# crowsonkb/style_transfer

Measured on AMD Instinct MI355X. Metric: tile-iterations/sec, VGG-19 2048px/1024-tile (fwd+bwd, Gram/content losses, regularizers, Adam step), higher is better.
Workload: dtype f32 (fp16x2-split MFMA, fp32 accumulate)

## Files before the change

### include/stx.h

```cpp
#ifndef STX_H_
#define STX_H_

#include <stddef.h>
#include <stdint.h>

#ifdef __cplusplus
extern "C" {
#endif

typedef struct stx_engine stx_engine;

typedef enum stx_status {
    STX_OK = 0,
    STX_ERR_ARG = -1,
    STX_ERR_HIP = -2,
    STX_ERR_STATE = -3,
    STX_ERR_UNSUPPORTED = -4,
    STX_ERR_NOMEM = -5
} stx_status;

typedef enum stx_mem { STX_HOST = 0, STX_DEVICE = 1 } stx_mem;

typedef enum stx_layer_type {
    STX_LAYER_INPUT = 0, STX_LAYER_CONV = 1, STX_LAYER_RELU = 2, STX_LAYER_POOL = 3
// ... 225 lines not shown
int stx_map_place(stx_engine *e, float *dst, int channels, int dst_h, int dst_w, int y0, int x0,
                  const float *src, int h, int w);
int stx_map_roll_add(stx_engine *e, float *acc, const float *src, int channels, int h, int w,
                     const int roll_xy[2], double alpha, double init_divisor);

int stx_image_resample(stx_engine *e, const float *src, int channels, int H, int W, float *dst,
                       int out_h, int out_w, const int *bounds_x, const double *weights_x,
                       int ksize_x, const int *bounds_y, const double *weights_y, int ksize_y,
                       int clamp_min_zero);

int stx_image_regularizers(stx_engine *e, const float *img, float *grad, int H, int W,
                           const float mean_bgr[3], double tv_scale, double tv_power,
                           double p_scale, double p_power, const float *aux, double aux_scale,
                           const int aux_roll_xy[2], double *loss_out);

int stx_image_swt_haar(stx_engine *e, const float *img, float *grad, int H, int W,
                       const int roll_xy[2], double scale, double power, double *loss_out);

int stx_image_swt_haar_levels(stx_engine *e, const float *img, float *grad, int H, int W, int levels,
                              const int roll_xy[2], double scale, double power, double *loss_out);

int stx_image_swt_daub_levels(stx_engine *e, const float *img, float *grad, int H, int W,
                              int order, int levels, const int *roll_xy,
                              double scale, double power, double *loss_out);

int stx_adam_step(stx_engine *e, float *params, const float *grad, float *g1, float *g2, float *p1,
                  float *avg_out, size_t n, double lr, double b1, double b2, double bp1,
                  double corr1, double corr2, double corrp);

int stx_vec_dot(stx_engine *e, const float *x, const float *y, size_t n, double *out_host_sync);
int stx_vec_axpy(stx_engine *e, double a, const float *x, float *y, size_t n);
int stx_vec_scale(stx_engine *e, double a, float *x, size_t n);
int stx_vec_mean_abs(stx_engine *e, const float *x, size_t n, double *out_host_sync);
int stx_vec_dot_async(stx_engine *e, const float *x, const float *y, size_t n, double *out_dev);
int stx_vec_abs_sum_async(stx_engine *e, const float *x, size_t n, double *out_dev);
int stx_vec_axpy_dev(stx_engine *e, double c1, const double *a_dev, double da, double c2,
                     const double *b_dev, double db, const float *x, float *y, size_t n);
int stx_vec_scale_dev(stx_engine *e, double c, const double *den_dev, double den_div, float *x,
                      size_t n);
int stx_vec_axpy_dot_dev(stx_engine *e, double c1, const double *a_dev, double da, double c2,
                         const double *b_dev, double db, double scale_c, const double *scale_den_dev,
                         double scale_div, const float *x, const float *src, float *y, const float *z,
                         size_t n, double *out_dev);
int stx_vec_lbfgs_pair(stx_engine *e, const float *g_new, float *g_old, const float *s, float *y, size_t n,
                       double *out_dev2, double *sy_host_sync);
int stx_vec_scale2_axpy(stx_engine *e, double c1, double c2, float *s, float *params, size_t n);

int stx_image_step_stats(stx_engine *e, const float *avg, float *old, int H, int W,
                         double stats[2]);
int stx_image_step_stats_async(stx_engine *e, const float *avg, float *old, int H, int W,
                               double raw_sums[2]);

int stx_image_to_u8(stx_engine *e, const float *img, int H, int W, const float mean_bgr[3],
                    uint8_t *out_rgb_u8);

int stx_image_to_u8_luma(stx_engine *e, const float *img, const float *content, int H, int W,
                         const float mean_bgr[3], uint8_t *out_rgb_u8);
int stx_image_color_stats(stx_engine *e, const float *img, int H, int W, double out_host_sync[9]);
int stx_image_color_affine(stx_engine *e, const float *src, float *dst, int H, int W, const double A[9],
                           const double b[3], const float mean_bgr[3]);

size_t stx_image_lap_floats(int H, int W, int n_pools, const int *pools);
int stx_image_lap_target(stx_engine *e, const float *content, int H, int W, int n_pools,
                         const int *pools, float *target_out);
int stx_image_lap(stx_engine *e, const float *img, float *grad, int H, int W, int n_pools,
                  const int *pools, const double *weights, const float *target, double scale,
                  double *loss_out);

int stx_image_photo(stx_engine *e, const float *img, const float *content, float *grad, int H, int W,
                    double eps, double scale, double *loss_out);

int stx_op_conv_forward(stx_engine *e, const float *x, int Cin, int H, int W, const float *w,
                        const float *b, int Cout, int ksize, int relu, float *y);
int stx_op_conv_backward_data(stx_engine *e, const float *dy, int Cout, int H, int W,
                              const float *w, int Cin, int ksize, const float *relu_mask_data,
                              float *dx);
int stx_op_pool_forward(stx_engine *e, const float *x, int C, int H, int W, int mode, float *y);
int stx_op_pool_backward(stx_engine *e, const float *dy, const float *x, int C, int H, int W,
                         int mode, const float *relu_mask_data, float *dx);

int stx_op_style_terms(stx_engine *e, const float *feat, int channels, int h, int w,
                       const float *gram_target, float *s_out, float *normalized_out,
                       double *half_sumsq, double *abs_sum);
int stx_op_masked_style_terms(stx_engine *e, const float *feat, int channels, int h, int w,
                              const float *mask_map, int mh, int mw, int oy, int ox, const int roll_xy[2],
                              const float *gram_target, float *sgrad_out, double out[3]);
int stx_op_masked_content_terms(stx_engine *e, const float *feat, int channels, int h, int w,
                                const float *content, int ch, int cw, const float *mask_map, int oy, int ox,
                                const int roll_xy[2], float *sgrad_out, double out[3]);
int stx_op_stat_terms(stx_engine *e, const float *feat, int channels, int h, int w, const float *MU,
                      const float *SD, float *s_out, double out[2]);
int stx_op_nnfm_terms(stx_engine *e, const float *feat, int channels, int h, int w, const float *bank, int rows,
                      float *s_out, int *index_out, double out[2]);
int stx_op_nnfm_patch_terms(stx_engine *e, const float *feat, int channels, int h, int w, int patch,
                            const float *bank, int rows, float *s_out, int *index_out, double out[2]);
int stx_op_nnfm_knn_terms(stx_engine *e, const float *feat, int channels, int h, int w, int patch, int k,
                          const float *bank, int rows, float *s_out, int *index_out, double out[2]);
int stx_op_nnfm_cover_terms(stx_engine *e, const float *feat, int channels, int h, int w, int patch, int k, float cover,
                            const float *bank, int rows, float *s_out, int *index_out, int *winner_out, double out[3]);
int stx_op_nnfm_guided_terms(stx_engine *e, const float *feat, int channels, int h, int w, int k, const float *bank,
                             const int *seg_rows, int segments, const float *mask_maps, int mh, int mw, int oy, int ox,
                             const int roll_xy[2], float *s_out, int *index_out, double out[3]);
int stx_op_swd_terms(stx_engine *e, const float *feat, int channels, int h, int w, const float *V, int dirs,
                     const float *Tq, int quantiles, float *s_out, int *rank_out, double out[2]);
int stx_op_selfsim_terms(stx_engine *e, const float *feat, const float *content, int channels, int h, int w,
                         int points, float *sgrad, double sc[2], signed char *signs_out);
int stx_op_shift_terms(stx_engine *e, const float *feat, int channels, int h, int w, const int *offsets,
                       int n_offsets, const float *grams, float *s_out, double out[2]);
int stx_op_content_terms(stx_engine *e, const float *feat, int channels, int h, int w,
                         const float *content, int content_h, int content_w, int oy, int ox,
                         const int roll_xy[2], float *normalized_out, double sums[2]);

int stx_profile_enable(stx_engine *e, int on);
int stx_profile_read(stx_engine *e, char *buf, size_t buf_len, size_t *needed);

int stx_amax_audit(stx_engine *e, int on);
int stx_amax_audit_read(stx_engine *e, char *buf, size_t buf_len, size_t *needed);

int stx_last_tile_ms(stx_engine *e, float *ms);

int stx_last_tile_flops(stx_engine *e, double *algorithmic, double *issued);

int stx_clock_marks(stx_engine *e, int on);
int stx_clock_marks_read(stx_engine *e, double *mhz, int max_values, int *n_values);

#ifdef __cplusplus
}
#endif
#endif
```

### style_transfer_amd/csrc/common.h

```cpp
#pragma once

#include <hip/hip_runtime.h>

#include <vector>

#include <cstdarg>
#include <cstdio>
#include <functional>
#include <string>

#include "stx.h"

namespace stx {

constexpr float kEps = 1.1920928955078125e-07f;

void set_error(const char *fmt, ...);

const char *sw_env(const char *name);
void sw_reread();

#define STX_HIP(call)                                                                       \
    do {                                                                                    \
        hipError_t err__ = (call);                                                          \
// ... 25 lines not shown
constexpr int kBlocks = 1024;
inline int blocks_for(size_t n) {
    const size_t b = (n + 255) / 256;
    return b < (size_t)kBlocks ? (int)b : kBlocks;
}
#ifdef __HIPCC__
__device__ __forceinline__ float wave_sum_f(float v) {
#pragma unroll
    for (int off = 32; off > 0; off >>= 1) v += __shfl_down(v, off, 64);
    return v;
}

template <int NV>
__device__ __forceinline__ void block_partials(float (&v)[NV], float *partials) {
    __shared__ float red[NV][4];
#pragma unroll
    for (int k = 0; k < NV; ++k) {
        const float s = wave_sum_f(v[k]);
        if ((threadIdx.x & 63) == 0) red[k][threadIdx.x >> 6] = s;
    }
    __syncthreads();
    if (threadIdx.x == 0) {
#pragma unroll
        for (int k = 0; k < NV; ++k)
            partials[k * gridDim.x + blockIdx.x] = red[k][0] + red[k][1] + red[k][2] + red[k][3];
    }
}

__device__ __forceinline__ unsigned pool_max_code(float v00, float v01, float v10, float v11, bool hx,
                                                  bool hy) {
    unsigned arg = 0;
    float best = v00;
    if (hx && v01 > best) best = v01, arg = 1;
    if (hy && v10 > best) best = v10, arg = 2;
    if (hx && hy && v11 > best) best = v11, arg = 3;
    return arg | (best > 0.f ? 4u : 0u);
}
__device__ __forceinline__ unsigned pool_ave_code(float v00, float v01, float v10, float v11, bool hx,
                                                  bool hy) {
    return (v00 > 0.f ? 1u : 0u) | (hx && v01 > 0.f ? 2u : 0u) | (hy && v10 > 0.f ? 4u : 0u) |
           (hx && hy && v11 > 0.f ? 8u : 0u);
}
#endif


enum ConvEpilogue {
    kEpiForward = 0,
    kEpiDgrad = 1,
    kEpiSymm = 2,
    kEpiDgradInject = 3,
    kEpiPartial = 4
};

struct ContentWindow {
    int C, fh, fw;
    int ch, cw;
    int oy, ox;
    int sy, sx;
};

struct ConvInject {
    const float *sgrad = nullptr, *s_abs_sum = nullptr;
    float s_coef = 0.f;
    const float *content = nullptr, *c_sums = nullptr, *feat = nullptr;
    float c_coef = 0.f;
    ContentWindow win{};
};

struct ConvProblem {
    const float *x;
    const float *w;
    float *y;
    const float *bias;
    const float *mask;
    float *partials;
    int K, M, H, W;
    int ksize;
    int relu;
    int epilogue;
    ConvInject inject;
    unsigned char *pool_codes = nullptr;
    unsigned char *in_codes = nullptr;
    const unsigned char *mask_codes = nullptr;
    unsigned char *out_codes = nullptr;
    bool wants_codes = false;
    bool skip_y = false;
    float *pool_out = nullptr;
    int pool_mode = 0;
    float *splitk_ws = nullptr;
    size_t splitk_ws_floats = 0;
    long long *clock_out = nullptr;
    const unsigned *x_amax = nullptr;
    unsigned *y_amax = nullptr;
    const unsigned char *pin_codes = nullptr;
    int pin_mode = 0;
    bool pin_mask = false;
    int *variant_out = nullptr;
#ifdef STX_EXPERIMENT_BF3
    const void *x_split = nullptr;
#endif
};

enum class ConvFamily { Direct, Wino2, H2 };

struct ConvConfig {
    ConvFamily family;
    int id;
    int bm;
    int kc;
    int pr, pc;
    int threads;
    size_t lds_bytes;
};

ConvConfig conv_pick_config(int ksize, int K, int M, int H, int W);
ConvConfig conv_config_by_id(int id);
bool direct_takes_inject(const ConvConfig &cfg);
int conv_num_workgroups(const ConvConfig &cfg, int M, int H, int W);
size_t conv_packed_floats(const ConvConfig &cfg, int K, int M, int ksize);
int conv_pack_weights(hipStream_t s, const float *w_caffe, int Mo, int Ko, int ksize,
                      int transpose_flip, const ConvConfig &cfg, float *packed);
int conv_launch(hipStream_t s, const ConvConfig &cfg, const ConvProblem &p, bool packed_weights);
int direct_splitk_factor(const ConvConfig &cfg, const ConvProblem &p, bool packed_weights);

int splitk_reduce_launch(hipStream_t s, const ConvProblem &p, int ksplit);
int splitk_reduce_items_launch(hipStream_t s, const ConvProblem &p, const ConvConfig &cfg, int slices,
                               int item_base, int items);
__host__ __device__ inline void wino2_item_tiles(int lt, int m_tiles, int n_patches, int &pt, int &mt) {
    pt = lt / m_tiles;
    mt = lt - pt * m_tiles;
    if (m_tiles == 8 && (n_patches & 7) == 0) {
        const int g = lt >> 5, r = lt & 31;
        mt = (g & 1) * 4 + (r & 3);
        pt = (g >> 1) * 8 + (r >> 2);
    }
}

struct WinoArgs {
    const float *x;
    const float *w;
    float *y;
    const float *bias;
    const float *mask;
    int K, M, H, W;
    int n_chunks, tiles_x, tiles_y, m_tiles, ksplit;
    int w_tile_stride;
    int x_bytes, w_bytes;
    int relu;
    ConvInject inj;
    float *pool_out;
    int pool_mode;
    unsigned char *pool_codes;
    int skip_y = 0;
    unsigned char *out_codes = nullptr;
    unsigned char *in_codes = nullptr;
    const unsigned char *mask_codes = nullptr;
    long long *clock_out = nullptr;
    int item_base = 0;
    const unsigned *x_amax = nullptr;
    unsigned *y_amax = nullptr;
    const unsigned char *pin_codes = nullptr;
    int pin_mode = 0, pin_mask = 0;
#ifdef STX_EXPERIMENT_BF3
    int vp_rows = 0, vp_tp = 0;
#endif
};

bool conv_first_usable(int K, int M, int ksize);
int conv_first_workgroups(int H, int W);
int conv_first_launch(hipStream_t s, const float *x, const float *w_caffe, const float *bias, float *y,
                      int K, int H, int W, int relu, float *gram_partials, unsigned *y_amax = nullptr);

ConvConfig wino2_config(int geometry = 0);
int wino2_pick_geometry(int H, int W);
size_t wino2_packed_floats(int K, int M);
int wino2_pack_weights(hipStream_t s, const float *w_caffe, int Mo, int Ko, int transpose_flip,
                       float *packed);
int wino2_launch(hipStream_t s, const ConvConfig &cfg, const ConvProblem &p, int ksplit);
bool wino2_fuses_pool(const ConvProblem &p);
bool wino2_uses_relu_codes(const ConvProblem &p, int ksplit);
bool wino2_writes_out_codes(const ConvConfig &cfg, const ConvProblem &p);
int wino2_splitk_factor(const ConvConfig &cfg, const ConvProblem &p);
struct Wino2Tail { int items, slices; };
Wino2Tail wino2_tail_split(const ConvConfig &cfg, const ConvProblem &p);
int wino2_max_slices(const ConvConfig &cfg, const ConvProblem &p);

constexpr int kAmaxSlots = 64;
ConvConfig h2_config(int mb, int pb = 1);
ConvConfig h2_pick_config(const ConvProblem &p);
bool h2_usable(const ConvProblem &p);
size_t h2_packed_floats(int K, int M);
int h2_pack_weights(hipStream_t s, const float *w_caffe, int Mo, int Ko, int transpose_flip, float *packed);
int h2_launch(hipStream_t s, const ConvConfig &cfg, const ConvProblem &p, int ksplit);
enum { kH2Style = 1, kH2Content = 2, kH2MaskNibbles = 4, kH2MaskBlob = 8 };
int h2_variant(const ConvProblem &p, int pin, bool split);
int h2_launch_variant(hipStream_t s, const WinoArgs &a, int n_wg, int cfg_id, int pin, int var);
int h2_splitk_factor(const ConvConfig &cfg, const ConvProblem &p);
bool h2_fuses_pool(const ConvProblem &p);
bool h2_takes_pooled_input(const ConvConfig &cfg, const ConvProblem &p);
int absmax_launch(hipStream_t s, const float *x, size_t n, unsigned *slots);

size_t conv_small_packed_floats(int K);
int conv_small_pack(hipStream_t s, const float *w_caffe, int Mo, int Ko, int transpose_flip,
                    float *packed);
int conv_small_launch(hipStream_t s, const float *x, const float *packed, float *y,
                      const float *mask, int K, int M, int H, int W);

bool conv_h2_enabled();
struct ConvTuner { int device; hipStream_t stream; hipEvent_t ev0, ev1; std::function<int(const ConvConfig &, const float **)> bank; };
int conv_choose(const ConvProblem &p, bool winograd, const ConvTuner *tuner, ConvConfig *out);
struct ConvBank { int key; size_t floats; std::function<int(hipStream_t, const float *w_caffe, float *packed)> pack; };
ConvBank conv_bank(const ConvConfig &cfg, int dir, int Mo, int Ko, int ksize);
ConvBank conv_small_bank(int Mo, int Ko);
int conv_dispatch(hipStream_t s, const ConvConfig &cfg, const ConvProblem &p, double *flop_algorithmic,
                  double *flop_issued);
int conv_splitk_factor(const ConvConfig &cfg, const ConvProblem &p);
size_t conv_splitk_floats(const ConvConfig &cfg, const ConvProblem &p);
bool conv_takes_clock(const ConvConfig &cfg);
bool conv_fuses_pool(const ConvConfig &cfg, const ConvProblem &p);
bool conv_writes_pool_codes(const ConvConfig &cfg);
bool conv_reads_x_amax(const ConvConfig &cfg);
bool conv_leaves_y_amax(const ConvConfig &cfg);
bool conv_takes_inject(const ConvConfig &cfg);
bool conv_takes_pooled_input(const ConvConfig &cfg, const ConvProblem &p);
bool conv_uses_relu_codes(const ConvConfig &cfg, const ConvProblem &p, int ksplit);
bool conv_writes_out_codes(const ConvConfig &cfg, const ConvProblem &p, int ksplit);

int pool_forward_launch(hipStream_t s, const float *x, int C, int H, int W, int mode, float *y,
                        unsigned char *codes = nullptr);
int pool_backward_codes_launch(hipStream_t s, const float *dy, const unsigned char *codes, int C,
                               int H, int W, int mode, bool relu_mask, float *dx);
int pool_backward_launch(hipStream_t s, const float *dy, const float *x, int C, int H, int W,
                         int mode, bool relu_mask, float *dx);

struct GramPlan {
    int C, HW, splits, tiles;
    int parts;
    size_t partial_floats;
};
GramPlan gram_plan(int C, int HW);
bool gram_h2_usable(const float *feat, int C, int HW);
int gram_partials_launch(hipStream_t s, const float *feat, const GramPlan &plan, float *partials,
                         const unsigned *f_amax = nullptr);
int gram_finish_blocks(const GramPlan &plan);
int gram_finish_launch(hipStream_t s, const float *partials, const GramPlan &plan, float *gram_out,
                       const float *target, float *dsym, float *sumsq, unsigned short *pieces = nullptr,
                       const unsigned *f_amax = nullptr, float *block_out = nullptr);

size_t symm_pieces_elems(int C);
int symm_num_workgroups(int C, int HW);
bool symm_bf3_usable(const float *feat, const float *out, int C, int HW);
bool symm_h2_usable(const float *feat, const float *out, int C, int HW);
int symm_h2_launch(hipStream_t s, const float *feat, const float *dsym, const unsigned *d_amax, int n_damax,
                   const unsigned *f_amax, float *out, float *partials, int C, int HW);
int symm_bf3_launch(hipStream_t s, const float *feat, const float *dsym, unsigned short *pieces,
                    bool pieces_ready, float *out, float *partials, int C, int HW);

#ifdef __HIPCC__
__device__ __forceinline__ int content_origin_y(const ContentWindow &w) { return w.oy - w.sy; }
__device__ __forceinline__ int content_origin_x(const ContentWindow &w) { return w.ox - w.sx; }
__device__ __forceinline__ size_t content_index(const ContentWindow &w, int c, int y, int x) {
    int yy = (content_origin_y(w) + y) % w.ch;
    int xx = (content_origin_x(w) + x) % w.cw;
    if (yy < 0) yy += w.ch;
    if (xx < 0) xx += w.cw;
    return ((size_t)c * w.ch + yy) * w.cw + xx;
}
#endif

struct SumJob {
    const float *src;
    int n;
    float *dst;
};
int sum_jobs_launch(hipStream_t s, const SumJob *jobs, int n_jobs);
int content_sums_launch(hipStream_t s, const float *feat, const float *content,
                        const ContentWindow &win, float *sums , std::vector<SumJob> *defer = nullptr);
int inject_style_launch(hipStream_t s, float *diff, const float *sgrad, size_t n,
                        const float *abs_sum, float coef, bool accumulate, unsigned *y_amax = nullptr);
int inject_content_launch(hipStream_t s, float *diff, const float *feat, const float *content,
                          const ContentWindow &win, const float *sums, float coef, bool accumulate,
                          unsigned *y_amax = nullptr);
int relu_inplace_launch(hipStream_t s, float *x, size_t n);
int sum_partials_launch(hipStream_t s, const float *partials, int n, float *out);
int sum_partials2_launch(hipStream_t s, const float *a, int na, float *out_a, const float *b, int nb,
                         float *out_b);

constexpr int kMaskParts = 1024;
constexpr int kMaskSgradParts = 2048;
int mask_map_launch(hipStream_t s, const float *mask, int H, int W, int scale, float *out);
int mask_apply_launch(hipStream_t s, const float *feat, const float *map, const ContentWindow &win, float *fm,
                      float *m2_partials, int *n_parts);
int mask_target_launch(hipStream_t s, const float *gs, int C, const float *m2_partials, int n_parts, int HW,
                       float *out, float *a_out);
int mask_sgrad_launch(hipStream_t s, float *sgrad, const float *map, const ContentWindow &win, const float *a,
                      float *partials, int *n_parts);

constexpr int kContentMaskParts = 1024;
int content_mask_mean_launch(hipStream_t s, const float *map, const ContentWindow &win, float *a_out);
int content_mask_term_launch(hipStream_t s, const float *feat, const float *content, const float *map,
                             const ContentWindow &win, const float *a, float *sgrad, float *partials,
                             int *n_parts);

constexpr int kStatSlice = 16384;
constexpr float kStatEps = 1e-5f;
int stat_slices(int HW);
size_t stat_scratch_floats(int C, int HW);
int stat_partials_launch(hipStream_t s, const float *feat, int C, int HW, float *partials);
int stat_finish_launch(hipStream_t s, const float *partials, int C, int HW, const float *MU, const float *SD,
                       float *table, float *e_out, float *mean_out, float *sd_out);
int stat_grad_launch(hipStream_t s, const float *feat, int C, int HW, const float *table, float *sgrad,
                     float *abs_partials, int *n_parts);

constexpr int kSwdBlock = 8192;
constexpr int kSwdMaxDirs = 4096, kSwdMaxQuantiles = 65536, kSwdMaxPixels = 1 << 22;
int swd_padded(int n);
int swd_check(const char *who, int C, long long n, int D, int Q);
int swd_e_parts(int n, int D);
size_t swd_scratch_floats(int C, int n, int D);
size_t swd_work_floats(int n, int D);
int swd_project_launch(hipStream_t s, const float *feat, int C, int n, const float *V, int D, void *records);
int swd_sort_launch(hipStream_t s, void *records, int n, int D);
int swd_finish_launch(hipStream_t s, void *records, int n, int D, const float *Tq, int Q, float *G, int *rank_out,
                      float *e_parts);
int swd_sort_passes(int n);
int swd_grad_launch(hipStream_t s, const float *V, const float *G, int C, int n, int D, float *sgrad, float *abs_parts,
                    int *n_parts);
int swd_quantiles_launch(hipStream_t s, const void *records, int n, int D, int Q, float *out);

constexpr int kSelfsimMaxPoints = 4096;
constexpr float kSelfsimEps = 1e-6f;
struct SelfsimGrid {
    int g, gh, gw, N;
};
SelfsimGrid selfsim_grid(int h, int w, int points);
int selfsim_check(const char *who, int C, int points);
struct SelfsimSource {
// ... 208 lines not shown
```

### style_transfer_amd/csrc/conv_h2.hip

```cpp

#include <algorithm>
#include <cstdlib>
#include <type_traits>

#include "common.h"
#include "f16x2.h"

#ifndef STX_H2_SKIP
#define STX_H2_SKIP 0
#endif

namespace stx {

namespace {

typedef _Float16 f16x8 __attribute__((ext_vector_type(8)));
typedef float f32x16 __attribute__((ext_vector_type(16)));
typedef float f32x4 __attribute__((ext_vector_type(4)));
typedef float f32x2 __attribute__((ext_vector_type(2)));
typedef unsigned int u32x4 __attribute__((ext_vector_type(4)));
typedef unsigned int u32x3 __attribute__((ext_vector_type(3)));
typedef unsigned int u32x2v __attribute__((__vector_size__(2 * sizeof(unsigned int))));

constexpr int KC = 16;
constexpr int NT = 512;
constexpr int PC = 32, TX = PC / 2;
constexpr int EX_BYTES = 4 * 2 * 4 * 4 * 64 * 16;
template <int PB>
struct Geo {
    static constexpr int PR = 8 * PB;
    static constexpr int XR = PR + 2;
    static constexpr int RT = XR * TX;
    static constexpr int V_PIECE = RT * 32;
    static constexpr int V_BYTES = 4 * 2 * V_PIECE;
    static constexpr int FULL = RT * 4 / 512;
    static constexpr int NU = FULL + 1;
    static constexpr size_t kLds = (EX_BYTES > 2 * V_BYTES ? EX_BYTES : 2 * V_BYTES) + 64;
};
constexpr int FRAG = 1024;
constexpr int U_KY = 4 * 2 * FRAG;
constexpr int U_BLK = 3 * U_KY;
constexpr int kHeaderFloats = 64;

__device__ __forceinline__ int sgpr(int v) { return __builtin_amdgcn_readfirstlane(v); }

template <int I, int N, typename F>
__device__ __forceinline__ void static_for(F &&f) {
    if constexpr (I < N) {
        f(std::integral_constant<int, I>{});
        static_for<I + 1, N>(f);
    }
}

__device__ __forceinline__ void lds_barrier() {
    asm volatile("s_waitcnt lgkmcnt(0)\n\ts_barrier" ::: "memory");
}


}

#ifdef STX_H2_TIMING
__device__ long long g_h2_timing[8][8];
__device__ long long g_h2_epi[8][8];
#define STX_H2_STAMP(i) if (pass == 0) t_epi[i] = clock64()
#else
#define STX_H2_STAMP(i)
#endif

template <int EPI, int MB, int PB, int PIN, int VAR = 0>
__global__ __launch_bounds__(NT) void conv_h2_kernel(WinoArgs a) {
    static_assert(VAR == 0 || EPI == kEpiDgradInject, "variants are of the injecting epilogue");
    static_assert(VAR == 0 || (((VAR & 3) == 1 || (VAR & 3) == 2) && ((VAR >> 2) == 1 || (VAR >> 2) == 2)), "h2_variant's codes");
    const bool inj_style = VAR ? (VAR & 1) != 0 : a.inj.sgrad != nullptr;
    const bool inj_content = VAR ? (VAR & 2) != 0 : a.inj.content != nullptr;
    const bool mask_nibbles = VAR ? (VAR >> 2) == 1 : a.mask_codes != nullptr;
    const bool mask_blob = VAR ? (VAR >> 2) == 2 : !a.mask_codes && a.mask;
    using G = Geo<PB>;
    [[maybe_unused]] constexpr int PR = G::PR, RT = G::RT, V_PIECE = G::V_PIECE, V_BYTES = G::V_BYTES, NU = G::NU, FULL = G::FULL;
    constexpr size_t kLdsBytes = G::kLds;
    constexpr int NJ = 4 * PB;
    extern __shared__ __attribute__((aligned(16))) char ldsb[];
#ifdef STX_H2_TIMING
    const long long t_start = clock64(), w_start = wall_clock64();
#endif
    constexpr int BM = 64 * MB;

    const int tid = threadIdx.x, lane = tid & 63;
    const int wave = sgpr(tid >> 6);
    const int xi = wave & 3, wh = wave >> 2;
    const int l31 = lane & 31, half = lane >> 5;

    const int m_tiles = a.m_tiles, a_tiles_x = a.tiles_x, a_tiles_y = a.tiles_y, a_H = a.H, a_W = a.W;
    const int a_n_chunks = a.n_chunks, a_ksplit = a.ksplit, a_item_base = a.item_base, a_x_bytes = a.x_bytes,
              a_w_bytes = a.w_bytes;
    const float *const a_x = a.x, *const a_w = a.w;
    asm volatile("" ::"s"(m_tiles), "s"(a_tiles_x), "s"(a_tiles_y), "s"(a_H), "s"(a_W), "s"(a_n_chunks), "s"(a_ksplit),
                 "s"(a_item_base), "s"(a_x_bytes), "s"(a_w_bytes), "s"(a_x), "s"(a_w));
    const int nb = gridDim.x, xcd = blockIdx.x & 7, slot_x = blockIdx.x >> 3;
    const int q8 = nb >> 3, r8 = nb & 7;
    const int L = (xcd < r8 ? xcd * (q8 + 1) : r8 * (q8 + 1) + (xcd - r8) * q8) + slot_x;
    const int kslice = sgpr(EPI == kEpiPartial ? L % a_ksplit : 0);
    const int Lt = sgpr(EPI == kEpiPartial ? a_item_base + L / a_ksplit : L);
    int ptile, mtile;
    wino2_item_tiles(Lt, m_tiles, a_tiles_x * a_tiles_y, ptile, mtile);
    ptile = sgpr(ptile);
    mtile = sgpr(mtile);
    const int c_begin = sgpr(EPI == kEpiPartial ? 2 * (kslice * (a_n_chunks >> 1) / a_ksplit) : 0);
    const int c_end = sgpr(EPI == kEpiPartial ? 2 * ((kslice + 1) * (a_n_chunks >> 1) / a_ksplit) : a_n_chunks);
    const int y0 = sgpr((ptile / a_tiles_x) * PR);
    const int x0 = sgpr((ptile % a_tiles_x) * PC);
    const int m0 = mtile * BM;
    const int HW = a_H * a_W;
    const unsigned HW4 = (unsigned)HW * 4u;
    const int pih = (a_H + 1) >> 1, piw = (a_W + 1) >> 1;
    const unsigned XP4 = PIN ? (unsigned)(pih * piw) * 4u : HW4;

    constexpr unsigned kOob = 0x80000000u;
    const __amdgpu_buffer_rsrc_t rx = __builtin_amdgcn_make_buffer_rsrc(
        const_cast<float *>(a_x), 0, a_x_bytes, 0x00020000);
    const __amdgpu_buffer_rsrc_t rw = __builtin_amdgcn_make_buffer_rsrc(
        const_cast<float *>(a_w), 0, a_w_bytes, 0x00020000);
    const __amdgpu_buffer_rsrc_t rcx = __builtin_amdgcn_make_buffer_rsrc(
        const_cast<unsigned char *>(a.pin_codes), 0, PIN ? (a_x_bytes >> 2) + 3 : 0, 0x00020000);

    float sv = 0.f, out_scale = 0.f, out_scale2 = 0.f;
    auto read_scales = [&]() __attribute__((always_inline)) {
        typedef const __attribute__((address_space(4))) unsigned *kconst_u32;
        const kconst_u32 slots = (kconst_u32)(uintptr_t)a.x_amax, header = (kconst_u32)(uintptr_t)a_w;
        unsigned amax_bits = 0;
#pragma unroll
        for (int i = 0; i < kAmaxSlots; ++i) amax_bits = max(amax_bits, slots[i]);
        const int es = sgpr(h2_scale_exp(amax_bits));
        const int ew = sgpr((int)header[(a_w_bytes >> 2) + 1]);
        sv = pow2f(es);
        const int eo = -es - ew, eo1 = eo < -126 ? -126 : eo > 127 ? 127 : eo;
        out_scale = pow2f(eo1), out_scale2 = pow2f(eo - eo1);
    };

    const bool edge = x0 == 0 || x0 + PC + 2 > a.W;
    unsigned xvoff[NU], v_dst[NU];
    bool left[NU], ok2[NU], ok3[NU];
#pragma unroll
    for (int n = 0; n < NU; ++n) {
        const int u = tid + n * NT;
        const int rt = n < FULL ? u >> 2 : 128 * FULL + (tid >> 4);
        const int ch0 = n < FULL ? (u & 3) * 4 : tid & 15;
        const int st_r = rt / TX, st_t = rt % TX;
        const int st_y = y0 - 1 + st_r, st_x = x0 + 2 * st_t - 1;
        left[n] = st_x < 0;
        ok2[n] = st_x + 2 < a.W, ok3[n] = st_x + 3 < a.W;
        xvoff[n] = kOob;
        if (PIN) {
            const int w0 = (x0 >> 1) + st_t - 1;
            if ((unsigned)st_y < (unsigned)a.H && st_x + 1 < a.W)
                xvoff[n] = (unsigned)(ch0 * pih * piw + (st_y >> 1) * piw + (left[n] ? 0 : w0)) * 4u +
                           (unsigned)(st_y & 1) + ((st_y | 1) < a.H ? 2u : 0u);
        } else if ((unsigned)st_y < (unsigned)a.H && st_x + 1 < a.W)
            xvoff[n] = (unsigned)(ch0 * HW + st_y * a.W + (left[n] ? 0 : st_x)) * 4u;
        v_dst[n] = (unsigned)(rt * 32 + ((ch0 * 2) ^ ((st_t & 8) << 1)));
// ... 160 lines not shown
        }
    };

    const unsigned a_voff = (unsigned)(xi * 2 * FRAG + lane * 16);
    const unsigned w_blk0 = (unsigned)(mtile * 2 * MB + wh * MB);
    constexpr bool LEAN = MB * PB == 2;
    f16x8 af[LEAN ? 2 : 3][MB][2];
    auto a_load = [&](int aslot, int ky, int chunk) __attribute__((always_inline)) {
#pragma unroll
        for (int b = 0; b < MB; ++b) {
            const unsigned ws = (unsigned)sgpr(
                (int)(((w_blk0 + b) * (unsigned)a.n_chunks + (unsigned)chunk) * U_BLK + (unsigned)ky * U_KY));
#pragma unroll
            for (int q = 0; q < 2; ++q)
                af[aslot][b][q] = __builtin_bit_cast(
                    f16x8, __builtin_amdgcn_raw_buffer_load_b128(rw, a_voff + q * FRAG, ws, 0));
        }
    };

    f32x16 acc[MB][NJ];
#pragma unroll
    for (int b = 0; b < MB; ++b)
#pragma unroll
        for (int j = 0; j < NJ; ++j)
#pragma unroll
            for (int r = 0; r < 16; ++r) acc[b][j][r] = 0.f;

    const unsigned b_base = (unsigned)(xi * 2 * V_PIECE + ((l31 >> 4) * 2 * TX + (l31 & 15)) * 32 +
                                       ((half * 16) ^ ((l31 & 8) << 1)));
    f16x8 bq[2][2];
    auto b_read = [&](int slot, int buf, int blk) __attribute__((always_inline)) {
        const int j = blk % NJ, ky = blk / NJ;
        const char *vb = ldsb + buf * V_BYTES + b_base + (4 * (j >> 1) + (j & 1) + ky) * TX * 32;
#pragma unroll
        for (int q = 0; q < 2; ++q) bq[slot][q] = *reinterpret_cast<const f16x8 *>(vb + q * V_PIECE);
    };

#ifdef STX_H2_TIMING
    const long long t_p0 = clock64();
#endif
    static_for<0, NU>([&](auto n_c) __attribute__((always_inline)) { x_load(decltype(n_c)::value, c_begin); });
    if (LEAN) {
        a_load(0, 0, c_begin);
    } else {
#pragma unroll
        for (int ky = 0; ky < 3; ++ky) a_load(ky, ky, c_begin);
    }
    __builtin_amdgcn_sched_barrier(0);
    read_scales();
#pragma unroll
    for (int b = 0; b < MB; ++b)
#pragma unroll
        for (int j = 0; j < NJ; ++j) asm volatile("" : "+v"(acc[b][j]));
    float s_scale = 0.f, c_scale = 0.f;
    if (EPI == kEpiDgradInject) {
        const float n = (float)((size_t)a.M * HW);
        if (inj_style) s_scale = a.inj.s_coef * (1.0f / (a.inj.s_abs_sum[0] / n + kEps));
        if (inj_content) c_scale = a.inj.c_coef * (1.0f / (a.inj.c_sums[1] / n + kEps));
    }
    const int hh = wave & 1, mrow = (wave >> 1) & 1, rqp = wave >> 2;
    const bool weven = (a.W & 1) == 0;
    const int xx0 = x0 + 2 * (l31 & 15);
    const unsigned plane_bytes = (unsigned)a.M * HW4;
    const __amdgpu_buffer_rsrc_t ry = __builtin_amdgcn_make_buffer_rsrc(
        a.y + (EPI == kEpiPartial ? (size_t)kslice * a.M * HW : 0), 0, (int)plane_bytes, 0x00020000);
    const __amdgpu_buffer_rsrc_t rmask = __builtin_amdgcn_make_buffer_rsrc(
        const_cast<float *>(a.mask), 0, a.mask ? (int)plane_bytes : 0, 0x00020000);
    const __amdgpu_buffer_rsrc_t rsg = __builtin_amdgcn_make_buffer_rsrc(
        const_cast<float *>(a.inj.sgrad), 0, a.inj.sgrad ? (int)plane_bytes : 0, 0x00020000);
    const __amdgpu_buffer_rsrc_t rft = __builtin_amdgcn_make_buffer_rsrc(
        const_cast<float *>(a.inj.feat), 0, a.inj.feat ? (int)plane_bytes : 0, 0x00020000);
    const __amdgpu_buffer_rsrc_t rbias = __builtin_amdgcn_make_buffer_rsrc(
        const_cast<float *>(a.bias), 0, a.bias ? a.M * 4 : 0, 0x00020000);
    const int ph = (a.H + 1) >> 1, pw = (a.W + 1) >> 1;
    const __amdgpu_buffer_rsrc_t rpool = __builtin_amdgcn_make_buffer_rsrc(
        a.pool_out, 0, a.pool_out ? a.M * ph * pw * 4 : 0, 0x00020000);
    const __amdgpu_buffer_rsrc_t rcodes = __builtin_amdgcn_make_buffer_rsrc(
        a.pool_codes, 0, a.pool_codes ? a.M * ph * pw : 0, 0x00020000);
    const int cph = (a.H + 1) >> 1, cpw = (a.W + 1) >> 1;
    const __amdgpu_buffer_rsrc_t rmc = __builtin_amdgcn_make_buffer_rsrc(
        const_cast<unsigned char *>(a.mask_codes), 0, a.mask_codes ? a.M * cph * cpw : 0, 0x00020000);
    const __amdgpu_buffer_rsrc_t roc = __builtin_amdgcn_make_buffer_rsrc(
        a.out_codes, 0, a.out_codes ? a.M * cph * cpw : 0, 0x00020000);
    const int M_ = a.M;
    struct LaneRows {
        int yy;
        unsigned vo[2][2], vpool, vmc;
    };
    const float *const content = a.inj.content;
    const int cw_ch = a.inj.win.ch, cw_cw = a.inj.win.cw, cw_oy = a.inj.win.oy - a.inj.win.sy,
              cw_ox = a.inj.win.ox - a.inj.win.sx;
    auto lane_rows = [&](int pbi) __attribute__((always_inline)) {
        LaneRows r;
        r.yy = y0 + 8 * pbi + 4 * mrow + 2 * (l31 >> 4);
        const unsigned lane_base = (unsigned)((4 * half) * HW + r.yy * a.W + xx0) * 4u;
#pragma unroll
        for (int y = 0; y < 2; ++y)
#pragma unroll
            for (int e = 0; e < 2; ++e)
                r.vo[y][e] = (r.yy + y < a.H && xx0 + e < a.W) ? lane_base + (unsigned)(y * a.W + e) * 4u : kOob;
        const bool in = r.yy < a.H && xx0 < a.W;
        r.vpool = in ? (unsigned)((4 * half) * ph * pw + (r.yy >> 1) * pw + (xx0 >> 1)) * 4u : kOob;
        r.vmc = in ? (unsigned)((4 * half) * cph * cpw + (r.yy >> 1) * cpw + (xx0 >> 1)) : kOob;
        return r;
    };
    constexpr bool HOIST = !(PIN && PB == 2);
    LaneRows rows0{};
    if (HOIST) rows0 = lane_rows(0);
    auto ld2 = [&](const __amdgpu_buffer_rsrc_t &rs, const LaneRows &lr, int y, unsigned so, auto even_c)
                   __attribute__((always_inline)) {
        if (decltype(even_c)::value)
            return __builtin_bit_cast(f32x2, __builtin_amdgcn_raw_buffer_load_b64(rs, lr.vo[y][0], so, 0));
        f32x2 v;
        v.x = __builtin_bit_cast(float, __builtin_amdgcn_raw_buffer_load_b32(rs, lr.vo[y][0], so, 0));
        v.y = __builtin_bit_cast(float, __builtin_amdgcn_raw_buffer_load_b32(rs, lr.vo[y][1], so, 0));
        return v;
    };
    auto st2 = [&](const __amdgpu_buffer_rsrc_t &rs, const LaneRows &lr, int y, unsigned so, f32x2 v, auto even_c)
                   __attribute__((always_inline)) {
        if (STX_H2_SKIP & 8) {
            if (v.x == 1.2345e-30f) __builtin_amdgcn_raw_buffer_store_b32(0u, rs, lr.vo[y][0], so, 0);
            return;
        }
        if (decltype(even_c)::value) {
            __builtin_amdgcn_raw_buffer_store_b64(__builtin_bit_cast(u32x2v, v), rs, lr.vo[y][0], so, 0);
        } else {
            const float v0 = v.x, v1 = v.y;
            __builtin_amdgcn_raw_buffer_store_b32(__builtin_bit_cast(unsigned, v0), rs, lr.vo[y][0], so, 0);
            __builtin_amdgcn_raw_buffer_store_b32(__builtin_bit_cast(unsigned, v1), rs, lr.vo[y][1], so, 0);
        }
    };
    int ccol[2] = {0, 0};
    auto content_columns = [&](const LaneRows &lr) __attribute__((always_inline)) {
        if (EPI == kEpiDgradInject && inj_content) {
#pragma unroll
            for (int e = 0; e < 2; ++e) {
                const bool ok = lr.yy < a.H && xx0 < a.W;
                const int x = ok ? (xx0 + e < a.W ? xx0 + e : xx0) : (e && 1 < a.W ? 1 : 0);
                int r = (cw_ox + x) % cw_cw;
                ccol[e] = r < 0 ? r + cw_cw : r;
            }
        }
    };
    if (HOIST) content_columns(rows0);
#ifdef STX_H2_TIMING
    __builtin_amdgcn_sched_barrier(0);
    const long long t_p1 = clock64();
    asm volatile("s_waitcnt vmcnt(0)" ::: "memory");
    const long long t_p2 = clock64();
#endif
    static_for<0, NU>([&](auto n_c) __attribute__((always_inline)) {
        constexpr int n = decltype(n_c)::value;
        stage_all(n, 0);
        if (c_begin + 1 < c_end) x_load(n, c_begin + 1);
    });
#ifdef STX_H2_TIMING
    __builtin_amdgcn_sched_barrier(0);
    const long long t_p3 = clock64();
#endif
    lds_barrier();
    b_read(0, 0, 0);

    constexpr int NBLK = 3 * NJ;
    constexpr int PER_BLK = 3 * MB, SLOTS = (NBLK - 1) * PER_BLK;
    constexpr int NQ = PIN ? 5 : 4, NQ1 = PIN ? 3 : 2;
    constexpr int NP = NQ * NU;
    constexpr int STEP = (SLOTS - 2) / NP;
#ifdef STX_H2_NO_BRANCH
    const bool edge_fix = false;
#else
    const bool edge_fix = edge;
#endif
    auto run_chunk = [&](auto buf_c, int chunk, auto more_c) __attribute__((always_inline)) {
        constexpr bool MORE = decltype(more_c)::value;
        constexpr int BUF = decltype(buf_c)::value, buf = BUF;
        char *vnext = ldsb + (buf ^ 1) * V_BYTES;
        static_for<0, NBLK>([&](auto blk_c) __attribute__((always_inline)) {
            constexpr int blk = decltype(blk_c)::value;
            constexpr int ky = blk / NJ, j = blk % NJ, slot = blk & 1;
            if (blk == NBLK - 1) {
                __builtin_amdgcn_sched_barrier(0);
                lds_barrier();
            }
            __builtin_amdgcn_sched_barrier(0);
            if (blk < NBLK - 1) b_read(slot ^ 1, buf, blk + 1);
            else if (MORE) b_read(0, buf ^ 1, 0);
            static_for<0, PER_BLK>([&](auto m_c) __attribute__((always_inline)) {
                constexpr int m = decltype(m_c)::value;
                constexpr int b = m % MB, t = m / MB;
// ... 7 lines not shown
                    if (ky < 2) a_load(as ^ 1, ky + 1, chunk);
                    else if (MORE) a_load(as ^ 1, 0, chunk + 1);
                }
                if (MORE && !(STX_H2_SKIP & 1) && s >= 1 && (s - 1) % STEP == 0) {
                    constexpr int k = (s - 1) / STEP;
                    constexpr int n = k % NU, q = k / NU;
                    if (k < NP && PIN && q == 0) unpool(n, edge_fix);
                    else if (k < NP && n < FULL) piece(n, q - (PIN ? 1 : 0), vnext, edge_fix);
                    else if (k < NP && q < NQ1) piece_one(2 * (q - (PIN ? 1 : 0)), vnext, edge_fix);
                }
                if (MORE && !(STX_H2_SKIP & 4)) {
                    static_for<0, NU>([&](auto u_c) __attribute__((always_inline)) {
                        constexpr int u = decltype(u_c)::value;
                        if (s == 1 + (((u < FULL ? NQ : NQ1) - 1) * NU + u) * STEP + 1 && chunk + 2 < c_end)
                            x_load(u, chunk + 2);
                    });
                }
            });
            if (!LEAN && j == NJ - 1 && MORE && !(STX_H2_SKIP & 2)) a_load(ky, ky, chunk + 1);
        });
        __builtin_amdgcn_sched_barrier(0);
    };
    using yes = std::integral_constant<bool, true>;
    using no = std::integral_constant<bool, false>;
    using b0 = std::integral_constant<int, 0>;
    using b1 = std::integral_constant<int, 1>;
#ifdef STX_H2_TIMING
    const long long t_loop = clock64(), w_loop = wall_clock64();
#endif
    const bool mark = a.clock_out != nullptr && (int)blockIdx.x == (int)(gridDim.x >> 1);
    long long mark_c = 0, mark_w = 0;
    if (mark) {
        mark_c = clock64();
        mark_w = wall_clock64();
    }
    {
        int chunk = c_begin;
        for (; chunk + 2 < c_end; chunk += 2) {
            run_chunk(b0{}, chunk, yes{});
            run_chunk(b1{}, chunk + 1, yes{});
        }
        run_chunk(b0{}, chunk, yes{});
        run_chunk(b1{}, chunk + 1, no{});
    }
    if (mark) {
        const long long dc = clock64() - mark_c, dw = wall_clock64() - mark_w;
        if (tid == 0) {
            a.clock_out[0] = dw >= 100 ? dc : 0;
            a.clock_out[1] = dw >= 100 ? dw : 0;
        }
    }
#ifdef STX_H2_TIMING
    const long long t_end = clock64(), w_end = wall_clock64();
#endif

    float amax = 0.f;
    f32x4 *ex = reinterpret_cast<f32x4 *>(ldsb);

#ifdef STX_H2_TIMING
    long long t_epi[4] = {0, 0, 0, 0};
#endif
    auto epilogue_pass = [&](auto pass_c, auto even_c) __attribute__((always_inline)) {
        constexpr int pass = decltype(pass_c)::value;
        constexpr int mbi = pass % MB, pbi = pass / MB;
        const LaneRows lr = pbi == 0 && HOIST ? rows0 : lane_rows(pbi);
        if (!HOIST && pass == 0) content_columns(lr);
        int crow[2] = {0, 0};
        if (EPI == kEpiDgradInject && inj_content) {
#pragma unroll
            for (int y = 0; y < 2; ++y) {
                const bool ok = lr.yy + y < a.H && xx0 < a.W;
                int q = (cw_oy + (ok ? lr.yy + y : 0)) % cw_ch;
                crow[y] = (q < 0 ? q + cw_ch : q) * cw_cw;
            }
        }
        const int cblk = m0 + (hh * MB + mbi) * 32;
        auto chan = [&](int n) __attribute__((always_inline)) {
            const int c0 = cblk + (n & 3) + 8 * (2 * rqp + (n >> 2));
            return sgpr(c0 < M_ ? c0 : M_);
        };
        float bs[8];
        f32x2 mk[16], sg[16];
        unsigned mkb[8];
#pragma unroll
        for (int n = 0; n < 8; ++n) {
            const int c = chan(n);
            const unsigned so = (unsigned)c * HW4;
            if (EPI == kEpiForward) {
                bs[n] = a.bias ? __builtin_bit_cast(float, __builtin_amdgcn_raw_buffer_load_b32(
                                                               rbias, (unsigned)half * 16u, (unsigned)c * 4u, 0))
                               : 0.f;
            } else if (EPI != kEpiPartial) {
                if (mask_nibbles) mkb[n] = __builtin_amdgcn_raw_buffer_load_b8(rmc, lr.vmc, (unsigned)(c * cph * cpw), 0);
#pragma unroll
                for (int y = 0; y < 2; ++y) {
                    if (mask_blob && !(STX_H2_SKIP & 16)) mk[2 * n + y] = ld2(rmask, lr, y, so, even_c);
                    if (EPI == kEpiDgradInject && inj_style) sg[2 * n + y] = ld2(rsg, lr, y, so, even_c);
                }
            }
        }
        STX_H2_STAMP(0);
        __syncthreads();
        STX_H2_STAMP(1);
#pragma unroll
        for (int j = 0; j < 4; ++j)
#pragma unroll
            for (int rq = 0; rq < 4; ++rq)
                ex[(((xi * 2 + wh) * 4 + j) * 4 + rq) * 64 + lane] =
                    f32x4{acc[mbi][4 * pbi + j][4 * rq], acc[mbi][4 * pbi + j][4 * rq + 1],
                          acc[mbi][4 * pbi + j][4 * rq + 2], acc[mbi][4 * pbi + j][4 * rq + 3]};
        __syncthreads();
        STX_H2_STAMP(2);
#pragma unroll
        for (int rqi = 0; rqi < 2; ++rqi) {
            const int rq = 2 * rqp + rqi;
            f32x4 o[2][2];
#pragma unroll
            for (int s = 0; s < 2; ++s) {
                f32x4 p[4];
#pragma unroll
                for (int c = 0; c < 4; ++c) p[c] = ex[(((c * 2 + hh) * 4 + 2 * mrow + s) * 4 + rq) * 64 + lane];
                o[s][0] = (p[0] + p[1] + p[2]) * out_scale * out_scale2;
                o[s][1] = (p[1] - p[2] - p[3]) * out_scale * out_scale2;
            }
#pragma unroll
            for (int e = 0; e < 4; ++e) {
                const int n = 4 * rqi + e;
                const int c = chan(n);
                const unsigned so = (unsigned)c * HW4;
                f32x2 v[2];
#pragma unroll
                for (int y = 0; y < 2; ++y) v[y] = f32x2{o[y][0][e], o[y][1][e]};
                if (EPI == kEpiForward) {
                    if (a.bias) {
#pragma unroll
                        for (int y = 0; y < 2; ++y) v[y].x += bs[n], v[y].y += bs[n];
                    }
                    if (a.relu) {
#pragma unroll
                        for (int y = 0; y < 2; ++y) v[y].x = fmaxf(v[y].x, 0.f), v[y].y = fmaxf(v[y].y, 0.f);
                    }
                } else if (EPI != kEpiPartial) {
#pragma unroll
                    for (int y = 0; y < 2; ++y) {
                        if (mask_nibbles) {
                            const unsigned nib = mkb[n] >> (2 * y);
                            v[y].x = (nib & 1u) ? v[y].x : 0.f;
                            v[y].y = (nib & 2u) ? v[y].y : 0.f;
                        } else if (mask_blob && !(STX_H2_SKIP & 16)) {
                            v[y].x = mk[2 * n + y].x > 0.f ? v[y].x : 0.f;
                            v[y].y = mk[2 * n + y].y > 0.f ? v[y].y : 0.f;
                        }
                        if (EPI == kEpiDgradInject) {
                            if (inj_content) {
                                const f32x2 ft = ld2(rft, lr, y, so, even_c);
                                const int mm = c + 4 * half;
                                const int cm = mm < a.M ? mm : 0;
                                const float *cp = content + (size_t)cm * cw_ch * cw_cw + crow[y];
                                v[y].x += c_scale * (ft.x - cp[ccol[0]]);
                                v[y].y += c_scale * (ft.y - cp[ccol[1]]);
                            }
                            if (inj_style) {
                                v[y].x += s_scale * sg[2 * n + y].x;
                                v[y].y += s_scale * sg[2 * n + y].y;
                            }
                        }
                    }
                }
#pragma unroll
                for (int y = 0; y < 2; ++y) {
                    if (EPI != kEpiForward || !a.skip_y) st2(ry, lr, y, so, v[y], even_c);
                    if (EPI != kEpiPartial)
                        amax = fmaxf(amax, fmaxf(lr.vo[y][0] != kOob ? fabsf(v[y].x) : 0.f,
                                                 lr.vo[y][1] != kOob ? fabsf(v[y].y) : 0.f));
                }
                if (EPI == kEpiForward && a.out_codes) {
                    const unsigned nib = (lr.vo[0][0] != kOob && v[0].x > 0.f ? 1u : 0u) |
                                         (lr.vo[0][1] != kOob && v[0].y > 0.f ? 2u : 0u) |
                                         (lr.vo[1][0] != kOob && v[1].x > 0.f ? 4u : 0u) |
                                         (lr.vo[1][1] != kOob && v[1].y > 0.f ? 8u : 0u);
                    __builtin_amdgcn_raw_buffer_store_b8((unsigned char)nib, roc, lr.vmc, (unsigned)(c * cph * cpw), 0);
                }
                if (EPI == kEpiForward && a.pool_out) {
                    const bool hy = lr.yy + 1 < a.H, hx = decltype(even_c)::value || xx0 + 1 < a.W;
                    float pr;
                    if (a.pool_mode == STX_POOL_MAX) {
                        pr = hx ? fmaxf(v[0].x, v[0].y) : v[0].x;
                        if (hy) pr = hx ? fmaxf(fmaxf(pr, v[1].x), v[1].y) : fmaxf(pr, v[1].x);
                    } else {
                        pr = (v[0].x + (hx ? v[0].y : 0.f) + (hy ? v[1].x : 0.f) + (hx && hy ? v[1].y : 0.f)) *
                             (hy ? (hx ? 0.25f : 0.5f) : (hx ? 0.5f : 1.0f));
                    }
                    __builtin_amdgcn_raw_buffer_store_b32(__builtin_bit_cast(unsigned, pr), rpool, lr.vpool,
                                                          (unsigned)c * (unsigned)(ph * pw * 4), 0);
                    if (a.pool_codes) {
                        const unsigned code = a.pool_mode == STX_POOL_MAX
                                                  ? pool_max_code(v[0].x, v[0].y, v[1].x, v[1].y, hx, hy)
                                                  : pool_ave_code(v[0].x, v[0].y, v[1].x, v[1].y, hx, hy);
                        __builtin_amdgcn_raw_buffer_store_b8((unsigned char)code, rcodes, lr.vpool >> 2,
                                                             (unsigned)c * (unsigned)(ph * pw), 0);
                    }
                }
            }
        }
    };
    static_for<0, MB * PB>([&](auto pass_c) __attribute__((always_inline)) {
        [[maybe_unused]] constexpr int pass = decltype(pass_c)::value;
        if (weven) epilogue_pass(pass_c, yes{});
        else epilogue_pass(pass_c, no{});
        STX_H2_STAMP(3);
    });
    if (EPI != kEpiPartial && a.y_amax) {
#pragma unroll
        for (int d = 32; d >= 1; d >>= 1) amax = fmaxf(amax, __shfl_xor(amax, d));
        float *wmax = reinterpret_cast<float *>(ldsb + kLdsBytes - 64);
        if (lane == 0) wmax[wave] = amax;
        __syncthreads();
        if (tid == 0) {
#pragma unroll
            for (int w = 1; w < 8; ++w) amax = fmaxf(amax, wmax[w]);
            atomicMax(a.y_amax + (blockIdx.x & (kAmaxSlots - 1)), __builtin_bit_cast(unsigned, amax));
        }
    }
#ifdef STX_H2_TIMING
    if (blockIdx.x == gridDim.x - 3 && lane == 0) {
        g_h2_timing[wave][0] = t_loop - t_start, g_h2_timing[wave][1] = t_end - t_loop;
        g_h2_timing[wave][2] = clock64() - t_end;
        g_h2_timing[wave][3] = w_loop - w_start, g_h2_timing[wave][4] = w_end - w_loop;
        g_h2_timing[wave][5] = wall_clock64() - w_end;
        for (int i = 0; i < 4; ++i) g_h2_epi[wave][i] = t_epi[i] - t_end;
        g_h2_epi[wave][4] = t_p0 - t_start, g_h2_epi[wave][5] = t_p1 - t_p0, g_h2_epi[wave][6] = t_p2 - t_p1, g_h2_epi[wave][7] = t_p3 - t_p2;
    }
#endif
}

template <int EPI, int MB, int PB, int PIN = 0, int VAR = 0>
static int h2_launch_epi(hipStream_t s, const WinoArgs &args, int n_wg) {
    auto kern = conv_h2_kernel<EPI, MB, PB, PIN, VAR>;
    constexpr size_t kLdsBytes = Geo<PB>::kLds;
    hipError_t e = hipFuncSetAttribute(reinterpret_cast<const void *>(kern),
                                       hipFuncAttributeMaxDynamicSharedMemorySize, (int)kLdsBytes);
    if (e != hipSuccess) {
        set_error("hipFuncSetAttribute(lds=%zu): %s", kLdsBytes, hipGetErrorString(e));
        return STX_ERR_HIP;
    }
    kern<<<n_wg, NT, kLdsBytes, s>>>(args);
    STX_CHECK_LAUNCH();
    return STX_OK;
}

#if defined(STX_H2_VARIANTS_ONLY) || !(defined(STX_H2_SPLIT_UNITS) || defined(STX_H2_DEV_SUBSET))
int h2_launch_variant(hipStream_t s, const WinoArgs &a, int n_wg, int cfg_id, int pin, int var) {
#define STX_H2_VAR(V, P)                                                                                      \
    if (var == (V) && pin == (P))                                                                             \
        return cfg_id == 1   ? h2_launch_epi<kEpiDgradInject, 2, 1, P, V>(s, a, n_wg)                         \
               : cfg_id == 2 ? h2_launch_epi<kEpiDgradInject, 1, 2, P, V>(s, a, n_wg)                         \
                             : h2_launch_epi<kEpiDgradInject, 1, 1, P, V>(s, a, n_wg);
    STX_H2_VAR(kH2Style | kH2MaskNibbles, 0)
    STX_H2_VAR(kH2Style | kH2MaskBlob, 0)
    STX_H2_VAR(kH2Content | kH2MaskNibbles, 0)
    STX_H2_VAR(kH2Content | kH2MaskBlob, 0)
    STX_H2_VAR(kH2Style | kH2MaskNibbles, 1 + STX_POOL_MAX)
    STX_H2_VAR(kH2Style | kH2MaskBlob, 1 + STX_POOL_MAX)
    STX_H2_VAR(kH2Style | kH2MaskNibbles, 1 + STX_POOL_AVE)
    STX_H2_VAR(kH2Style | kH2MaskBlob, 1 + STX_POOL_AVE)
#undef STX_H2_VAR
    set_error("h2_launch_variant: no specialised body %d for a pooled input of kind %d", var, pin);
    return STX_ERR_UNSUPPORTED;
}
#endif
#ifndef STX_H2_VARIANTS_ONLY

__global__ __launch_bounds__(256) void absmax_kernel(const float *__restrict__ x, size_t n, unsigned *slots) {
    float m = 0.f;
    const size_t head = ((16 - (reinterpret_cast<size_t>(x) & 15)) & 15) >> 2;
    const size_t h = head < n ? head : n;
    const size_t n4 = (n - h) >> 2;
    const f32x4 *x4 = reinterpret_cast<const f32x4 *>(x + h);
    for (size_t i = blockIdx.x * (size_t)256 + threadIdx.x; i < n4; i += (size_t)gridDim.x * 256) {
        const f32x4 v = x4[i];
        m = fmaxf(fmaxf(m, fmaxf(fabsf(v.x), fabsf(v.y))), fmaxf(fabsf(v.z), fabsf(v.w)));
    }
    if (blockIdx.x == 0) {
        if (threadIdx.x < h) m = fmaxf(m, fabsf(x[threadIdx.x]));
        const size_t tail = h + (n4 << 2);
        if (tail + threadIdx.x < n && threadIdx.x < 4) m = fmaxf(m, fabsf(x[tail + threadIdx.x]));
    }
#pragma unroll
    for (int d = 32; d >= 1; d >>= 1) m = fmaxf(m, __shfl_xor(m, d));
    __shared__ float wmax[4];
    if ((threadIdx.x & 63) == 0) wmax[threadIdx.x >> 6] = m;
    __syncthreads();
    if (threadIdx.x == 0)
        atomicMax(slots + (blockIdx.x & (kAmaxSlots - 1)),
                  __builtin_bit_cast(unsigned, fmaxf(fmaxf(wmax[0], wmax[1]), fmaxf(wmax[2], wmax[3]))));
}

int absmax_launch(hipStream_t s, const float *x, size_t n, unsigned *slots) {
    STX_HIP(hipMemsetAsync(slots, 0, kAmaxSlots * sizeof(unsigned), s));
    if ((reinterpret_cast<size_t>(x) & 3) != 0) {
        set_error("absmax_launch: the array is not float-aligned");
        return STX_ERR_ARG;
    }
    const int blocks = (int)std::min<size_t>((n / 4 + 2047) / 2048 + 1, 1024);
    absmax_kernel<<<blocks, 256, 0, s>>>(x, n, slots);
    STX_CHECK_LAUNCH();
    return STX_OK;
}

size_t h2_packed_floats(int K, int M) {
    return (size_t)ceil_div(M, 32) * ceil_div(K, KC) * (U_BLK / 4) + kHeaderFloats;
}

__device__ __forceinline__ float h2_u(const float *__restrict__ w, int Ko, int transpose_flip, int m, int k,
                                      int ky, int x) {
    float g[3];
#pragma unroll
    for (int b = 0; b < 3; ++b) {
        const int t = ky * 3 + b;
        g[b] = transpose_flip ? w[((size_t)k * Ko + m) * 9 + (8 - t)] : w[((size_t)m * Ko + k) * 9 + t];
    }
    return x == 0 ? g[0] : x == 1 ? (g[0] + g[1] + g[2]) * 0.5f : x == 2 ? (g[0] - g[1] + g[2]) * 0.5f : g[2];
}

__global__ void h2_bank_max_kernel(const float *__restrict__ w, int Ko, int transpose_flip, int M, int K,
                                   unsigned *header) {
    const size_t total = (size_t)M * K * 12;
    float mx = 0.f;
    for (size_t idx = blockIdx.x * (size_t)blockDim.x + threadIdx.x; idx < total;
         idx += (size_t)gridDim.x * blockDim.x) {
        const int x = idx % 4, ky = (idx / 4) % 3;
        const size_t mk = idx / 12;
        mx = fmaxf(mx, fabsf(h2_u(w, Ko, transpose_flip, (int)(mk / K), (int)(mk % K), ky, x)));
    }
#pragma unroll
    for (int d = 32; d >= 1; d >>= 1) mx = fmaxf(mx, __shfl_xor(mx, d));
    __shared__ float wmax[4];
    if ((threadIdx.x & 63) == 0) wmax[threadIdx.x >> 6] = mx;
    __syncthreads();
    if (threadIdx.x == 0)
        atomicMax(header, __builtin_bit_cast(unsigned, fmaxf(fmaxf(wmax[0], wmax[1]), fmaxf(wmax[2], wmax[3]))));
}

__global__ void h2_pack_kernel(const float *__restrict__ w, int Ko, int transpose_flip, int M, int K,
                               int n_chunks, unsigned short *__restrict__ packed, size_t total,
                               unsigned *header) {
    const int ew = h2_scale_exp(header[0]);
    const float sw = pow2f(ew);
// ... 30 lines not shown
        w_caffe, Ko, transpose_flip, M, K, header);
    STX_CHECK_LAUNCH();
    const size_t total = bank_floats * 2;
    h2_pack_kernel<<<(int)std::min<size_t>((total + 255) / 256, 8192), 256, 0, s>>>(
        w_caffe, Ko, transpose_flip, M, K, ceil_div(K, KC), reinterpret_cast<unsigned short *>(packed), total,
        header);
    STX_CHECK_LAUNCH();
    return STX_OK;
}

ConvConfig h2_config(int mb, int pb) {
    const bool two = mb != 2 && pb == 2;
    return {ConvFamily::H2, mb == 2 ? 1 : two ? 2 : 0, mb == 2 ? 128 : 64, KC, two ? 16 : 8, PC, NT,
            two ? Geo<2>::kLds : Geo<1>::kLds};
}

bool h2_usable(const ConvProblem &p) {
    if (p.ksize != 3 || p.K % (2 * KC) != 0 || p.K < 2 * KC) return false;
    if (p.epilogue != kEpiForward && p.epilogue != kEpiDgrad) return false;
    if (p.epilogue == kEpiForward && (p.wants_codes || p.in_codes)) return false;
    const double xb = 4.0 * p.K * (double)p.H * p.W, yb = 4.0 * p.M * (double)p.H * p.W;
    const double wb = 4.0 * (double)h2_packed_floats(p.K, p.M);
    return xb < 2147483648.0 && yb < 2147483648.0 && wb < 2147483648.0;
}

static double h2_plan(const ConvConfig &cfg, const ConvProblem &p, int *factor) {
    const int n_pairs = p.K / (2 * KC);
    const long n = (long)ceil_div(p.M, cfg.bm) * ceil_div(p.H, cfg.pr) * ceil_div(p.W, PC);
    const double out_mb = 4e-6 * p.M * (double)p.H * p.W;
    const double t_chunk = cfg.id == 1 ? 2.75 : cfg.id == 2 ? 3.5 : 2.0, t_fixed = cfg.id != 0 ? 17.0 : 8.5;
    const bool may_split = p.epilogue == kEpiForward || p.epilogue == kEpiDgrad;
    double best_cost = 0;
    int best = 1;
    for (int f = 1; f <= 8 && (f == 1 || (may_split && n_pairs / f >= 2)); ++f) {
        const double rounds = (double)ceil_div((int)std::min<long>(n * f, 1 << 30), 256);
        double c = rounds * (2.0 * ceil_div(n_pairs, f) * t_chunk + t_fixed);
        if (f > 1) c += (f + 1) * out_mb / 3.0 + 5.0;
        if (f == 1 || c < best_cost) {
            best_cost = c;
            best = f;
        }
    }
    *factor = best;
    return best_cost;
}

int h2_splitk_factor(const ConvConfig &cfg, const ConvProblem &p) {
    int f;
    h2_plan(cfg, p, &f);
    return f;
}

ConvConfig h2_pick_config(const ConvProblem &p) {
    int f;
    ConvConfig best = h2_config(1, 1);
    double best_cost = h2_plan(best, p, &f);
    const ConvConfig cand[2] = {h2_config(2, 1), h2_config(1, 2)};
    for (int i = 0; i < 2; ++i) {
        if (i == 0 && p.M % 128 != 0) continue;
        const double c = h2_plan(cand[i], p, &f);
        if (c < best_cost) best_cost = c, best = cand[i];
    }
    return best;
}

bool h2_takes_pooled_input(const ConvConfig &cfg, const ConvProblem &p) {
    return p.epilogue == kEpiDgrad && h2_usable(p) && h2_splitk_factor(cfg, p) == 1;
}

bool h2_fuses_pool(const ConvProblem &p) {
    return p.pool_out && p.epilogue == kEpiForward && (((size_t)p.y | (size_t)p.pool_out) & 7) == 0;
}

#ifdef STX_H2_DEV_SUBSET
template __global__ void conv_h2_kernel<0, 2, 1, 0>(WinoArgs);
template __global__ void conv_h2_kernel<0, 1, 2, 0>(WinoArgs);
template __global__ void conv_h2_kernel<1, 2, 1, 0>(WinoArgs);
template __global__ void conv_h2_kernel<3, 2, 1, 0>(WinoArgs);
template __global__ void conv_h2_kernel<3, 1, 2, 1>(WinoArgs);
template __global__ void conv_h2_kernel<3, 2, 1, 0, kH2Style | kH2MaskNibbles>(WinoArgs);
template __global__ void conv_h2_kernel<3, 2, 1, 0, kH2Content | kH2MaskNibbles>(WinoArgs);
template __global__ void conv_h2_kernel<3, 1, 2, 1, kH2Style | kH2MaskBlob>(WinoArgs);
template __global__ void conv_h2_kernel<3, 2, 1, 1, kH2Style | kH2MaskNibbles>(WinoArgs);
#else
int h2_variant(const ConvProblem &p, int pin, bool split) {
    if (split || p.epilogue != kEpiDgrad) return 0;
    const bool style = p.inject.sgrad != nullptr, content = p.inject.content != nullptr;
    if (style == content) return 0;
    if (!p.mask_codes && !p.mask) return 0;
    if (content && pin) return 0;
    const char *env = sw_env("STX_H2_INJECT_GENERIC");
    if (env && atoi(env) != 0) return 0;
    return (style ? kH2Style : kH2Content) | (p.mask_codes ? kH2MaskNibbles : kH2MaskBlob);
}

int h2_launch(hipStream_t s, const ConvConfig &cfg, const ConvProblem &p, int ksplit) {
    if (!h2_usable(p) || !p.x_amax) {
        set_error("h2_launch: unsupported problem (K %d, epilogue %d, input maximum %s)", p.K, p.epilogue,
                  p.x_amax ? "given" : "missing");
        return STX_ERR_UNSUPPORTED;
    }
    WinoArgs a;
    a.x = p.x;
    a.w = p.w;
    a.y = p.y;
    a.bias = p.bias;
    a.mask = p.mask;
    a.K = p.K;
    a.M = p.M;
    a.H = p.H;
    a.W = p.W;
    a.n_chunks = p.K / KC;
    a.tiles_x = ceil_div(p.W, PC);
    a.tiles_y = ceil_div(p.H, cfg.pr);
    a.m_tiles = ceil_div(p.M, cfg.bm);
    a.ksplit = 1;
    a.w_tile_stride = 0;
    a.relu = p.relu;
    a.inj = p.inject;
    a.pool_out = nullptr;
    a.pool_codes = nullptr;
    a.pool_mode = p.pool_mode;
    a.x_bytes = (int)(4.0 * p.K * (double)p.H * p.W);
    const bool pin = p.pin_codes != nullptr;
    if (pin) {
        if (!h2_takes_pooled_input(cfg, p) || ksplit > 1) {
            set_error("h2_launch: a pooled input goes with unsplit backward launches only");
            return STX_ERR_UNSUPPORTED;
        }
        a.x_bytes = (int)(4.0 * p.K * (double)((p.H + 1) / 2) * ((p.W + 1) / 2));
        a.pin_codes = p.pin_codes;
        a.pin_mode = p.pin_mode;
        a.pin_mask = p.pin_mask ? 1 : 0;
    }
    a.w_bytes = (int)(4 * (h2_packed_floats(p.K, p.M) - kHeaderFloats));
    a.clock_out = p.clock_out;
    a.x_amax = p.x_amax;
    a.y_amax = p.y_amax;
    a.mask_codes = p.epilogue == kEpiDgrad ? p.mask_codes : nullptr;
    a.out_codes = p.epilogue == kEpiForward && p.relu ? p.out_codes : nullptr;
    const bool inject = p.epilogue == kEpiDgrad && (p.inject.sgrad || p.inject.content);
    int n_wg = a.m_tiles * a.tiles_x * a.tiles_y;
    const bool split = ksplit > 1 && p.splitk_ws && p.splitk_ws_floats >= (size_t)ksplit * p.M * p.H * p.W;
    if (split) {
        a.ksplit = ksplit;
        a.y = p.splitk_ws;
        a.y_amax = nullptr;
        a.mask_codes = nullptr;
        a.out_codes = nullptr;
        n_wg *= ksplit;
    } else if (h2_fuses_pool(p)) {
        a.pool_out = p.pool_out;
        a.pool_codes = p.pool_codes;
        a.skip_y = p.skip_y && p.pool_codes != nullptr;
    }
    const int epi = split ? kEpiPartial : inject ? kEpiDgradInject : p.epilogue;
    const int pin_kind = pin ? 1 + p.pin_mode : 0;
    const int var = h2_variant(p, pin_kind, split);
    if (p.variant_out) *p.variant_out = var;
    if (var) return h2_launch_variant(s, a, n_wg, cfg.id, pin_kind, var);
#define STX_H2_CASE(E)                                                                   \
    case E:                                                                              \
        STX_TRY(cfg.id == 1   ? (h2_launch_epi<E, 2, 1>(s, a, n_wg))                   \
                : cfg.id == 2 ? (h2_launch_epi<E, 1, 2>(s, a, n_wg))                   \
                                : (h2_launch_epi<E, 1, 1>(s, a, n_wg)));                 \
        break;
#define STX_H2_PIN_CASE(E, P)                                                            \
    case E:                                                                              \
        STX_TRY(cfg.id == 1   ? (h2_launch_epi<E, 2, 1, P>(s, a, n_wg))                \
                : cfg.id == 2 ? (h2_launch_epi<E, 1, 2, P>(s, a, n_wg))                \
                                : (h2_launch_epi<E, 1, 1, P>(s, a, n_wg)));              \
        break;
    if (pin && p.pin_mode == STX_POOL_MAX) {
        switch (epi) {
            STX_H2_PIN_CASE(kEpiDgrad, 1 + STX_POOL_MAX)
            STX_H2_PIN_CASE(kEpiDgradInject, 1 + STX_POOL_MAX)
        }
        return STX_OK;
    }
    if (pin) {
        switch (epi) {
            STX_H2_PIN_CASE(kEpiDgrad, 1 + STX_POOL_AVE)
            STX_H2_PIN_CASE(kEpiDgradInject, 1 + STX_POOL_AVE)
        }
        return STX_OK;
    }
#undef STX_H2_PIN_CASE
    switch (epi) {
        STX_H2_CASE(kEpiForward)
        STX_H2_CASE(kEpiDgrad)
        STX_H2_CASE(kEpiDgradInject)
        STX_H2_CASE(kEpiPartial)
        default:
            set_error("h2_launch: no kernel for epilogue %d", p.epilogue);
            return STX_ERR_UNSUPPORTED;
    }
#undef STX_H2_CASE
    return split ? splitk_reduce_launch(s, p, ksplit) : STX_OK;
}
#endif
#endif

}
```

### style_transfer_amd/csrc/engine.cpp

```cpp

#include <algorithm>
#include <atomic>
#include <cstdlib>
#include <cstring>

#include "engine.h"

namespace stx {

static thread_local std::string g_error;

void set_error(const char *fmt, ...) {
    char buf[1024];
    va_list ap;
    va_start(ap, fmt);
    vsnprintf(buf, sizeof buf, fmt, ap);
    va_end(ap);
    g_error = buf;
}

int alloc_scalars(stx_engine *e, size_t n, size_t *index) {
    stx_engine::ScalarArena &a = e->A();
    if (a.used + n > e->scalars_cap) {
        set_error("scalar arena exhausted (%zu + %zu > %zu)", a.used, n, e->scalars_cap);
// ... 264 lines not shown
    }
    {
        std::vector<int> h224(e->blobs.size(), 224);
        for (size_t li = 1; li < e->layers.size(); ++li) {
            const Layer &L = e->layers[li];
            if (L.type == STX_LAYER_CONV) h224[L.top_blob] = h224[L.bottom_blob];
            if (L.type == STX_LAYER_POOL) h224[L.top_blob] = pooled_len(h224[L.bottom_blob]);
        }
        for (size_t bi = 0; bi < e->blobs.size(); ++bi) e->blobs[bi].scale = 224 / h224[bi];
    }
    enable_peer_access(device);
    STX_HIP(hipStreamCreateWithFlags(&e->stream, hipStreamNonBlocking));
    for (int i = 0; i < stx_engine::kTimed; ++i) {
        STX_HIP(hipEventCreate(&e->ev_start[i]));
        STX_HIP(hipEventCreate(&e->ev_stop[i]));
    }
    STX_HIP(hipEventCreate(&e->ev_tune0));
    STX_HIP(hipEventCreate(&e->ev_tune1));
    if (const char *env = sw_env("STX_AUTOTUNE")) e->autotune = atoi(env) != 0;
    if (const char *env = sw_env("STX_POOL_CODES")) e->pool_codes = atoi(env) != 0;
    if (const char *env = sw_env("STX_WINOGRAD")) e->winograd = atoi(env) != 0;
    e->scalars_cap = kScalarFloats;
    for (stx_engine::ScalarArena &a : e->arena) {
        STX_TRY(a.scalars.ensure(e->scalars_cap * sizeof(float)));
        STX_HIP(hipHostMalloc(reinterpret_cast<void **>(&a.host), e->scalars_cap * sizeof(float),
                              hipHostMallocDefault));
        STX_TRY(a.dscalars.ensure(e->dscalars_cap * sizeof(double)));
        STX_HIP(hipHostMalloc(reinterpret_cast<void **>(&a.dhost), e->dscalars_cap * sizeof(double),
                              hipHostMallocDefault));
        STX_HIP(hipEventCreateWithFlags(&a.fence, hipEventDisableTiming));
    }
    STX_TRY(e->red_scratch.ensure(9 * kBlocks * sizeof(float)));
    {
        std::lock_guard<std::mutex> lock(e->sh->mutex);
        e->sh->members.push_back(e.get());
    }
    *out = e.release();
    return STX_OK;
}

extern "C" {

int stx_engine_create(int device, const stx_layer_desc *layers, int n_layers, stx_engine **out) {
    return build_engine(device, layers, n_layers, nullptr, out);
}

int stx_engine_create_shared(stx_engine *primary, stx_engine **out) {
    if (!primary || !out) {
        set_error("stx_engine_create_shared: bad arguments");
        return STX_ERR_ARG;
    }
    std::vector<stx_layer_desc> descs(primary->layers.size());
    for (size_t i = 0; i < descs.size(); ++i) {
        const Layer &L = primary->layers[i];
        stx_layer_desc &d = descs[i];
        d.name = L.name.c_str();
        d.type = L.type;
        d.bottom = L.bottom.empty() ? nullptr : L.bottom.c_str();
        d.top = L.top.c_str();
        d.num_output = i == 0 ? primary->blobs[L.top_blob].channels : L.num_output;
        d.kernel_size = L.ksize;
        d.pad = L.pad;
        d.stride = L.stride;
        d.pool_mode = L.pool_mode;
    }
    STX_TRY(primary->set_device());
    for (stx_engine *m : primary->sh->members) STX_HIP(hipStreamSynchronize(m->stream));
    return build_engine(primary->device, descs.data(), (int)descs.size(), primary->sh, out);
}

void stx_engine_destroy(stx_engine *e) {
    if (!e) return;
    (void)hipSetDevice(e->device);
    if (e->stream) (void)hipStreamSynchronize(e->stream);
    for (auto &b : e->sgrad) b->release();
    e->marks_buf.release();
    e->amax.release();
    e->audit_buf.release();
    for (Blob &b : e->blobs) {
        b.data.release();
        b.diff.release();
        b.codes.release();
        b.relu_codes.release();
    }
    for (hipEvent_t ev : e->fence_events) (void)hipEventDestroy(ev);
    bool last;
    {
        std::lock_guard<std::mutex> lock(e->sh->mutex);
        auto &m = e->sh->members;
        m.erase(std::remove(m.begin(), m.end(), e), m.end());
        last = m.empty();
    }
    if (last) {
        for (auto &kv : e->sh->conv) {
            kv.second.w.release();
            kv.second.b.release();
            for (auto &p : kv.second.packed) p.second->release();
        }
        clear_all_targets(*e->sh);
    }
    DevBuf *bufs[] = {&e->shift_io, &e->selfsim_io, &e->swd_work, &e->swd_io, &e->nnfm_scratch, &e->stat_scratch, &e->masked_feat, &e->masked_target, &e->splitk, &e->gram_partials, &e->gram, &e->dsym, &e->dsym_pieces, &e->symm_partials,
                      &e->upload, &e->red_scratch, &e->swt_scratch, &e->lap_scratch, &e->first_gram, &e->color_sums};
    for (DevBuf *b : bufs) b->release();
    for (stx_engine::SwtTable &t : e->swt_tables) t.taps.release();
    for (stx_engine::ScalarArena &a : e->arena) {
        a.scalars.release();
        a.dscalars.release();
        if (a.host) (void)hipHostFree(a.host);
        if (a.dhost) (void)hipHostFree(a.dhost);
        if (a.fence) (void)hipEventDestroy(a.fence);
    }
    for (auto &pe : e->prof) {
        (void)hipEventDestroy(pe.start);
        (void)hipEventDestroy(pe.stop);
    }
    for (hipEvent_t ev : e->event_pool) (void)hipEventDestroy(ev);
    for (int i = 0; i < stx_engine::kTimed; ++i) {
        if (e->ev_start[i]) (void)hipEventDestroy(e->ev_start[i]);
        if (e->ev_stop[i]) (void)hipEventDestroy(e->ev_stop[i]);
    }
    if (e->ev_tune0) (void)hipEventDestroy(e->ev_tune0);
    if (e->ev_tune1) (void)hipEventDestroy(e->ev_tune1);
    if (e->stream) (void)hipStreamDestroy(e->stream);
    delete e;
}

int stx_set_conv_weights(stx_engine *e, const char *conv_layer, const float *weights,
                         const float *bias, int mem) {
    if (!e || !conv_layer || !weights) return STX_ERR_ARG;
    STX_TRY(e->set_device());
    auto it = e->layer_index.find(conv_layer);
    if (it == e->layer_index.end() || e->layers[it->second].type != STX_LAYER_CONV) {
        set_error("stx_set_conv_weights: '%s' is not a convolution layer", conv_layer);
        return STX_ERR_ARG;
    }
    std::lock_guard<std::mutex> lock(e->sh->mutex);
    const bool shared = e->sh->members.size() > 1;
    if (shared) STX_TRY(quiesce_members(e));
    ConvParams &cp = e->sh->conv[it->second];
    const size_t nw = (size_t)cp.cout * cp.cin * cp.ks * cp.ks;
    STX_TRY(cp.w.ensure(nw * sizeof(float)));
    STX_TRY(cp.b.ensure((size_t)cp.cout * sizeof(float)));
    STX_TRY(copy_in(e, cp.w.ptr, weights, mem, nw * sizeof(float)));
    if (bias)
        STX_TRY(copy_in(e, cp.b.ptr, bias, mem, (size_t)cp.cout * sizeof(float)));
    else
        STX_HIP(hipMemsetAsync(cp.b.ptr, 0, (size_t)cp.cout * sizeof(float), e->stream));
    if (mem == STX_HOST || shared) STX_HIP(hipStreamSynchronize(e->stream));
    for (auto &p : cp.packed) p.second->release();
    cp.packed.clear();
    cp.set = true;
    return STX_OK;
}

int stx_sync(stx_engine *e) {
    if (!e) return STX_ERR_ARG;
    STX_TRY(e->set_device());
    return do_sync(e);
}

int stx_fence(stx_engine *e, unsigned long long *ticket) {
    if (!e || !ticket) return STX_ERR_ARG;
    STX_TRY(e->set_device());
    stx_engine::ScalarArena &a = e->A();
    STX_HIP(hipEventRecord(a.fence, e->stream));
    a.ticket = e->next_ticket++;
// ... 262 lines not shown
```

### style_transfer_amd/csrc/engine.h

```cpp
#pragma once

#include <deque>
#include <map>
#include <memory>
#include <mutex>
#include <string>
#include <vector>

#include "common.h"

namespace stx {

struct DevBuf {
    void *ptr = nullptr;
    size_t bytes = 0;
    int ensure(size_t need) {
        if (need <= bytes) return STX_OK;
        if (ptr) STX_HIP(hipFree(ptr));
        ptr = nullptr;
        bytes = 0;
        const size_t want = (need + 255) & ~(size_t)255;
        hipError_t err = hipMalloc(&ptr, want);
        if (err != hipSuccess) {
            set_error("hipMalloc(%zu bytes) failed: %s", want, hipGetErrorString(err));
            ptr = nullptr;
            return STX_ERR_NOMEM;
        }
        bytes = want;
        return STX_OK;
    }
    void release() {
        if (ptr) (void)hipFree(ptr);
        ptr = nullptr;
        bytes = 0;
    }
    float *f() const { return static_cast<float *>(ptr); }
};

struct Layer {
    std::string name, bottom, top;
    int type = 0, num_output = 0, ksize = 0, pad = 0, stride = 1, pool_mode = 0;
    int bottom_blob = -1, top_blob = -1;
};

struct Blob {
    std::string name;
    int channels = 0;
    int producer = -1;
    bool relu = false;
    int scale = 1;
    int h = 0, w = 0;
    DevBuf data, diff;
    DevBuf codes;
    bool codes_valid = false;
    DevBuf relu_codes;
    bool relu_codes_valid = false;
    bool relu_codes_wanted = false;
    int amax_data = -1, amax_diff = -1;
    size_t count() const { return (size_t)channels * h * w; }
};

struct ConvParams {
    int cin = 0, cout = 0, ks = 0;
    DevBuf w, b;
    bool set = false;
    std::map<int, std::unique_ptr<DevBuf>> packed;
};

struct ContentTarget {
    int index, blob, C, h, w;
    std::unique_ptr<DevBuf> feat;
    void release() { feat->release(); }
};

struct StyleTarget {
    int index, blob, C;
    std::unique_ptr<DevBuf> gram;
    void release() { gram->release(); }
};

struct StyleMask {
    int index, blob, h, w;
    std::unique_ptr<DevBuf> map;
    void release() { map->release(); }
};

struct ContentMask {
    int blob, h, w;
    std::unique_ptr<DevBuf> map;
    void release() { map->release(); }
};

struct StatTarget {
    int blob, C;
    double weight;
    std::unique_ptr<DevBuf> ms;
    void release() { ms->release(); }
};

struct NnfmTarget {
    int blob, C, rows;
    double weight;
    std::unique_ptr<DevBuf> bank, pieces;
    int patch = 1, k = 1;
    float cover = 0.f;
    NnfmSegments segs{};
    int mh = 0, mw = 0;
    std::unique_ptr<DevBuf> maps;
    const unsigned short *pieces_hi_lo() const { return static_cast<const unsigned short *>(pieces->ptr); }
    void release() {
        bank->release();
        pieces->release();
        if (maps) maps->release();
    }
};

struct SwdTarget {
    int blob, C, D, Q;
    double weight;
    std::unique_ptr<DevBuf> vt;
    const float *V() const { return vt->f(); }
    const float *Tq() const { return vt->f() + (size_t)D * C; }
    void release() { vt->release(); }
};

struct SelfsimTarget {
    int blob, points;
    double weight;
    void release() {}
};

struct ShiftTarget {
    int blob, C;
    ShiftOffsets off;
    double weight;
    std::unique_ptr<DevBuf> grams;
    void release() { grams->release(); }
};

struct LossTerm {
// ... 197 lines not shown
    clear_dependent_targets(sh);
}
ConvProblem conv_fwd_problem(const float *x, float *y, const float *bias, int Cin, int Cout, int H, int W,
                             int ks, int relu);
ConvProblem conv_bwd_problem(const float *dy, float *dx, const float *mask, int Cout, int Cin, int H, int W,
                             int ks);
int attach_splitk(stx_engine *e, const ConvConfig &cfg, ConvProblem &p);
int launch_conv(stx_engine *e, const ConvConfig &cfg, const ConvProblem &problem);
int amax_scratch(stx_engine *e, unsigned **out);
constexpr size_t kMaxAmaxAudit = 2048;
int amax_audit_note(stx_engine *e, hipStream_t stream, const std::string &consumer, const std::string &blob,
                    bool diff, const unsigned *slots, const float *x, size_t n);
struct Tap {
    int blob;
    const stx_tap *t;
};

struct TileCall {
    const float *img;
    int img_mem, th, tw, rx, ry, start[2];
    const stx_tap *taps;
    int n_taps;
    float *grad_out;
    int grad_mem;
};

enum class TermKind { Content, MaskedContent, Style, MaskedStyle, Stat, Nnfm, NnfmGuided, Swd, Selfsim, Shift, Dream };
constexpr size_t kNoSlot = ~(size_t)0;
constexpr size_t kResidualScalars = 2 + 2 * 1024;

struct PlannedTerm {
    TermKind kind;
    int tap;
    const float *target, *mask;
    ContentWindow win;
    double coef;
    size_t scalars;
    size_t scratch_off, scratch_len;
    size_t sgrad_off;
    const NnfmTarget *nnfm = nullptr;
    const SwdTarget *swd = nullptr;
    int points = 0;
    const ShiftTarget *shift = nullptr;
};

struct TilePlan {
    std::vector<Tap> order;
    std::vector<char> needed;
    std::vector<int> tap_of;
    std::deque<stx_tap> extra;
    bool sums_late;
    bool interleave;
    std::vector<PlannedTerm> terms;
    std::vector<size_t> first_term;
    std::vector<size_t> sgrad_floats;
    size_t scratch_floats = 0, scalars = 0;
};

struct Term {
    enum Kind { Gradient, Residual } kind;
    const float *src;
    const float *sums;
    float coef;
    ContentWindow win;
};

struct TileRun {
    stx_engine *e;
    const TilePlan &plan;
    PendingLoss &pl;
    std::vector<std::vector<Term>> terms;
    std::vector<SumJob> sum_jobs;
    std::vector<SumJob> *defer() { return plan.sums_late ? &sum_jobs : nullptr; }
};

int plan_terms(stx_engine *e, const TileCall &c, TilePlan &plan);
int queue_tap_terms(TileRun &run, size_t k);
int inject_terms(TileRun &run, size_t k, bool &diff_written);
bool tap_fusable(const TileRun &run, size_t k);
ConvInject make_inject(const TileRun &run, size_t k, const Blob &bot);
int launch_style_terms(stx_engine *e, hipStream_t stream, const float *feat, int C, int h, int w,
                       const float *target, float *sgrad, float *sc, const std::string &name,
                       const unsigned *f_amax = nullptr, float *term_scratch = nullptr,
                       std::vector<SumJob> *defer = nullptr);
constexpr size_t kMaskScratchFloats = kMaskParts + kMaskSgradParts;
int launch_masked_style_terms(stx_engine *e, hipStream_t stream, const float *feat, int C, int h, int w,
                              const float *mask_map, const ContentWindow &win, const float *target,
                              float *sgrad, float *sc, const std::string &name, const unsigned *f_amax,
                              float *term_scratch, float *mask_scratch, std::vector<SumJob> *defer);
int launch_stat_terms(stx_engine *e, hipStream_t stream, const float *feat, int C, int h, int w, const float *MU,
                      const float *SD, float *sgrad, float *sc, const std::string &name, float *stat_scratch,
                      std::vector<SumJob> *defer);
int launch_nnfm_terms(stx_engine *e, hipStream_t stream, const float *feat, int C, int h, int w, int patch,
                      const float *bank, const unsigned short *pieces, int rows, float *sgrad, int *idx_out, float *sc,
                      const std::string &name, float *scratch, std::vector<SumJob> *defer, int k = 1, float cover = 0.f,
                      int *winner_out = nullptr, float *e_cov_out = nullptr);
int launch_nnfm_guided_terms(stx_engine *e, hipStream_t stream, const float *feat, int C, int h, int w,
                             const float *bank, const unsigned short *pieces, const NnfmSegments &segs,
                             const float *maps, const ContentWindow &win, float *sgrad, int *idx_out, float *sc,
                             const std::string &name, float *scratch, std::vector<SumJob> *defer, int k,
                             bool scale_by_a);
int launch_swd_terms(stx_engine *e, hipStream_t stream, const float *feat, int C, int h, int w, const float *V, int D,
                     const float *Tq, int Q, float *sgrad, int *rank_out, float *sc, const std::string &name,
                     float *scratch, std::vector<SumJob> *defer);
int launch_selfsim_terms(stx_engine *e, hipStream_t stream, const float *feat, const SelfsimSource &content, int C,
                         int h, int w, int points, float *sgrad, signed char *signs_out, float *sc,
                         const std::string &name, float *scratch, std::vector<SumJob> *defer);
int launch_shift_terms(stx_engine *e, hipStream_t stream, const float *feat, int C, int h, int w,
                       const ShiftOffsets &off, const float *targets, float *sgrad, float *sc, const std::string &name,
                       float *scratch, std::vector<SumJob> *defer);
constexpr size_t kContentMaskScratchFloats = 2 * kContentMaskParts;
int launch_masked_content_terms(stx_engine *e, hipStream_t stream, const float *feat, const float *content,
                                const float *mask_map, const ContentWindow &win, float *sgrad, float *sc,
                                const std::string &name, float *partials, std::vector<SumJob> *defer);
#pragma GCC visibility pop

}
```

### style_transfer_amd/csrc/op_hooks.cpp

```cpp

#include <cmath>

#include "engine.h"

extern "C" {

static int scratch_pack(stx_engine *e, const ConvBank &bank, const float *w, const float **packed) {
    STX_TRY(e->upload.ensure(bank.floats * sizeof(float)));
    STX_TRY(bank.pack(e->stream, w, e->upload.f()));
    *packed = e->upload.f();
    return STX_OK;
}

static int hook_conv(stx_engine *e, ConvProblem &p, const float *w, int Mo, int Ko, int dir) {
    ConvConfig cfg;
    STX_TRY(conv_choose(p, e->winograd, nullptr, &cfg));
    if (conv_reads_x_amax(cfg)) {
        unsigned *scratch;
        STX_TRY(amax_scratch(e, &scratch));
        STX_TRY(absmax_launch(e->stream, p.x, (size_t)p.K * p.H * p.W, scratch));
        STX_HIP(hipMemsetAsync(scratch + kAmaxSlots, 0, kAmaxSlots * sizeof(unsigned), e->stream));
        p.x_amax = scratch;
        p.y_amax = scratch + kAmaxSlots;
    }
// ... 310 lines not shown

int stx_op_nnfm_guided_terms(stx_engine *e, const float *feat, int C, int h, int w, int k, const float *bank,
                             const int *seg_rows, int segments, const float *mask_maps, int mh, int mw, int oy, int ox,
                             const int roll_xy[2], float *s_out, int *index_out, double out[3]) {
    const char *const who = "stx_op_nnfm_guided_terms";
    if (!e || !feat || !bank || !seg_rows || !mask_maps || !s_out || !index_out || !out || C <= 0 || h <= 0 || w <= 0) {
        set_error("%s: bad arguments", who);
        return STX_ERR_ARG;
    }
    if (segments < 1 || segments > kNnfmMaxSegments) {
        set_error("%s: %d segments (1 to %d are expected)", who, segments, kNnfmMaxSegments);
        return STX_ERR_ARG;
    }
    if (k < 1 || k > kNnfmMaxK) {
        set_error("%s: k %d (1 to %d is expected)", who, k, kNnfmMaxK);
        return STX_ERR_ARG;
    }
    long long rows = 0;
    for (int s = 0; s < segments; ++s) {
        if (seg_rows[s] < k) {
            set_error("%s: segment %d has %d rows, fewer than k = %d", who, s, seg_rows[s], k);
            return STX_ERR_ARG;
        }
        rows += seg_rows[s];
    }
    if (oy < 0 || ox < 0 || oy + h > mh || ox + w > mw) {
        set_error("%s: window exceeds the mask maps", who);
        return STX_ERR_ARG;
    }
    if (C % 64 != 0) {
        set_error("%s: the channel count %d is not a multiple of 64", who, C);
        return STX_ERR_UNSUPPORTED;
    }
    const long long n = (long long)h * w;
    if (n >= (1ll << 31) / C || rows >= (1ll << 31) / C) {
        set_error("%s: %lld columns against %lld rows of %d channels exceed 32-bit offsets", who, n, rows, C);
        return STX_ERR_UNSUPPORTED;
    }
    const NnfmSegments segs = nnfm_segments(seg_rows, segments);
    STX_TRY(e->set_device());
    HookScalars scalars(e);
    float *sc;
    const float *host;
    STX_TRY(scalars.take(3, &sc));
    const size_t pieces = nnfm_pieces_floats((int)rows, C);
    STX_TRY(e->nnfm_scratch.ensure((pieces + nnfm_guided_scratch_floats(C, h * w, segs, k)) * sizeof(float)));
    unsigned short *bhi = static_cast<unsigned short *>(e->nnfm_scratch.ptr);
    STX_TRY(nnfm_split_rows_launch(e->stream, bank, (int)rows, C, bhi, bhi + (size_t)rows * C));
    STX_TRY(launch_nnfm_guided_terms(e, e->stream, feat, C, h, w, bank, bhi, segs, mask_maps,
                                     hook_window(C, h, w, mh, mw, oy, ox, roll_xy), s_out, index_out, sc, "op",
                                     e->nnfm_scratch.f() + pieces, nullptr, k, false));
    STX_TRY(scalars.fetch(&host));
    out[0] = (double)host[0];
    out[1] = (double)host[1];
    out[2] = (double)host[2];
    return STX_OK;
}

int stx_op_content_terms(stx_engine *e, const float *feat, int C, int h, int w,
                         const float *content, int content_h, int content_w, int oy, int ox,
                         const int roll_xy[2], float *normalized_out, double sums[2]) {
    if (!e || !feat || !content || C <= 0 || h <= 0 || w <= 0) return STX_ERR_ARG;
    if (oy < 0 || ox < 0 || oy + h > content_h || ox + w > content_w) {
        set_error("stx_op_content_terms: window exceeds the content map");
        return STX_ERR_ARG;
    }
    STX_TRY(e->set_device());
    const ContentWindow win = hook_window(C, h, w, content_h, content_w, oy, ox, roll_xy);
    HookScalars scalars(e);
    float *s;
    const float *host;
    STX_TRY(scalars.take(kResidualScalars, &s));
    STX_TRY(content_sums_launch(e->stream, feat, content, win, s));
    if (normalized_out)
        STX_TRY(inject_content_launch(e->stream, normalized_out, feat, content, win, s, 1.0f, false));
    STX_TRY(scalars.fetch(&host));
    if (sums) {
        sums[0] = (double)host[0];
        sums[1] = (double)host[1];
    }
    return STX_OK;
}

}
```

### style_transfer_amd/csrc/symm.hip

```cpp

#include <algorithm>
#include <cstdlib>
#include <cstring>

#include "bf16x3.h"
#include "common.h"
#include "f16x2.h"

#ifndef STX_SYMM_SKIP
#define STX_SYMM_SKIP 0
#endif

namespace stx {

namespace {

constexpr int kSM = 64;
constexpr int kSN = 256;
#ifndef STX_SYMM_KSK
#define STX_SYMM_KSK 32
#endif
constexpr int kSK = STX_SYMM_KSK;
constexpr int kSPC = kSK / 16;
constexpr int kSegs = kSK / 8;
constexpr int kDLoads = 3 * kSM * kSegs / 256;
constexpr int kRowBytes = 2 * kSK + 16;
#ifndef STX_SYMM_RING
#define STX_SYMM_RING 3
#endif
constexpr int kRing = STX_SYMM_RING;
constexpr int kPieceBytes = kSM * kRowBytes;
constexpr int kChunkBytes = 3 * kPieceBytes;

typedef unsigned u32x4y __attribute__((ext_vector_type(4)));

}

size_t symm_pieces_elems(int C) {
    const size_t cp = (size_t)ceil_div(C, kSM) * kSM;
    return 3 * cp * cp;
}

template <bool BIG>
__global__ __launch_bounds__(256, 2) void symm_bf3_kernel(const float *__restrict__ F,
                                                          const unsigned short *__restrict__ Dp,
                                                          float *__restrict__ S,
                                                          float *__restrict__ partials, int C, int Cp,
                                                          int HW, unsigned f_bytes, int m_tiles) {
    __shared__ __attribute__((aligned(16))) unsigned char lds[2 * kChunkBytes];
    __shared__ float wave_sum[4];
    const int tid = threadIdx.x, lane = tid & 63;
    const int wave = __builtin_amdgcn_readfirstlane(tid >> 6);
    const int l31 = lane & 31, g = lane >> 5;
    const int nb = gridDim.x, xcd = blockIdx.x & 7, slot = blockIdx.x >> 3;
    const int q8 = nb >> 3, r8 = nb & 7;
    const int L = (xcd < r8 ? xcd * (q8 + 1) : r8 * (q8 + 1) + (xcd - r8) * q8) + slot;
    const int mt = __builtin_amdgcn_readfirstlane(L % m_tiles), pt = __builtin_amdgcn_readfirstlane(L / m_tiles);
    const int m0 = mt * kSM;
    const int px0 = pt * kSN + wave * 64;

    constexpr unsigned kOob = 0x80000000u;
    const __amdgpu_buffer_rsrc_t rf =
        __builtin_amdgcn_make_buffer_rsrc(const_cast<float *>(F), 0, BIG ? 0 : f_bytes, 0x00020000);
    const __amdgpu_buffer_rsrc_t rs = __builtin_amdgcn_make_buffer_rsrc(S, 0, BIG ? 0 : f_bytes, 0x00020000);
    unsigned voff[2];
#pragma unroll
    for (int j = 0; j < 2; ++j) {
        const int px = px0 + j * 32 + l31;
        voff[j] = px < HW ? (unsigned)((g * 8) * HW + px) * 4u : kOob;
    }
    const unsigned HW4 = (unsigned)HW * 4u;
    const int n_steps = Cp / 16, n_chunks = Cp / kSK;

    const unsigned short *dsrc[kDLoads];
    unsigned ddst[kDLoads];
#pragma unroll
    for (int n = 0; n < kDLoads; ++n) {
        const int e = tid + 256 * n;
        const int pc = e / (kSM * kSegs), rem = e - pc * (kSM * kSegs);
        const int row = rem / kSegs, seg = rem - row * kSegs;
        dsrc[n] = Dp + ((size_t)pc * Cp + (m0 + row)) * Cp + seg * 8;
        ddst[n] = (unsigned)(pc * kPieceBytes + row * kRowBytes + seg * 16);
    }
    u32x4y dreg[kDLoads];
    auto d_load = [&](int chunk) {
#pragma unroll
        for (int n = 0; n < kDLoads; ++n) dreg[n] = *reinterpret_cast<const u32x4y *>(dsrc[n] + chunk * kSK);
    };
    auto d_store = [&](int buf) {
#pragma unroll
        for (int n = 0; n < kDLoads; ++n) *reinterpret_cast<u32x4y *>(lds + buf * kChunkBytes + ddst[n]) = dreg[n];
    };

    float raw[kRing][2][8];
    auto f_load = [&](int step, int slot_) {
        const int k0 = __builtin_amdgcn_readfirstlane(step * 16);
        const int left = C - k0 < 16 ? C - k0 : 16;
        const __amdgpu_buffer_rsrc_t rk =
            BIG ? __builtin_amdgcn_make_buffer_rsrc(const_cast<float *>(F) + (size_t)k0 * (size_t)HW, 0,
                                                    (left > 0 ? left : 0) * HW * 4, 0x00020000)
                : rf;
#pragma unroll
        for (int j = 0; j < 2; ++j)
#pragma unroll
            for (int e = 0; e < 8; ++e)
                raw[slot_][j][e] = __builtin_bit_cast(
                    float, __builtin_amdgcn_raw_buffer_load_b32(
                               rk, voff[j], BIG ? (unsigned)e * HW4 : (unsigned)min(k0 + e, C) * HW4, 0));
    };

    f32x16b acc[2][2];
#pragma unroll
    for (int i = 0; i < 2; ++i)
#pragma unroll
        for (int j = 0; j < 2; ++j)
#pragma unroll
            for (int r = 0; r < 16; ++r) acc[i][j][r] = 0.f;
// ... 12 lines not shown
#pragma unroll
        for (int j = 0; j < 2; ++j) {
            if (STX_SYMM_SKIP & 2) {
                typedef float f32x4s __attribute__((ext_vector_type(4)));
                const float *x = raw[slot_][j];
                pb[j][0] = __builtin_bit_cast(bf16x8, (f32x4s){x[0], x[1], x[2], x[3]});
                pb[j][1] = __builtin_bit_cast(bf16x8, (f32x4s){x[4], x[5], x[6], x[7]});
                pb[j][2] = pb[j][0];
            } else {
                split3_bf16(raw[slot_][j], pb[j][0], pb[j][1], pb[j][2]);
            }
        }
        const unsigned char *base = lds + buf * kChunkBytes + a_off + s_in_chunk * 32;
#pragma unroll
        for (int i = 0; i < 2; ++i)
#pragma unroll
            for (int n = 0; n < 3; ++n)
                pa[i][n] = *reinterpret_cast<const bf16x8 *>(base + n * kPieceBytes + i * 32 * kRowBytes);
#pragma unroll
        for (int i = 0; i < 2; ++i)
#pragma unroll
            for (int j = 0; j < 2; ++j) {
                if (STX_SYMM_SKIP & 1) {
#pragma unroll
                    for (int q = 0; q < 3; ++q) acc[i][j][q] += (float)(pa[i][q][0] + pb[j][q][1]);
                    continue;
                }
                acc[i][j] = mfma_split6(pa[i], pb[j], acc[i][j]);
            }
    };

    int step = 0;
    auto advance = [&](int slot_) {
        const int chunk = step / kSPC, s_in = step % kSPC, buf = chunk & 1;
        if (step + kRing - 1 < n_steps && !(STX_SYMM_SKIP & 4)) f_load(step + kRing - 1, (slot_ + kRing - 1) % kRing);
        do_step(step, slot_, buf, s_in);
        if (s_in == kSPC - 1) {
            if (chunk + 1 < n_chunks) d_store(buf ^ 1);
            if (chunk + 2 < n_chunks) d_load(chunk + 2);
            __syncthreads();
        }
        ++step;
    };
    while (step < n_steps) {
#pragma unroll
        for (int r = 0; r < kRing; ++r)
            if (step < n_steps) advance(r);
    }

    float asum = 0.f;
#pragma unroll
    for (int i = 0; i < 2; ++i)
#pragma unroll
        for (int r = 0; r < 16; ++r) {
            const int row = m0 + i * 32 + (r & 3) + 8 * (r >> 2) + 4 * g;
            const int row0 = min(__builtin_amdgcn_readfirstlane(m0 + i * 32 + (r & 3) + 8 * (r >> 2)), C);
            const unsigned so = BIG ? 0u : (unsigned)row0 * HW4;
            const int rows_left = C - row0 < 5 ? C - row0 : 5;
            const __amdgpu_buffer_rsrc_t rrow =
                BIG ? __builtin_amdgcn_make_buffer_rsrc(S + (size_t)row0 * (size_t)HW, 0,
                                                        (rows_left > 0 ? rows_left : 0) * HW * 4, 0x00020000)
                    : rs;
#pragma unroll
            for (int j = 0; j < 2; ++j) {
                const int px = px0 + j * 32 + l31;
                const bool ok = row < C && px < HW;
                const float v = acc[i][j][r];
                asum += ok ? fabsf(v) : 0.f;
                const unsigned vo = ok ? (unsigned)((4 * g) * HW + px) * 4u : kOob;
                if (!(STX_SYMM_SKIP & 8))
                    __builtin_amdgcn_raw_buffer_store_b32(__builtin_bit_cast(unsigned, v), rrow, vo, so, 0);
            }
        }
#pragma unroll
    for (int off = 32; off > 0; off >>= 1) asum += __shfl_down(asum, off, 64);
    if (lane == 0) wave_sum[wave] = asum;
    __syncthreads();
    if (tid == 0) partials[blockIdx.x] = ((wave_sum[0] + wave_sum[1]) + wave_sum[2]) + wave_sum[3];
}

constexpr int kHChunkBytes = 2 * kPieceBytes;
constexpr int kHDLoads = kSM * kSK / 4 / 256;

template <bool BIG>
__global__ __launch_bounds__(256, 2) void symm_h2_kernel(const float *__restrict__ F,
                                                         const float *__restrict__ D,
                                                         const unsigned *__restrict__ d_amax, int n_damax,
                                                         const unsigned *__restrict__ f_amax,
                                                         float *__restrict__ S,
                                                         float *__restrict__ partials, int C, int Cp,
                                                         int HW, unsigned f_bytes, int m_tiles) {
    __shared__ __attribute__((aligned(16))) unsigned char lds[2 * kHChunkBytes];
    __shared__ float wave_sum[4];
    __shared__ unsigned wave_max[4];
    const int tid = threadIdx.x, lane = tid & 63;
    const int wave = __builtin_amdgcn_readfirstlane(tid >> 6);
    const int l31 = lane & 31, g = lane >> 5;
    const int nb = gridDim.x, xcd = blockIdx.x & 7, slot = blockIdx.x >> 3;
    const int q8 = nb >> 3, r8 = nb & 7;
    const int L = (xcd < r8 ? xcd * (q8 + 1) : r8 * (q8 + 1) + (xcd - r8) * q8) + slot;
    const int mt = __builtin_amdgcn_readfirstlane(L % m_tiles), pt = __builtin_amdgcn_readfirstlane(L / m_tiles);
    const int m0 = mt * kSM;
    const int px0 = pt * kSN + wave * 64;

    constexpr unsigned kOob = 0x80000000u;
    const __amdgpu_buffer_rsrc_t rf =
        __builtin_amdgcn_make_buffer_rsrc(const_cast<float *>(F), 0, BIG ? 0 : f_bytes, 0x00020000);
    const __amdgpu_buffer_rsrc_t rs = __builtin_amdgcn_make_buffer_rsrc(S, 0, BIG ? 0 : f_bytes, 0x00020000);
    const __amdgpu_buffer_rsrc_t rd =
        __builtin_amdgcn_make_buffer_rsrc(const_cast<float *>(D), 0, (unsigned)(C * C) * 4u, 0x00020000);
    unsigned voff[2];
#pragma unroll
    for (int j = 0; j < 2; ++j) {
        const int px = px0 + j * 32 + l31;
        voff[j] = px < HW ? (unsigned)((g * 8) * HW + px) * 4u : kOob;
    }
    const unsigned HW4 = (unsigned)HW * 4u;
    const int n_steps = Cp / 16, n_chunks = Cp / kSK;

    unsigned dvoff[kHDLoads], ddst[kHDLoads];
    int dcol[kHDLoads];
#pragma unroll
    for (int n = 0; n < kHDLoads; ++n) {
        const int e = tid + 256 * n;
        const int row = e / (kSK / 4), seg = e - row * (kSK / 4);
        dcol[n] = seg * 4;
        dvoff[n] = m0 + row < C ? (unsigned)((m0 + row) * C + seg * 4) * 4u : kOob;
        ddst[n] = (unsigned)(row * kRowBytes + seg * 8);
    }
    u32x4y dreg[kHDLoads];
    auto d_load = [&](int chunk) {
        const unsigned so = (unsigned)__builtin_amdgcn_readfirstlane(chunk * kSK * 4);
#pragma unroll
        for (int n = 0; n < kHDLoads; ++n)
            dreg[n] = __builtin_amdgcn_raw_buffer_load_b128(rd, dcol[n] + chunk * kSK < C ? dvoff[n] : kOob, so, 0);
    };

    float raw[kRing][2][8];
    auto f_load = [&](int step, int slot_) {
        const int k0 = __builtin_amdgcn_readfirstlane(step * 16);
        const int left = C - k0 < 16 ? C - k0 : 16;
        const __amdgpu_buffer_rsrc_t rk =
            BIG ? __builtin_amdgcn_make_buffer_rsrc(const_cast<float *>(F) + (size_t)k0 * (size_t)HW, 0,
                                                    (left > 0 ? left : 0) * HW * 4, 0x00020000)
                : rf;
#pragma unroll
        for (int j = 0; j < 2; ++j)
#pragma unroll
            for (int e = 0; e < 8; ++e)
                raw[slot_][j][e] = __builtin_bit_cast(
                    float, __builtin_amdgcn_raw_buffer_load_b32(
                               rk, voff[j], BIG ? (unsigned)e * HW4 : (unsigned)min(k0 + e, C) * HW4, 0));
    };

    f32x16h acc[2][2];
#pragma unroll
    for (int i = 0; i < 2; ++i)
#pragma unroll
        for (int j = 0; j < 2; ++j)
#pragma unroll
            for (int r = 0; r < 16; ++r) acc[i][j][r] = 0.f;

    d_load(0);
#pragma unroll
    for (int r = 0; r < kRing - 1; ++r)
        if (r < n_steps) f_load(r, r);

    const int ef = h2_scale_exp(amax_of_slots(f_amax, kAmaxSlots));
    unsigned dm = 0;
    for (int i = tid; i < n_damax; i += 256) dm = max(dm, d_amax[i]);
#pragma unroll
    for (int off = 32; off > 0; off >>= 1) dm = max(dm, (unsigned)__shfl_xor((int)dm, off, 64));
    if (lane == 0) wave_max[wave] = dm;
    __syncthreads();
    dm = max(max(wave_max[0], wave_max[1]), max(wave_max[2], wave_max[3]));
    const int ed = __builtin_amdgcn_readfirstlane(h2_scale_exp(dm));
    const float sf = pow2f(ef), sd = pow2f(ed);

    auto d_store = [&](int buf) {
#pragma unroll
        for (int n = 0; n < kHDLoads; ++n) {
            unsigned h[2], l[2];
            const unsigned d0 = dreg[n].x, d1 = dreg[n].y, d2 = dreg[n].z, d3 = dreg[n].w;
            split2_f16_quad(__builtin_bit_cast(float, d0), __builtin_bit_cast(float, d1),
                            __builtin_bit_cast(float, d2), __builtin_bit_cast(float, d3), sd, h, l);
            typedef unsigned u32x2s __attribute__((ext_vector_type(2)));
            unsigned char *q = lds + buf * kHChunkBytes + ddst[n];
            *reinterpret_cast<u32x2s *>(q) = (u32x2s){h[0], h[1]};
            *reinterpret_cast<u32x2s *>(q + kPieceBytes) = (u32x2s){l[0], l[1]};
        }
    };
    d_store(0);
    if (n_chunks > 1) d_load(1);
    __syncthreads();

    const unsigned a_off = (unsigned)(l31 * kRowBytes + g * 16);
    auto do_step = [&](int slot_, int buf, int s_in_chunk) {
        f16x8h bh[2], bl[2], ah[2], al[2];
#pragma unroll
        for (int j = 0; j < 2; ++j) split2_f16(raw[slot_][j], sf, bh[j], bl[j]);
        const unsigned char *base = lds + buf * kHChunkBytes + a_off + s_in_chunk * 32;
#pragma unroll
        for (int i = 0; i < 2; ++i) {
            ah[i] = *reinterpret_cast<const f16x8h *>(base + i * 32 * kRowBytes);
            al[i] = *reinterpret_cast<const f16x8h *>(base + kPieceBytes + i * 32 * kRowBytes);
        }
#pragma unroll
        for (int i = 0; i < 2; ++i)
#pragma unroll
            for (int j = 0; j < 2; ++j) acc[i][j] = mfma_split3(ah[i], al[i], bh[j], bl[j], acc[i][j]);
    };

    int step = 0;
    auto advance = [&](int slot_) {
        const int chunk = step / kSPC, s_in = step % kSPC, buf = chunk & 1;
        if (step + kRing - 1 < n_steps) f_load(step + kRing - 1, (slot_ + kRing - 1) % kRing);
        do_step(slot_, buf, s_in);
        if (s_in == kSPC - 1) {
            if (chunk + 1 < n_chunks) d_store(buf ^ 1);
            if (chunk + 2 < n_chunks) d_load(chunk + 2);
            __syncthreads();
        }
        ++step;
    };
    while (step < n_steps) {
#pragma unroll
        for (int r = 0; r < kRing; ++r)
            if (step < n_steps) advance(r);
    }

    const float ud = pow2f(-ed), uf = pow2f(-ef);
    float asum = 0.f;
#pragma unroll
    for (int i = 0; i < 2; ++i)
#pragma unroll
        for (int r = 0; r < 16; ++r) {
            const int row = m0 + i * 32 + (r & 3) + 8 * (r >> 2) + 4 * g;
            const int row0 = min(__builtin_amdgcn_readfirstlane(m0 + i * 32 + (r & 3) + 8 * (r >> 2)), C);
            const unsigned so = BIG ? 0u : (unsigned)row0 * HW4;
            const int rows_left = C - row0 < 5 ? C - row0 : 5;
            const __amdgpu_buffer_rsrc_t rrow =
                BIG ? __builtin_amdgcn_make_buffer_rsrc(S + (size_t)row0 * (size_t)HW, 0,
                                                        (rows_left > 0 ? rows_left : 0) * HW * 4, 0x00020000)
                    : rs;
#pragma unroll
            for (int j = 0; j < 2; ++j) {
                const int px = px0 + j * 32 + l31;
                const bool ok = row < C && px < HW;
                const float v = (acc[i][j][r] * ud) * uf;
                asum += ok ? fabsf(v) : 0.f;
                const unsigned vo = ok ? (unsigned)((4 * g) * HW + px) * 4u : kOob;
                __builtin_amdgcn_raw_buffer_store_b32(__builtin_bit_cast(unsigned, v), rrow, vo, so, 0);
            }
        }
#pragma unroll
    for (int off = 32; off > 0; off >>= 1) asum += __shfl_down(asum, off, 64);
    if (lane == 0) wave_sum[wave] = asum;
    __syncthreads();
    if (tid == 0) partials[blockIdx.x] = ((wave_sum[0] + wave_sum[1]) + wave_sum[2]) + wave_sum[3];
}

__global__ void symm_split_kernel(const float *__restrict__ dsym, int C, int Cp,
                                  unsigned short *__restrict__ pieces) {
    const int idx = blockIdx.x * blockDim.x + threadIdx.x;
    if (idx >= Cp * Cp) return;
    const int i = idx / Cp, j = idx - i * Cp;
    unsigned short s1 = 0, s2 = 0, s3 = 0;
    if (i < C && j < C) split3_bf16_scalar(dsym[i * C + j], s1, s2, s3);
    pieces[idx] = s1;
    pieces[(size_t)Cp * Cp + idx] = s2;
    pieces[2 * (size_t)Cp * Cp + idx] = s3;
}

int symm_num_workgroups(int C, int HW) { return ceil_div(C, kSM) * ceil_div(HW, kSN); }

bool symm_bf3_usable(const float *feat, const float *out, int C, int HW) {
    const char *env = sw_env("STX_SYMM");
    if (env && !strcmp(env, "fp32")) return false;
    return 64.0 * (double)HW < 2147483648.0 &&
           ((reinterpret_cast<uintptr_t>(feat) | reinterpret_cast<uintptr_t>(out)) & 3) == 0;
}

int symm_bf3_launch(hipStream_t s, const float *feat, const float *dsym, unsigned short *pieces,
                    bool pieces_ready, float *out, float *partials, int C, int HW) {
    const int Cp = ceil_div(C, kSM) * kSM;
    if (!pieces_ready || Cp != C) {
        symm_split_kernel<<<ceil_div(Cp * Cp, 256), 256, 0, s>>>(dsym, C, Cp, pieces);
        STX_CHECK_LAUNCH();
    }
    const int m_tiles = Cp / kSM;
    const double bytes = 4.0 * C * (double)HW;
    const char *force_big = sw_env("STX_WINO_BIG");
    if (bytes >= 2147483648.0 || (force_big && atoi(force_big) == 1))
        symm_bf3_kernel<true><<<symm_num_workgroups(C, HW), 256, 0, s>>>(feat, pieces, out, partials, C, Cp,
                                                                       HW, 0u, m_tiles);
    else
        symm_bf3_kernel<false><<<symm_num_workgroups(C, HW), 256, 0, s>>>(feat, pieces, out, partials, C, Cp,
                                                                        HW, (unsigned)bytes, m_tiles);
    STX_CHECK_LAUNCH();
    return STX_OK;
}

bool symm_h2_usable(const float *feat, const float *out, int C, int HW) {
    const char *env = sw_env("STX_SYMM");
    if (env && (!strcmp(env, "fp32") || !strcmp(env, "bf3"))) return false;
    return C % 4 == 0 && symm_bf3_usable(feat, out, C, HW);
}

int symm_h2_launch(hipStream_t s, const float *feat, const float *dsym, const unsigned *d_amax, int n_damax,
                   const unsigned *f_amax, float *out, float *partials, int C, int HW) {
    const int Cp = ceil_div(C, kSM) * kSM;
    const int m_tiles = Cp / kSM;
    const double bytes = 4.0 * C * (double)HW;
    const char *force_big = sw_env("STX_WINO_BIG");
    if (bytes >= 2147483648.0 || (force_big && atoi(force_big) == 1))
        symm_h2_kernel<true><<<symm_num_workgroups(C, HW), 256, 0, s>>>(feat, dsym, d_amax, n_damax, f_amax, out,
                                                                      partials, C, Cp, HW, 0u, m_tiles);
    else
        symm_h2_kernel<false><<<symm_num_workgroups(C, HW), 256, 0, s>>>(feat, dsym, d_amax, n_damax, f_amax, out,
                                                                       partials, C, Cp, HW, (unsigned)bytes, m_tiles);
    STX_CHECK_LAUNCH();
    return STX_OK;
}

}
```

### style_transfer_amd/csrc/tile_path.cpp

```cpp

#include <algorithm>
#include <cmath>
#include <cstdlib>

#include "engine.h"

namespace stx {

ConvProblem conv_fwd_problem(const float *x, float *y, const float *bias, int Cin, int Cout, int H, int W,
                             int ks, int relu) {
    ConvProblem p{};
    p.x = x;
    p.y = y;
    p.bias = bias;
    p.K = Cin;
    p.M = Cout;
    p.H = H;
    p.W = W;
    p.ksize = ks;
    p.relu = relu;
    p.epilogue = kEpiForward;
    return p;
}

// ... 95 lines not shown
    ConvProblem p = problem;
    e->last_mark = -1;
    if (e->clock_marks && conv_takes_clock(cfg) && e->marks_used < kMaxClockMarks) {
        e->last_mark = e->marks_used++;
        p.clock_out = static_cast<long long *>(e->marks_buf.ptr) + 2 * (size_t)e->last_mark;
    }
    int var = 0;
    p.variant_out = &var;
    const int rc = conv_dispatch(e->stream, cfg, p, &e->flop_algorithmic, &e->flop_issued);
    if (var) {
        ++e->n_inject_specialised;
        e->inject_variants |= 1u << var;
    }
    return rc;
}

static int amax_for(stx_engine *e, int blob, bool diff, const std::string &consumer, const unsigned **out) {
    Blob &b = e->blobs[blob];
    int &src = diff ? b.amax_diff : b.amax_data;
    if (src < 0) {
        ProfScope scope(e, std::string("absmax ") + b.name, 0.0);
        STX_TRY(absmax_launch(e->stream, diff ? b.diff.f() : b.data.f(), b.count(), e->amax_slots(blob, diff)));
        src = blob;
    } else if (e->amax_audit) {
        STX_TRY(amax_audit_note(e, e->stream, consumer, b.name, diff, e->amax_slots(src, diff),
                                diff ? b.diff.f() : b.data.f(), b.count()));
    }
    *out = e->amax_slots(src, diff);
    return STX_OK;
}

int amax_audit_note(stx_engine *e, hipStream_t stream, const std::string &consumer, const std::string &blob,
                    bool diff, const unsigned *slots, const float *x, size_t n) {
    if (!e->amax_audit) return STX_OK;
    if (e->audit.size() >= kMaxAmaxAudit) {
        set_error("stx_amax_audit: more than %zu hand-offs since the last stx_amax_audit_read", kMaxAmaxAudit);
        return STX_ERR_STATE;
    }
    const size_t group = (size_t)(slots - static_cast<const unsigned *>(e->amax.ptr)) / kAmaxSlots;
    const size_t nb = e->blobs.size();
    const std::string source = group < 2 * nb ? e->blobs[group % nb].name : "(scratch)";
    unsigned *const rec = static_cast<unsigned *>(e->audit_buf.ptr) + 2 * e->audit.size() * kAmaxSlots;
    STX_HIP(hipMemcpyAsync(rec, slots, kAmaxSlots * sizeof(unsigned), hipMemcpyDeviceToDevice, stream));
    STX_TRY(absmax_launch(stream, x, n, rec + kAmaxSlots));
    e->audit.push_back(stx_engine::AuditEntry{consumer, blob, source, diff});
    return STX_OK;
}

int amax_scratch(stx_engine *e, unsigned **out) {
    STX_TRY(e->amax_ensure());
    *out = e->amax_slots((int)e->blobs.size(), true);
    return STX_OK;
}

struct FwdConvPlan {
    bool force_relu;
    const Layer *pool;
    int pool_li;
    bool top_unobserved;
    bool conv_reader;
    bool relu_codes;
};

static FwdConvPlan plan_fwd_conv(const stx_engine *e, size_t li, const std::vector<char> &needed, int relu_blob,
                                 bool relu_codes, const std::vector<char> &observed) {
    const Layer &L = e->layers[li];
    FwdConvPlan plan{L.top_blob == relu_blob, nullptr, -1, false, false, relu_codes};
    int readers = 0;
    for (size_t lj = li + 1; lj < e->layers.size(); ++lj) {
        const Layer &P = e->layers[lj];
        if (P.type == STX_LAYER_RELU || P.bottom_blob != L.top_blob) continue;
        ++readers;
        plan.conv_reader |= P.type == STX_LAYER_CONV && needed[P.top_blob];
        if (!plan.pool && P.type == STX_LAYER_POOL && needed[P.top_blob] && P.ksize == 2 && P.stride == 2 &&
            P.pad == 0 && !e->blobs[P.top_blob].relu && P.top_blob != relu_blob) {
            plan.pool = &P;
            plan.pool_li = (int)lj;
        }
    }
    plan.top_unobserved = plan.pool && !observed[L.top_blob] && L.top_blob != relu_blob && readers == 1;
    return plan;
}

static int run_conv_forward(stx_engine *e, int li, const FwdConvPlan &plan, bool *pooled) {
    const Layer &L = e->layers[li];
    const Layer *const pool = plan.pool;
    Blob &b = e->blobs[L.bottom_blob];
    Blob &t = e->blobs[L.top_blob];
    const ConvParams &cp = e->sh->conv[li];
    ConvProblem p = conv_fwd_problem(b.data.f(), t.data.f(), cp.b.f(), cp.cin, cp.cout, b.h, b.w, cp.ks,
                                     (t.relu || plan.force_relu) ? 1 : 0);
    const double direct = conv_flops(cp.cin, cp.cout, b.h, b.w, cp.ks);
    *pooled = false;
    if (conv_first_usable(cp.cin, cp.cout, cp.ks) && !pool) {
        b.relu_codes_valid = false;
        b.relu_codes_wanted = false;
        t.relu_codes_valid = false;
        unsigned *y_amax = nullptr;
        t.amax_data = -1;
        if (conv_h2_enabled()) {
            y_amax = e->amax_slots(L.top_blob, false);
            t.amax_data = L.top_blob;
        }
        float *gram = nullptr;
        if (L.top_blob == e->first_gram_blob) {
            const int parts = conv_first_workgroups(b.h, b.w);
            STX_TRY(e->first_gram.ensure(((size_t)parts * 64 * 64 + 64 * 64 / 64 + 64) * sizeof(float)));
            gram = e->first_gram.f();
            e->first_gram_parts = parts;
            e->first_gram_valid = true;
        }
        ProfScope scope(e, "fwd " + L.name, direct);
        e->flop_algorithmic += direct;
        e->flop_issued += direct;
        return conv_first_launch(e->stream, p.x, cp.w.f(), cp.b.f(), p.y, cp.cin, b.h, b.w, p.relu, gram, y_amax);
    }
    ConvConfig cfg;
    STX_TRY(choose_conv(e, li, 0, p, &cfg));
    b.relu_codes_wanted = !conv_reads_x_amax(cfg) && !b.relu_codes_valid && plan.relu_codes && b.relu && b.channels <= 128;
    p.wants_codes = b.relu_codes_wanted;
    t.amax_data = -1;
    if (conv_reads_x_amax(cfg)) STX_TRY(amax_for(e, L.bottom_blob, false, "fwd " + L.name, &p.x_amax));
    if (conv_leaves_y_amax(cfg)) {
        p.y_amax = e->amax_slots(L.top_blob, false);
        t.amax_data = L.top_blob;
    }
    STX_TRY(get_packed(e, li, 0, cfg, &p.w));
    STX_TRY(attach_splitk(e, cfg, p));
    if (b.relu_codes_wanted) {
        const size_t bytes = (size_t)b.channels * ((b.h + 1) / 2) * ((b.w + 1) / 2);
        STX_TRY(b.relu_codes.ensure(bytes));
        p.in_codes = static_cast<unsigned char *>(b.relu_codes.ptr);
        b.relu_codes_valid = conv_uses_relu_codes(cfg, p, conv_splitk_factor(cfg, p));
        if (!b.relu_codes_valid) p.in_codes = nullptr;
    }
    if (pool) {
        Blob &pt = e->blobs[pool->top_blob];
        p.pool_out = pt.data.f();
        p.pool_mode = pool->pool_mode;
        pt.codes_valid = false;
        pt.amax_data = -1;
        if (conv_fuses_pool(cfg, p)) {
            *pooled = true;
            pt.amax_data = t.amax_data;
            if (conv_writes_pool_codes(cfg) && e->pool_codes) {
                STX_TRY(pt.codes.ensure(pt.count() + 4));
                p.pool_codes = static_cast<unsigned char *>(pt.codes.ptr);
                pt.codes_valid = true;
                p.skip_y = plan.top_unobserved;
            }
        } else {
            p.pool_out = nullptr;
        }
    }
    t.relu_codes_valid = false;
    if (plan.relu_codes && t.relu && plan.conv_reader && conv_h2_enabled()) {
        const size_t bytes = (size_t)t.channels * ((t.h + 1) / 2) * ((t.w + 1) / 2);
        STX_TRY(t.relu_codes.ensure(bytes));
        p.out_codes = static_cast<unsigned char *>(t.relu_codes.ptr);
        t.relu_codes_valid = conv_writes_out_codes(cfg, p, conv_splitk_factor(cfg, p));
        if (!t.relu_codes_valid) p.out_codes = nullptr;
    }
    ProfScope scope(e, "fwd " + L.name, direct);
    return launch_conv(e, cfg, p);
}

static ConvProblem conv_backward_shape(stx_engine *e, int li) {
    const Layer &L = e->layers[li];
    const Blob &b = e->blobs[L.bottom_blob];
    const ConvParams &cp = e->sh->conv[li];
    return conv_bwd_problem(nullptr, nullptr, nullptr, cp.cout, cp.cin, b.h, b.w, cp.ks);
}

static bool conv_backward_takes_pooled(stx_engine *e, int li) {
    const char *env = sw_env("STX_POOL_BWD_FUSE");
    if (env && atoi(env) == 0) return false;
    const ConvProblem p = conv_backward_shape(e, li);
    ConvConfig cfg;
    return p.ksize == 3 && p.M > 4 && conv_choose(p, e->winograd, nullptr, &cfg) == STX_OK &&
           conv_takes_pooled_input(cfg, p);
}

static bool conv_backward_reads_amax(stx_engine *e, int li) {
    const ConvProblem p = conv_backward_shape(e, li);
    ConvConfig cfg;
    return !(p.ksize == 3 && p.M <= 4) && conv_choose(p, e->winograd, nullptr, &cfg) == STX_OK && conv_reads_x_amax(cfg);
}

static int run_conv_backward(stx_engine *e, int li, const ConvInject *inj, bool *fused, const Layer *pooled) {
    const Layer &L = e->layers[li];
    Blob &b = e->blobs[L.bottom_blob];
    const Blob &t = e->blobs[L.top_blob];
    const ConvParams &cp = e->sh->conv[li];
    ConvProblem p = conv_backward_shape(e, li);
    p.x = t.diff.f();
    p.y = b.diff.f();
    p.mask = b.relu ? b.data.f() : nullptr;
    p.mask_codes = b.relu && b.relu_codes_valid ? static_cast<const unsigned char *>(b.relu_codes.ptr) : nullptr;
    p.wants_codes = b.relu && b.relu_codes_wanted;
    if (cp.ks == 3 && cp.cin <= 4) {
        if (fused) *fused = false;
        const float *packed = nullptr;
        STX_TRY(get_bank(e, li, conv_small_bank(cp.cout, cp.cin), &packed));
        const double direct = conv_flops(cp.cout, cp.cin, b.h, b.w, cp.ks);
        ProfScope scope(e, "bwd " + L.name, direct);
        e->flop_algorithmic += direct;
        e->flop_issued += direct * 4.0 / p.M;
        return conv_small_launch(e->stream, p.x, packed, p.y, p.mask, p.K, p.M, p.H, p.W);
    }
    ConvConfig cfg;
    STX_TRY(choose_conv(e, li, 1, p, &cfg));
    const bool can_fuse = inj && conv_takes_inject(cfg);
    if (fused) *fused = can_fuse;
    if (can_fuse) p.inject = *inj;
    b.amax_diff = -1;
    if (pooled) {
        const Blob &pt = e->blobs[pooled->top_blob];
        if (!conv_takes_pooled_input(cfg, p) || !pt.codes_valid) {
            set_error("run_conv_backward: %s cannot take the gradient of %s pooled", L.name.c_str(), pt.name.c_str());
            return STX_ERR_UNSUPPORTED;
        }
        p.x = pt.diff.f();
        p.pin_codes = static_cast<const unsigned char *>(pt.codes.ptr);
        p.pin_mode = pooled->pool_mode;
        p.pin_mask = t.relu;
        STX_TRY(amax_for(e, pooled->top_blob, true, "bwd " + L.name, &p.x_amax));
    } else if (conv_reads_x_amax(cfg)) {
        STX_TRY(amax_for(e, L.top_blob, true, "bwd " + L.name, &p.x_amax));
    }
    if (conv_leaves_y_amax(cfg)) {
        p.y_amax = e->amax_slots(L.bottom_blob, true);
        b.amax_diff = L.bottom_blob;
    }
    STX_TRY(get_packed(e, li, 1, cfg, &p.w));
    STX_TRY(attach_splitk(e, cfg, p));
    ProfScope scope(e, "bwd " + L.name, conv_flops(cp.cout, cp.cin, b.h, b.w, cp.ks));
    return launch_conv(e, cfg, p);
}

static int begin_timing(stx_engine *e) {
    e->ev_cur = (e->ev_cur + 1) % stx_engine::kTimed;
    STX_HIP(hipEventRecord(e->ev_start[e->ev_cur], e->stream));
    e->flop_algorithmic = e->flop_issued = 0;
    return STX_OK;
}

static int end_timing(stx_engine *e) {
    STX_HIP(hipEventRecord(e->ev_stop[e->ev_cur], e->stream));
    if (e->ev_recorded < stx_engine::kTimed) ++e->ev_recorded;
    e->timed = true;
    return STX_OK;
}

static int sc_grad_prepare(stx_engine *e, const TileCall &c, TilePlan &plan) {
    std::vector<Tap> &order = plan.order;
    const stx_tap *taps = c.taps;
    const int n_taps = c.n_taps;
    const auto tapped = [&](int blob) {
        return std::any_of(order.begin(), order.end(), [=](const Tap &o) { return o.blob == blob; });
    };
    const auto has_statistics = [&](int blob) {
        return std::any_of(e->sh->stats.begin(), e->sh->stats.end(), [=](const StatTarget &t) { return t.blob == blob; }) ||
               std::any_of(e->sh->nnfms.begin(), e->sh->nnfms.end(), [=](const NnfmTarget &t) { return t.blob == blob; }) ||
               std::any_of(e->sh->swds.begin(), e->sh->swds.end(), [=](const SwdTarget &t) { return t.blob == blob; }) ||
               std::any_of(e->sh->selfsims.begin(), e->sh->selfsims.end(),
                           [=](const SelfsimTarget &t) { return t.blob == blob; }) ||
               std::any_of(e->sh->shifts.begin(), e->sh->shifts.end(), [=](const ShiftTarget &t) { return t.blob == blob; });
    };
    for (int i = 0; i < n_taps; ++i) {
        const int blob = e->find_blob(taps[i].layer);
        if (blob <= 0) {
            set_error("stx_sc_grad_tile: unknown tap layer '%s'",
                      taps[i].layer ? taps[i].layer : "(null)");
            return STX_ERR_ARG;
        }
        if (tapped(blob)) {
            set_error("stx_sc_grad_tile: layer '%s' is tapped twice", taps[i].layer);
            return STX_ERR_ARG;
        }
        if (!taps[i].is_content && !taps[i].is_style && !taps[i].is_dd && !has_statistics(blob)) continue;
        order.push_back(Tap{blob, &taps[i]});
    }
    for (const StatTarget &st : e->sh->stats) {
        if (tapped(st.blob)) continue;
        stx_tap t{};
        t.layer_weight = 1.0;
        plan.extra.push_back(t);
        order.push_back(Tap{st.blob, &plan.extra.back()});
    }
    for (const NnfmTarget &nt : e->sh->nnfms) {
        if (tapped(nt.blob)) continue;
        stx_tap t{};
        t.layer_weight = 1.0;
        plan.extra.push_back(t);
        order.push_back(Tap{nt.blob, &plan.extra.back()});
    }
    for (const SwdTarget &wt : e->sh->swds) {
        if (tapped(wt.blob)) continue;
        stx_tap t{};
        t.layer_weight = 1.0;
        plan.extra.push_back(t);
        order.push_back(Tap{wt.blob, &plan.extra.back()});
    }
    for (const SelfsimTarget &ft : e->sh->selfsims) {
        if (tapped(ft.blob)) continue;
        stx_tap t{};
        t.layer_weight = 1.0;
        plan.extra.push_back(t);
        order.push_back(Tap{ft.blob, &plan.extra.back()});
    }
    for (const ShiftTarget &ht : e->sh->shifts) {
        if (tapped(ht.blob)) continue;
        stx_tap t{};
        t.layer_weight = 1.0;
        plan.extra.push_back(t);
        order.push_back(Tap{ht.blob, &plan.extra.back()});
    }
    if (order.empty()) {
        set_error("stx_sc_grad_tile: no content, style or Deep-Dream layer");
        return STX_ERR_ARG;
    }
    std::sort(order.begin(), order.end(), [](const Tap &a, const Tap &b) { return a.blob > b.blob; });
    std::vector<char> &needed = plan.needed;
    needed.assign(e->blobs.size(), 0);
    mark_ancestors(e, order[0].blob, needed);
    std::vector<int> &tap_of = plan.tap_of;
    tap_of.assign(e->blobs.size(), -1);
    for (size_t i = 0; i < order.size(); ++i) {
        if (!needed[order[i].blob]) {
            set_error("stx_sc_grad_tile: tapped layers must lie on one path through the network "
                      "('%s' does not feed '%s')", e->blobs[order[i].blob].name.c_str(),
                      e->blobs[order[0].blob].name.c_str());
            return STX_ERR_UNSUPPORTED;
        }
        tap_of[order[i].blob] = (int)i;
    }
    for (const Tap &tp : order) {
        if (tp.t->is_content && e->sh->n_contents == 0) {
            set_error("stx_sc_grad_tile: no content targets set");
            return STX_ERR_STATE;
        }
        if (tp.t->is_style && e->sh->n_styles == 0) {
            set_error("stx_sc_grad_tile: no style targets set");
            return STX_ERR_STATE;
        }
    }
    STX_TRY(shape_blobs(e, c.th, c.tw, needed, true));
    plan.sums_late = !(sw_env("STX_SUMS_LATE") && !atoi(sw_env("STX_SUMS_LATE")));
    plan.interleave = !(sw_env("STX_TERMS_LATE") && atoi(sw_env("STX_TERMS_LATE")));
    return plan_terms(e, c, plan);
}

static int blob_done(TileRun *run, int blob) {
    const int k = run ? run->plan.tap_of[blob] : -1;
    return k >= 0 ? queue_tap_terms(*run, (size_t)k) : STX_OK;
}

static int forward(stx_engine *e, const std::vector<char> &needed, int relu_blob, TileRun *run,
                   bool relu_codes, const std::vector<char> &observed) {
    int pooled_layer = -1;
    STX_TRY(e->amax_ensure());
    STX_HIP(hipMemsetAsync(e->amax_slots(0, false), 0, 2 * e->blobs.size() * kAmaxSlots * sizeof(unsigned), e->stream));
    for (Blob &b : e->blobs) {
        b.amax_data = -1;
        b.relu_codes_valid = false;
    }
    for (size_t li = 1; li < e->layers.size(); ++li) {
        const Layer &L = e->layers[li];
        if (L.type == STX_LAYER_RELU || !needed[L.top_blob]) continue;
        const Blob &b = e->blobs[L.bottom_blob];
        Blob &t = e->blobs[L.top_blob];
        if (L.type == STX_LAYER_CONV) {
            const FwdConvPlan plan = plan_fwd_conv(e, li, needed, relu_blob, relu_codes, observed);
            bool pooled = false;
            STX_TRY(run_conv_forward(e, (int)li, plan, &pooled));
            if (pooled) pooled_layer = plan.pool_li;
            STX_TRY(blob_done(run, L.top_blob));
            if (pooled) STX_TRY(blob_done(run, plan.pool->top_blob));
        } else if ((int)li == pooled_layer) {
            continue;
        } else {
            {
                ProfScope scope(e, "fwd " + L.name, 0.0);
                unsigned char *codes = nullptr;
                t.codes_valid = false;
                if (e->pool_codes) {
                    STX_TRY(t.codes.ensure(t.count() + 4));
                    codes = static_cast<unsigned char *>(t.codes.ptr);
                    t.codes_valid = true;
                }
                STX_TRY(pool_forward_launch(e->stream, b.data.f(), b.channels, b.h, b.w, L.pool_mode,
                                            t.data.f(), codes));
                t.amax_data = b.amax_data;
                if (t.relu || L.top_blob == relu_blob)
                    STX_TRY(relu_inplace_launch(e->stream, t.data.f(), t.count()));
            }
            STX_TRY(blob_done(run, L.top_blob));
        }
    }
    return STX_OK;
}

static int backward_walk(TileRun &run) {
    stx_engine *e = run.e;
    const int data_blob = e->layers[0].top_blob;
    int cur = run.plan.order[0].blob;
    for (Blob &b : e->blobs) b.amax_diff = -1;
    {
        bool written = false;
        STX_TRY(inject_terms(run, 0, written));
        if (!written)
            STX_HIP(hipMemsetAsync(e->blobs[cur].diff.ptr, 0, e->blobs[cur].count() * sizeof(float),
                                   e->stream));
    }
    const Layer *pooled = nullptr;
    while (cur != data_blob) {
        const int li = e->blobs[cur].producer;
        const Layer &L = e->layers[li];
        Blob &bot = e->blobs[L.bottom_blob];
        const Blob &top = e->blobs[cur];
        const int k = run.plan.tap_of[L.bottom_blob];
        bool fused = false;
        if (L.type == STX_LAYER_POOL && top.codes_valid && k < 0 && L.ksize == 2 && L.stride == 2 && L.pad == 0 &&
            e->layers[bot.producer].type == STX_LAYER_CONV && conv_backward_takes_pooled(e, bot.producer)) {
            pooled = &L;
            cur = L.bottom_blob;
            continue;
        }
        if (L.type == STX_LAYER_CONV) {
            ConvInject inj{};
            if (k >= 0 && tap_fusable(run, (size_t)k)) {
                inj = make_inject(run, (size_t)k, bot);
                fused = true;
            }
            STX_TRY(run_conv_backward(e, li, fused ? &inj : nullptr, &fused, pooled));
            pooled = nullptr;
        } else {
            if (top.amax_diff < 0 && e->layers[bot.producer].type == STX_LAYER_CONV &&
                conv_backward_reads_amax(e, bot.producer)) {
                const unsigned *unused;
                STX_TRY(amax_for(e, cur, true, "bwd " + L.name, &unused));
            }
            ProfScope scope(e, "bwd " + L.name, 0.0);
            if (top.codes_valid)
                STX_TRY(pool_backward_codes_launch(
                    e->stream, top.diff.f(), static_cast<const unsigned char *>(top.codes.ptr),
                    bot.channels, bot.h, bot.w, L.pool_mode, bot.relu, bot.diff.f()));
            else
// ... 362 lines not shown
```

### style_transfer_amd/csrc/tile_terms.cpp

```cpp

#include <algorithm>
#include <cmath>
#include <cstring>

#include "engine.h"

namespace stx {

static size_t style_term_scratch_floats(int C, int HW) {
    return 2 * (size_t)ceil_div(C * C, 64) + (size_t)symm_num_workgroups(C, HW) + 64;
}

int launch_style_terms(stx_engine *e, hipStream_t stream, const float *feat, int C, int h, int w,
                       const float *target, float *sgrad, float *sc, const std::string &name,
                       const unsigned *f_amax, float *term_scratch, std::vector<SumJob> *defer) {
    const int HW = h * w;
    const bool fused = e->first_gram_valid && e->first_gram_blob >= 0 &&
                       feat == e->blobs[e->first_gram_blob].data.f() && C == 64;
    GramPlan plan = gram_plan(C, HW);
    if (fused) {
        plan.splits = e->first_gram_parts;
        plan.tiles = 1;
        plan.parts = 1;
        plan.partial_floats = (size_t)plan.splits * 64 * 64;
    }
    const int fin_blocks = gram_finish_blocks(plan);
    float *const partials = fused ? e->first_gram.f() : nullptr;
    if (!fused) STX_TRY(e->gram_partials.ensure((plan.partial_floats + 2 * fin_blocks) * sizeof(float)));
    STX_TRY(e->dsym.ensure((size_t)C * C * sizeof(float)));
    const bool gram_h2 = !fused && gram_h2_usable(feat, C, HW);
    const bool symm_h2 = symm_h2_usable(feat, sgrad, C, HW);
    const bool bf3 = !symm_h2 && symm_bf3_usable(feat, sgrad, C, HW);
    if ((gram_h2 || symm_h2) && !f_amax) {
        unsigned *scratch;
        STX_TRY(amax_scratch(e, &scratch));
        ProfScope scope(e, "absmax " + name, 0.0, stream);
        STX_TRY(absmax_launch(stream, feat, (size_t)C * HW, scratch));
        f_amax = scratch;
    } else if ((gram_h2 || symm_h2) && e->amax_audit) {
        STX_TRY(amax_audit_note(e, stream, (feat == e->masked_feat.f() ? "masked style " : "style ") + name, name,
                                false, f_amax, feat, (size_t)C * HW));
    }
    if (bf3) STX_TRY(e->dsym_pieces.ensure(symm_pieces_elems(C) * sizeof(unsigned short)));
    unsigned short *pieces = bf3 && C % 64 == 0 ? static_cast<unsigned short *>(e->dsym_pieces.ptr) : nullptr;
    {
        ProfScope scope(e, "gram " + name, 2.0 * C * C * (double)HW, stream);
        if (!fused) STX_TRY(gram_partials_launch(stream, feat, plan, e->gram_partials.f(), gram_h2 ? f_amax : nullptr));
        STX_TRY(gram_finish_launch(stream, fused ? partials : e->gram_partials.f(), plan, nullptr, target,
                                   e->dsym.f(), nullptr, pieces, gram_h2 ? f_amax : nullptr,
                                   defer ? term_scratch : nullptr));
    }
    ProfScope scope(e, "symm " + name, 2.0 * C * C * (double)HW, stream);
    const float *block_sumsq = defer ? term_scratch : (fused ? partials : e->gram_partials.f()) + plan.partial_floats;
    auto finish = [&](float *symm_partials, int n_wg) -> int {
        if (!defer) return sum_partials2_launch(stream, block_sumsq, fin_blocks, sc, symm_partials, n_wg, sc + 1);
        defer->push_back(SumJob{block_sumsq, fin_blocks, sc});
        defer->push_back(SumJob{symm_partials, n_wg, sc + 1});
        return STX_OK;
    };
    if (symm_h2 || bf3) {
        const int n_wg = symm_num_workgroups(C, HW);
        float *symm_partials = defer ? term_scratch + 2 * fin_blocks : nullptr;
        if (!defer) {
            STX_TRY(e->symm_partials.ensure((size_t)n_wg * sizeof(float)));
            symm_partials = e->symm_partials.f();
        }
        if (symm_h2)
            STX_TRY(symm_h2_launch(stream, feat, e->dsym.f(), reinterpret_cast<const unsigned *>(block_sumsq + fin_blocks),
                                   fin_blocks, f_amax, sgrad, symm_partials, C, HW));
        else
            STX_TRY(symm_bf3_launch(stream, feat, e->dsym.f(), static_cast<unsigned short *>(e->dsym_pieces.ptr),
                                    pieces != nullptr, sgrad, symm_partials, C, HW));
        return finish(symm_partials, n_wg);
    }
    const ConvConfig cfg = conv_pick_config(1, C, C, h, w);
    const int n_wg = conv_num_workgroups(cfg, C, h, w);
    STX_TRY(e->symm_partials.ensure((size_t)n_wg * sizeof(float)));
    ConvProblem p{};
    p.x = feat;
    p.w = e->dsym.f();
    p.y = sgrad;
    p.partials = e->symm_partials.f();
    p.K = C;
    p.M = C;
    p.H = h;
    p.W = w;
    p.ksize = 1;
    p.epilogue = kEpiSymm;
    STX_TRY(conv_launch(stream, cfg, p, false));
    return sum_partials2_launch(stream, block_sumsq, fin_blocks, sc, e->symm_partials.f(), n_wg, sc + 1);
}

int launch_masked_style_terms(stx_engine *e, hipStream_t stream, const float *feat, int C, int h, int w,
                              const float *mask_map, const ContentWindow &win, const float *target,
                              float *sgrad, float *sc, const std::string &name, const unsigned *f_amax,
                              float *term_scratch, float *mask_scratch, std::vector<SumJob> *defer) {
    STX_TRY(e->masked_feat.ensure((size_t)C * h * w * sizeof(float)));
    STX_TRY(e->masked_target.ensure((size_t)C * C * sizeof(float)));
    float *const m2_partials = mask_scratch, *const ms_partials = mask_scratch + kMaskParts;
    {
        ProfScope scope(e, "mask " + name, 0.0, stream);
        int n_m2 = 0;
        STX_TRY(mask_apply_launch(stream, feat, mask_map, win, e->masked_feat.f(), m2_partials, &n_m2));
        STX_TRY(mask_target_launch(stream, target, C, m2_partials, n_m2, h * w, e->masked_target.f(), sc + 3));
    }
    STX_TRY(launch_style_terms(e, stream, e->masked_feat.f(), C, h, w, e->masked_target.f(), sgrad, sc, name,
                               f_amax, term_scratch, defer));
    ProfScope scope(e, "smask " + name, 0.0, stream);
    int n_ms = 0;
    STX_TRY(mask_sgrad_launch(stream, sgrad, mask_map, win, sc + 3, ms_partials, &n_ms));
    if (!defer) return sum_partials_launch(stream, ms_partials, n_ms, sc + 2);
    defer->push_back(SumJob{ms_partials, n_ms, sc + 2});
    return STX_OK;
}

int launch_stat_terms(stx_engine *e, hipStream_t stream, const float *feat, int C, int h, int w, const float *MU,
                      const float *SD, float *sgrad, float *sc, const std::string &name, float *stat_scratch,
                      std::vector<SumJob> *defer) {
    const int HW = h * w;
    float *const partials = stat_scratch;
    float *const table = partials + 4 * (size_t)C * stat_slices(HW);
    float *const abs_partials = table + 4 * (size_t)C;
    ProfScope scope(e, "stat " + name, 0.0, stream);
    STX_TRY(stat_partials_launch(stream, feat, C, HW, partials));
    STX_TRY(stat_finish_launch(stream, partials, C, HW, MU, SD, table, sc, nullptr, nullptr));
    int n_parts = 0;
    STX_TRY(stat_grad_launch(stream, feat, C, HW, table, sgrad, abs_partials, &n_parts));
    if (!defer) return sum_partials_launch(stream, abs_partials, n_parts, sc + 1);
    defer->push_back(SumJob{abs_partials, n_parts, sc + 1});
    return STX_OK;
}

int launch_nnfm_terms(stx_engine *e, hipStream_t stream, const float *feat, int C, int h, int w, int patch,
                      const float *bank, const unsigned short *pieces, int rows, float *sgrad, int *idx_out, float *sc,
                      const std::string &name, float *scratch, std::vector<SumJob> *defer, int k, float cover,
                      int *winner_out, float *e_cov_out) {
    const int n = h * w;
    const bool covered = cover != 0.f;
    if (covered && patch != 1) {
        set_error("launch_nnfm_terms: the coverage part with patch %d", patch);
        return STX_ERR_ARG;
    }
    const NnfmScratch x = nnfm_carve(scratch, C, n, rows, patch, k, covered);
    const NnfmPlan plan = nnfm_plan(n, rows);
    int *const idx = idx_out ? idx_out : x.idx;
    const std::string tag = std::string(patch == 3 ? "nnfm patch " : "nnfm ") + (k > 1 ? "k" + std::to_string(k) + " " : "");
    {
        ProfScope scope(e, tag + "prepare " + name, 0.0, stream);
        STX_TRY(nnfm_prepare_launch(stream, feat, C, h, w, patch, 1, x.work, x.inv_r, x.xhi, x.xlo, nullptr));
    }
    {
        ProfScope scope(e, tag + "search " + name + " x" + std::to_string(plan.slices),
                        6.0 * n * (double)rows * C * (patch * patch), stream);
// ... 279 lines not shown
                set_error("no style target for layer %s", b.name.c_str());
                return STX_ERR_STATE;
            }
            if (b.channels % 4 != 0) {
                set_error("style layer %s: channel count %d is not a multiple of 4", b.name.c_str(), b.channels);
                return STX_ERR_UNSUPPORTED;
            }
            const size_t late = plan.sums_late ? style_term_scratch_floats(b.channels, b.h * b.w) : 0;
            for (const StyleTarget &st : sh.styles) {
                if (st.blob != tp.blob) continue;
                const double coef = lw * tp.t->style_weight / sh.n_styles;
                if (const StyleMask *mk = style_mask_of(e, st.index, tp.blob)) {
                    const ContentWindow win = content_window(b, mk->h, mk->w, c.start, c.rx, c.ry);
                    STX_TRY(check_window(win, "style mask", b));
                    add(TermKind::MaskedStyle, st.gram->f(), mk->map->f(), win, coef, 4, late + kMaskScratchFloats,
                        style_slot);
                } else {
                    add(TermKind::Style, st.gram->f(), nullptr, ContentWindow{}, coef, 2, late, style_slot);
                }
                style_slot += b.count();
            }
        }
        size_t nnfm_slot = align(content_slot);
        if (const StatTarget *st = stat_target_of(e, tp.blob)) {
            add(TermKind::Stat, st->ms->f(), nullptr, ContentWindow{}, lw * st->weight, 2,
                stat_scratch_floats(b.channels, b.h * b.w), align(content_slot));
            nnfm_slot = align(nnfm_slot + b.count());
        }
        if (const NnfmTarget *nt = nnfm_target_of(e, tp.blob)) {
            if (nt->segs.count) {
                const ContentWindow win = content_window(b, nt->mh, nt->mw, c.start, c.rx, c.ry);
                STX_TRY(check_window(win, "NNFM mask", b));
                add(TermKind::NnfmGuided, nt->bank->f(), nt->maps->f(), win, lw * nt->weight, 3,
                    nnfm_guided_scratch_floats(b.channels, b.h * b.w, nt->segs, nt->k), nnfm_slot);
            } else {
                add(TermKind::Nnfm, nt->bank->f(), nullptr, ContentWindow{}, lw * nt->weight, 2,
                    nnfm_scratch_floats(b.channels, b.h * b.w, nt->rows, nt->patch, nt->k, nt->cover != 0.f), nnfm_slot);
            }
            plan.terms.back().nnfm = nt;
        }
        if (const SwdTarget *wt = swd_target_of(e, tp.blob)) {
            STX_TRY(swd_check(("sliced Wasserstein target of layer " + b.name).c_str(), b.channels,
                              (long long)b.h * b.w, wt->D, wt->Q));
            const size_t swd_slot = nnfm_target_of(e, tp.blob) ? align(nnfm_slot + b.count()) : nnfm_slot;
            add(TermKind::Swd, wt->Tq(), nullptr, ContentWindow{}, lw * wt->weight, 2,
                swd_scratch_floats(b.channels, b.h * b.w, wt->D), swd_slot);
            plan.terms.back().swd = wt;
        }
        if (const SelfsimTarget *ft = selfsim_target_of(e, tp.blob)) {
            STX_TRY(selfsim_check(("self-similarity target of layer " + b.name).c_str(), b.channels, ft->points));
            const ContentTarget *map = nullptr;
            for (const ContentTarget &ct : sh.contents)
                if (ct.blob == tp.blob && ct.index == 0 && !map) map = &ct;
            if (!map) {
                set_error("self-similarity target of layer %s: no content map of content_index 0 there", b.name.c_str());
                return STX_ERR_STATE;
            }
            const ContentWindow win = content_window(b, map->h, map->w, c.start, c.rx, c.ry);
            STX_TRY(check_window(win, "content", b));
            size_t slot = nnfm_target_of(e, tp.blob) ? align(nnfm_slot + b.count()) : nnfm_slot;
            if (swd_target_of(e, tp.blob)) slot = align(slot + b.count());
            add(TermKind::Selfsim, map->feat->f(), nullptr, win, lw * ft->weight, 2,
                selfsim_scratch_floats(b.channels, selfsim_grid(b.h, b.w, ft->points).N), slot);
            plan.terms.back().points = ft->points;
        }
        if (const ShiftTarget *ht = shift_target_of(e, tp.blob)) {
            STX_TRY(shift_check_map(("shifted-Gram target of layer " + b.name).c_str(), b.channels, b.h, b.w, ht->off));
            size_t slot = nnfm_target_of(e, tp.blob) ? align(nnfm_slot + b.count()) : nnfm_slot;
            if (swd_target_of(e, tp.blob)) slot = align(slot + b.count());
            if (selfsim_target_of(e, tp.blob)) slot = align(slot + b.count());
            add(TermKind::Shift, ht->grams->f(), nullptr, ContentWindow{}, lw * ht->weight, 2,
                shift_scratch_floats(b.channels, b.h * b.w, ht->off.n), slot);
            plan.terms.back().shift = ht;
        }
        if (tp.t->is_dd)
            add(TermKind::Dream, nullptr, nullptr, dream_window(b), -lw * tp.t->dd_weight, kResidualScalars, 0, kNoSlot);
    }
    return STX_OK;
}

int queue_tap_terms(TileRun &run, size_t k) {
    stx_engine *e = run.e;
    const TilePlan &plan = run.plan;
    const Blob &b = e->blobs[plan.order[k].blob];
    for (size_t i = plan.first_term[k]; i < plan.terms.size() && plan.terms[i].tap == (int)k; ++i) {
        const PlannedTerm &t = plan.terms[i];
        size_t si;
        STX_TRY(alloc_scalars(e, t.scalars, &si));
        float *const sc = e->A().scalars.f() + si;
        float *const scratch = e->term_scratch.f() + t.scratch_off;
        float *const late = plan.sums_late ? scratch : nullptr;
        float *const sgrad = t.sgrad_off == kNoSlot ? nullptr : e->sgrad[k]->f() + t.sgrad_off;
        const unsigned *f_amax = b.amax_data >= 0 ? e->amax_slots(b.amax_data, false) : nullptr;
        const float *abs_sum = sc + 1;
        switch (t.kind) {
        case TermKind::Content:
        case TermKind::Dream: {
            ProfScope scope(e, (t.kind == TermKind::Dream ? "dream " : "content ") + b.name, 0.0, e->stream);
            STX_TRY(content_sums_launch(e->stream, b.data.f(), t.target, t.win, sc, run.defer()));
            break;
        }
        case TermKind::MaskedContent:
            STX_TRY(launch_masked_content_terms(e, e->stream, b.data.f(), t.target, t.mask, t.win, sgrad, sc, b.name,
                                                scratch, run.defer()));
            break;
        case TermKind::Style:
            STX_TRY(launch_style_terms(e, e->stream, b.data.f(), b.channels, b.h, b.w, t.target, sgrad, sc, b.name,
                                       f_amax, late, run.defer()));
            break;
        case TermKind::MaskedStyle:
            STX_TRY(launch_masked_style_terms(e, e->stream, b.data.f(), b.channels, b.h, b.w, t.mask, t.win, t.target,
                                              sgrad, sc, b.name, f_amax, late,
                                              scratch + t.scratch_len - kMaskScratchFloats, run.defer()));
            abs_sum = sc + 2;
            break;
        case TermKind::Stat:
            STX_TRY(launch_stat_terms(e, e->stream, b.data.f(), b.channels, b.h, b.w, t.target, t.target + b.channels,
                                      sgrad, sc, b.name, scratch, run.defer()));
            break;
        case TermKind::Nnfm:
            STX_TRY(launch_nnfm_terms(e, e->stream, b.data.f(), b.channels, b.h, b.w, t.nnfm->patch, t.target,
                                      t.nnfm->pieces_hi_lo(), t.nnfm->rows, sgrad, nullptr, sc, b.name, scratch,
                                      run.defer(), t.nnfm->k, t.nnfm->cover));
            break;
        case TermKind::NnfmGuided:
            STX_TRY(launch_nnfm_guided_terms(e, e->stream, b.data.f(), b.channels, b.h, b.w, t.target,
                                             t.nnfm->pieces_hi_lo(), t.nnfm->segs, t.mask, t.win, sgrad, nullptr, sc,
                                             b.name, scratch, run.defer(), t.nnfm->k, true));
            break;
        case TermKind::Swd:
            STX_TRY(launch_swd_terms(e, e->stream, b.data.f(), b.channels, b.h, b.w, t.swd->V(), t.swd->D, t.target,
                                     t.swd->Q, sgrad, nullptr, sc, b.name, scratch, run.defer()));
            break;
        case TermKind::Selfsim:
            STX_TRY(launch_selfsim_terms(e, e->stream, b.data.f(),
                                         SelfsimSource{t.target, t.win.ch, t.win.cw, t.win.oy - t.win.sy,
                                                       t.win.ox - t.win.sx},
                                         b.channels, b.h, b.w, t.points, sgrad, nullptr, sc, b.name, scratch,
                                         run.defer()));
            break;
        case TermKind::Shift:
            STX_TRY(launch_shift_terms(e, e->stream, b.data.f(), b.channels, b.h, b.w, t.shift->off, t.target, sgrad, sc,
                                       b.name, scratch, run.defer()));
            break;
        }
        run.pl.terms.push_back(LossTerm{si, t.coef * 0.5});
        run.terms[k].push_back(sgrad ? Term{Term::Gradient, sgrad, abs_sum, (float)t.coef, ContentWindow{}}
                                     : Term{Term::Residual, t.target, sc, (float)t.coef, t.win});
    }
    return STX_OK;
}

int inject_terms(TileRun &run, size_t k, bool &diff_written) {
    stx_engine *e = run.e;
    const int blob = run.plan.order[k].blob;
    const std::vector<Term> &terms = run.terms[k];
    Blob &b = e->blobs[blob];
    ProfScope scope(e, "inject " + b.name, 0.0);
    b.amax_diff = -1;
    for (size_t ti = 0; ti < terms.size(); ++ti) {
        const Term &t = terms[ti];
        unsigned *amax = nullptr;
        if (ti + 1 == terms.size() && conv_h2_enabled()) {
            amax = e->amax_slots(blob, true);
            b.amax_diff = blob;
        }
        if (t.kind == Term::Gradient)
            STX_TRY(inject_style_launch(e->stream, b.diff.f(), t.src, b.count(), t.sums, t.coef,
                                        diff_written, amax));
        else
            STX_TRY(inject_content_launch(e->stream, b.diff.f(), b.data.f(), t.src, t.win,
                                          t.sums, t.coef, diff_written, amax));
        diff_written = true;
    }
    return STX_OK;
}

bool tap_fusable(const TileRun &run, size_t k) {
    int ns = 0, nc = 0;
    for (const Term &t : run.terms[k]) {
        if (t.kind == Term::Residual && !t.src) return false;
        (t.kind == Term::Gradient ? ns : nc)++;
    }
    return ns <= 1 && nc <= 1;
}

ConvInject make_inject(const TileRun &run, size_t k, const Blob &bot) {
    ConvInject inj{};
    for (const Term &t : run.terms[k]) {
        if (t.kind == Term::Gradient) {
            inj.sgrad = t.src;
// ... 15 lines not shown
```

### style_transfer_amd/lib.py

```python

import ctypes
import os

_HERE = os.path.dirname(os.path.abspath(__file__))
LIB_PATH = os.environ.get('STX_LIB') or os.path.join(_HERE, 'csrc', 'libstx.so')

HOST, DEVICE = 0, 1
LAYER_INPUT, LAYER_CONV, LAYER_RELU, LAYER_POOL = 0, 1, 2, 3
POOL_MAX, POOL_AVE = 0, 1
(Q_SHARED_ENGINES, Q_TARGET_UPLOADS, Q_TARGET_BYTES, Q_WEIGHT_BYTES, Q_TILE_EVALS,
 Q_PEERS_WITHOUT_ACCESS, Q_TILE_IO_DIRECT, Q_INJECT_SPECIALISED, Q_INJECT_VARIANTS) = range(9)

c_float_p = ctypes.POINTER(ctypes.c_float)
c_double_p = ctypes.POINTER(ctypes.c_double)
c_int_p = ctypes.POINTER(ctypes.c_int)


class StxError(RuntimeError):

    def __init__(self, func, code, message):
        super().__init__('%s failed with status %d: %s' % (func, code, message))
        self.code = code


# ... 82 lines not shown

_vp, _i, _sz, _d = ctypes.c_void_p, ctypes.c_int, ctypes.c_size_t, ctypes.c_double
SIGNATURES = {
    'stx_reread_env': [],
    'stx_device_count': [c_int_p],
    'stx_device_name': [_i, ctypes.c_char_p, _sz],
    'stx_engine_create': [_i, ctypes.POINTER(LayerDesc), _i, ctypes.POINTER(_vp)],
    'stx_engine_create_shared': [_vp, ctypes.POINTER(_vp)],
    'stx_engine_wait': [_vp, _vp],
    'stx_engine_query': [_vp, _i, c_double_p],
    'stx_set_conv_weights': [_vp, ctypes.c_char_p, _vp, _vp, _i],
    'stx_sync': [_vp],
    'stx_fence': [_vp, ctypes.POINTER(ctypes.c_ulonglong)],
    'stx_fence_wait': [_vp, ctypes.c_ulonglong],
    'stx_engine_device': [_vp, c_int_p],
    'stx_engine_stream': [_vp, ctypes.POINTER(_vp)],
    'stx_malloc': [_vp, _sz, ctypes.POINTER(_vp)],
    'stx_free': [_vp, _vp],
    'stx_memset_async': [_vp, _vp, _i, _sz],
    'stx_memcpy_async': [_vp, _vp, _i, _vp, _i, _sz],
    'stx_set_contents_and_styles': [_vp, ctypes.POINTER(ContentTarget), _i,
                                    ctypes.POINTER(StyleTarget), _i],
    'stx_set_style_masks': [_vp, ctypes.POINTER(StyleMask), _i],
    'stx_set_stat_targets': [_vp, ctypes.POINTER(StatTarget), _i],
    'stx_set_nnfm_targets': [_vp, ctypes.POINTER(NnfmTarget), _i],
    'stx_set_nnfm_patch_targets': [_vp, ctypes.POINTER(NnfmPatchTarget), _i],
    'stx_set_nnfm_knn_targets': [_vp, ctypes.POINTER(NnfmKnnTarget), _i],
    'stx_set_nnfm_cover_targets': [_vp, ctypes.POINTER(NnfmCoverTarget), _i],
    'stx_set_nnfm_guided_targets': [_vp, ctypes.POINTER(NnfmGuidedTarget), _i, ctypes.POINTER(ctypes.c_void_p), _i, _i,
                                    _i, _i],
    'stx_set_swd_targets': [_vp, ctypes.POINTER(SwdTarget), _i],
    'stx_set_selfsim_targets': [_vp, ctypes.POINTER(SelfsimTarget), _i],
    'stx_set_shift_targets': [_vp, ctypes.POINTER(ShiftTarget), _i],
    'stx_set_content_mask': [_vp, _vp, _i, _i, _i],
    'stx_features_tile': [_vp, _vp, _i, _i, _i, ctypes.POINTER(ctypes.c_char_p), _i,
                          ctypes.POINTER(_vp), _i],
    'stx_sc_grad_tile': [_vp, _vp, _i, _i, _i, c_int_p, c_int_p, ctypes.POINTER(Tap), _i,
                         c_double_p, _vp, _i, _i],
    'stx_tile_buffers': [_vp, _i, _i, ctypes.POINTER(_vp), ctypes.POINTER(_vp)],
    'stx_gram_matrix': [_vp, _vp, _i, _i, _i, _vp, _i],
    'stx_feature_stats': [_vp, _vp, _i, _i, _i, _vp, _vp, _i],
    'stx_swd_target': [_vp, _vp, _i, _i, _i, _i, _vp, _i, _i, _vp],
    'stx_shift_gram': [_vp, _vp, _i, _i, _i, _i, ctypes.POINTER(ctypes.c_int), _i, _vp],
    'stx_nnfm_bank': [_vp, _vp, _i, _i, _i, _i, _i, _vp, _i],
    'stx_nnfm_patch_bank': [_vp, _vp, _i, _i, _i, _i, _i, _i, _vp, _i],
    'stx_image_cut_tile': [_vp, _vp, _i, _i, c_int_p, _i, _i, _i, _i, _vp],
    'stx_image_put_tile': [_vp, _vp, _i, _i, c_int_p, _i, _i, _i, _i, _vp],
    'stx_image_mask_map': [_vp, _vp, _i, _i, _i, _vp],
    'stx_map_place': [_vp, _vp, _i, _i, _i, _i, _i, _vp, _i, _i],
    'stx_map_roll_add': [_vp, _vp, _vp, _i, _i, _i, c_int_p, _d, _d],
    'stx_image_resample': [_vp, _vp, _i, _i, _i, _vp, _i, _i, c_int_p, c_double_p, _i, c_int_p,
                           c_double_p, _i, _i],
    'stx_image_regularizers': [_vp, _vp, _vp, _i, _i, c_float_p, _d, _d, _d, _d, _vp, _d,
                               c_int_p, c_double_p],
    'stx_image_swt_haar': [_vp, _vp, _vp, _i, _i, c_int_p, _d, _d, c_double_p],
    'stx_image_swt_haar_levels': [_vp, _vp, _vp, _i, _i, _i, c_int_p, _d, _d, c_double_p],
    'stx_image_swt_daub_levels': [_vp, _vp, _vp, _i, _i, _i, _i, c_int_p, _d, _d, c_double_p],
    'stx_image_lap_target': [_vp, _vp, _i, _i, _i, c_int_p, _vp],
    'stx_image_lap': [_vp, _vp, _vp, _i, _i, _i, c_int_p, c_double_p, _vp, _d, c_double_p],
    'stx_image_photo': [_vp, _vp, _vp, _vp, _i, _i, _d, _d, c_double_p],
    'stx_adam_step': [_vp, _vp, _vp, _vp, _vp, _vp, _vp, _sz, _d, _d, _d, _d, _d, _d, _d],
    'stx_vec_dot': [_vp, _vp, _vp, _sz, c_double_p],
    'stx_vec_axpy': [_vp, _d, _vp, _vp, _sz],
    'stx_vec_scale': [_vp, _d, _vp, _sz],
    'stx_vec_mean_abs': [_vp, _vp, _sz, c_double_p],
    'stx_vec_dot_async': [_vp, _vp, _vp, _sz, _vp],
    'stx_vec_abs_sum_async': [_vp, _vp, _sz, _vp],
    'stx_vec_axpy_dev': [_vp, _d, _vp, _d, _d, _vp, _d, _vp, _vp, _sz],
    'stx_vec_scale_dev': [_vp, _d, _vp, _d, _vp, _sz],
    'stx_vec_axpy_dot_dev': [_vp, _d, _vp, _d, _d, _vp, _d, _d, _vp, _d, _vp, _vp, _vp, _vp, _sz, _vp],
    'stx_vec_lbfgs_pair': [_vp, _vp, _vp, _vp, _vp, _sz, _vp, c_double_p],
    'stx_vec_scale2_axpy': [_vp, _d, _d, _vp, _vp, _sz],
    'stx_image_step_stats': [_vp, _vp, _vp, _i, _i, c_double_p],
    'stx_image_step_stats_async': [_vp, _vp, _vp, _i, _i, c_double_p],
    'stx_image_to_u8': [_vp, _vp, _i, _i, c_float_p, _vp],
    'stx_image_to_u8_luma': [_vp, _vp, _vp, _i, _i, c_float_p, _vp],
    'stx_image_color_stats': [_vp, _vp, _i, _i, c_double_p],
    'stx_image_color_affine': [_vp, _vp, _vp, _i, _i, c_double_p, c_double_p, c_float_p],
    'stx_op_conv_forward': [_vp, _vp, _i, _i, _i, _vp, _vp, _i, _i, _i, _vp],
    'stx_op_conv_backward_data': [_vp, _vp, _i, _i, _i, _vp, _i, _i, _vp, _vp],
    'stx_op_pool_forward': [_vp, _vp, _i, _i, _i, _i, _vp],
    'stx_op_pool_backward': [_vp, _vp, _vp, _i, _i, _i, _i, _vp, _vp],
    'stx_op_style_terms': [_vp, _vp, _i, _i, _i, _vp, _vp, _vp, c_double_p, c_double_p],
    'stx_op_masked_style_terms': [_vp, _vp, _i, _i, _i, _vp, _i, _i, _i, _i, c_int_p, _vp, _vp, c_double_p],
    'stx_op_masked_content_terms': [_vp, _vp, _i, _i, _i, _vp, _i, _i, _vp, _i, _i, c_int_p, _vp, c_double_p],
    'stx_op_stat_terms': [_vp, _vp, _i, _i, _i, _vp, _vp, _vp, c_double_p],
    'stx_op_swd_terms': [_vp, _vp, _i, _i, _i, _vp, _i, _vp, _i, _vp, _vp, c_double_p],
    'stx_op_selfsim_terms': [_vp, _vp, _vp, _i, _i, _i, _i, _vp, c_double_p, _vp],
    'stx_op_shift_terms': [_vp, _vp, _i, _i, _i, ctypes.POINTER(ctypes.c_int), _i, _vp, _vp, c_double_p],
    'stx_op_nnfm_terms': [_vp, _vp, _i, _i, _i, _vp, _i, _vp, _vp, c_double_p],
    'stx_op_nnfm_patch_terms': [_vp, _vp, _i, _i, _i, _i, _vp, _i, _vp, _vp, c_double_p],
    'stx_op_nnfm_knn_terms': [_vp, _vp, _i, _i, _i, _i, _i, _vp, _i, _vp, _vp, c_double_p],
    'stx_op_nnfm_cover_terms': [_vp, _vp, _i, _i, _i, _i, _i, ctypes.c_float, _vp, _i, _vp, _vp, _vp, c_double_p],
    'stx_op_nnfm_guided_terms': [_vp, _vp, _i, _i, _i, _i, _vp, ctypes.POINTER(ctypes.c_int), _i, _vp, _i, _i, _i, _i,
                                 ctypes.POINTER(ctypes.c_int), _vp, _vp, c_double_p],
    'stx_op_content_terms': [_vp, _vp, _i, _i, _i, _vp, _i, _i, _i, _i, c_int_p, _vp, c_double_p],
    'stx_last_tile_ms': [_vp, c_float_p],
    'stx_last_tile_flops': [_vp, c_double_p, c_double_p],
    'stx_clock_marks': [_vp, ctypes.c_int],
    'stx_clock_marks_read': [_vp, c_double_p, ctypes.c_int, ctypes.POINTER(ctypes.c_int)],
    'stx_profile_enable': [_vp, _i],
    'stx_profile_read': [_vp, ctypes.c_char_p, _sz, ctypes.POINTER(_sz)],
    'stx_amax_audit': [_vp, _i],
    'stx_amax_audit_read': [_vp, ctypes.c_char_p, _sz, ctypes.POINTER(_sz)],
}
NON_STATUS = {'stx_version': (ctypes.c_char_p, []), 'stx_last_error': (ctypes.c_char_p, []),
              'stx_engine_destroy': (None, [_vp]),
              'stx_image_lap_floats': (_sz, [_i, _i, _i, c_int_p])}

_lib = None


def load():
    global _lib
    if _lib is not None:
        return _lib
    if not os.path.exists(LIB_PATH):
        raise ImportError('%s is missing: build the HIP extension first '
                          '(python -m style_transfer_amd.build)' % LIB_PATH)
    lib = ctypes.CDLL(LIB_PATH, mode=ctypes.RTLD_GLOBAL)
    for name, argtypes in SIGNATURES.items():
        fn = getattr(lib, name)
        fn.argtypes, fn.restype = argtypes, ctypes.c_int
    for name, (restype, argtypes) in NON_STATUS.items():
        fn = getattr(lib, name)
        fn.argtypes, fn.restype = argtypes, restype
    _lib = lib
    return lib


def call(name, *args):
    lib = load()
    rc = getattr(lib, name)(*args)
    if rc != 0:
        raise StxError(name, rc, lib.stx_last_error().decode('utf-8', 'replace'))


def reread_env():
    if _lib is not None:
        call('stx_reread_env')


def device_count():
    n = ctypes.c_int(0)
    call('stx_device_count', ctypes.byref(n))
    return n.value


def device_name(device):
    buf = ctypes.create_string_buffer(256)
    call('stx_device_name', device, buf, 256)
    return buf.value.decode()


def version():
    return load().stx_version().decode()
```

Baseline: 283.4.

## Emit ReLU sign-bit plane from Gram kernel and mask dgrad with it

The style-term symmetric Gram kernel now ballots feature signs while it streams the features and stores a 1-bit-per-element ReLU mask plane. The backward conv's injecting epilogue then gets a new variant that reads this bit plane instead of reloading the full fp32 activation blob to build the ReLU mask. This cuts dgrad mask traffic by a large factor for style layers that have no relu codes. In exchange the Gram kernel does extra ballots, writelanes and stores, and there are more kernel instantiations. A debug API to read the plane back is also added.

```diff
diff --git a/include/stx.h b/include/stx.h
--- a/include/stx.h
+++ b/include/stx.h
@@ -331,6 +331,7 @@
 int stx_op_style_terms(stx_engine *e, const float *feat, int channels, int h, int w,
                        const float *gram_target, float *s_out, float *normalized_out,
                        double *half_sumsq, double *abs_sum);
+int stx_op_blob_sign_bits(stx_engine *e, const char *layer, unsigned *words_out, size_t n_words, int *valid);
 int stx_op_masked_style_terms(stx_engine *e, const float *feat, int channels, int h, int w,
                               const float *mask_map, int mh, int mw, int oy, int ox, const int roll_xy[2],
                               const float *gram_target, float *sgrad_out, double out[3]);
diff --git a/style_transfer_amd/csrc/common.h b/style_transfer_amd/csrc/common.h
--- a/style_transfer_amd/csrc/common.h
+++ b/style_transfer_amd/csrc/common.h
@@ -131,6 +131,7 @@
     unsigned char *pool_codes = nullptr;
     unsigned char *in_codes = nullptr;
     const unsigned char *mask_codes = nullptr;
+    const unsigned *mask_bits = nullptr;
     unsigned char *out_codes = nullptr;
     bool wants_codes = false;
     bool skip_y = false;
@@ -210,6 +211,7 @@
     unsigned *y_amax = nullptr;
     const unsigned char *pin_codes = nullptr;
     int pin_mode = 0, pin_mask = 0;
+    const unsigned *mask_bits = nullptr;
 #ifdef STX_EXPERIMENT_BF3
     int vp_rows = 0, vp_tp = 0;
 #endif
@@ -241,7 +243,7 @@
 size_t h2_packed_floats(int K, int M);
 int h2_pack_weights(hipStream_t s, const float *w_caffe, int Mo, int Ko, int transpose_flip, float *packed);
 int h2_launch(hipStream_t s, const ConvConfig &cfg, const ConvProblem &p, int ksplit);
-enum { kH2Style = 1, kH2Content = 2, kH2MaskNibbles = 4, kH2MaskBlob = 8 };
+enum { kH2Style = 1, kH2Content = 2, kH2MaskNibbles = 4, kH2MaskBlob = 8, kH2MaskBits = 12 };
 int h2_variant(const ConvProblem &p, int pin, bool split);
 int h2_launch_variant(hipStream_t s, const WinoArgs &a, int n_wg, int cfg_id, int pin, int var);
 int h2_splitk_factor(const ConvConfig &cfg, const ConvProblem &p);
@@ -300,8 +302,11 @@
 int symm_num_workgroups(int C, int HW);
 bool symm_bf3_usable(const float *feat, const float *out, int C, int HW);
 bool symm_h2_usable(const float *feat, const float *out, int C, int HW);
+bool symm_h2_writes_sign_bits(int C, int HW);
+size_t symm_sign_bits_words(int C, int HW);
 int symm_h2_launch(hipStream_t s, const float *feat, const float *dsym, const unsigned *d_amax, int n_damax,
-                   const unsigned *f_amax, float *out, float *partials, int C, int HW);
+                   const unsigned *f_amax, float *out, float *partials, int C, int HW,
+                   unsigned *sign_bits = nullptr);
 int symm_bf3_launch(hipStream_t s, const float *feat, const float *dsym, unsigned short *pieces,
                     bool pieces_ready, float *out, float *partials, int C, int HW);
 
diff --git a/style_transfer_amd/csrc/conv_h2.hip b/style_transfer_amd/csrc/conv_h2.hip
--- a/style_transfer_amd/csrc/conv_h2.hip
+++ b/style_transfer_amd/csrc/conv_h2.hip
@@ -70,11 +70,13 @@
 template <int EPI, int MB, int PB, int PIN, int VAR = 0>
 __global__ __launch_bounds__(NT) void conv_h2_kernel(WinoArgs a) {
     static_assert(VAR == 0 || EPI == kEpiDgradInject, "variants are of the injecting epilogue");
-    static_assert(VAR == 0 || (((VAR & 3) == 1 || (VAR & 3) == 2) && ((VAR >> 2) == 1 || (VAR >> 2) == 2)), "h2_variant's codes");
+    static_assert(VAR == 0 || (((VAR & 3) == 1 || (VAR & 3) == 2) && (VAR >> 2) >= 1 && (VAR >> 2) <= 3), "h2_variant's codes");
+    static_assert((VAR >> 2) != 3 || (VAR & 3) == 1, "the sign-bit plane masks under a style term");
     const bool inj_style = VAR ? (VAR & 1) != 0 : a.inj.sgrad != nullptr;
     const bool inj_content = VAR ? (VAR & 2) != 0 : a.inj.content != nullptr;
     const bool mask_nibbles = VAR ? (VAR >> 2) == 1 : a.mask_codes != nullptr;
     const bool mask_blob = VAR ? (VAR >> 2) == 2 : !a.mask_codes && a.mask;
+    constexpr bool mask_bits = (VAR >> 2) == 3;
     using G = Geo<PB>;
     [[maybe_unused]] constexpr int PR = G::PR, RT = G::RT, V_PIECE = G::V_PIECE, V_BYTES = G::V_BYTES, NU = G::NU, FULL = G::FULL;
     constexpr size_t kLdsBytes = G::kLds;
@@ -401,6 +403,9 @@
         const_cast<unsigned char *>(a.mask_codes), 0, a.mask_codes ? a.M * cph * cpw : 0, 0x00020000);
     const __amdgpu_buffer_rsrc_t roc = __builtin_amdgcn_make_buffer_rsrc(
         a.out_codes, 0, a.out_codes ? a.M * cph * cpw : 0, 0x00020000);
+    [[maybe_unused]] const int mbw = (HW + 31) >> 5;
+    [[maybe_unused]] const __amdgpu_buffer_rsrc_t rmb = __builtin_amdgcn_make_buffer_rsrc(
+        const_cast<unsigned *>(a.mask_bits), 0, mask_bits ? a.M * mbw * 4 : 0, 0x00020000);
     const int M_ = a.M;
     struct LaneRows {
         int yy;
@@ -423,7 +428,7 @@
         r.vmc = in ? (unsigned)((4 * half) * cph * cpw + (r.yy >> 1) * cpw + (xx0 >> 1)) : kOob;
         return r;
     };
-    constexpr bool HOIST = !(PIN && PB == 2);
+    constexpr bool HOIST = !(PIN && PB == 2) || mask_bits;
     LaneRows rows0{};
     if (HOIST) rows0 = lane_rows(0);
     auto ld2 = [&](const __amdgpu_buffer_rsrc_t &rs, const LaneRows &lr, int y, unsigned so, auto even_c)
@@ -597,6 +602,19 @@
         float bs[8];
         f32x2 mk[16], sg[16];
         unsigned mkb[8];
+        constexpr bool even_w = decltype(even_c)::value;
+        [[maybe_unused]] unsigned mw[mask_bits ? 16 : 1], mw2[mask_bits && !even_w ? 16 : 1];
+        [[maybe_unused]] unsigned bvo[2][2], bsh[2][2];
+        if constexpr (mask_bits) {
+#pragma unroll
+            for (int y = 0; y < 2; ++y)
+#pragma unroll
+                for (int e = 0; e < (even_w ? 1 : 2); ++e) {
+                    const unsigned p = (unsigned)((lr.yy + y) * a.W + xx0 + e);
+                    bvo[y][e] = lr.vo[y][e] != kOob ? ((unsigned)(4 * half * mbw) + (p >> 5)) * 4u : kOob;
+                    bsh[y][e] = p & 31u;
+                }
+        }
 #pragma unroll
         for (int n = 0; n < 8; ++n) {
             const int c = chan(n);
@@ -607,6 +625,14 @@
                                : 0.f;
             } else if (EPI != kEpiPartial) {
                 if (mask_nibbles) mkb[n] = __builtin_amdgcn_raw_buffer_load_b8(rmc, lr.vmc, (unsigned)(c * cph * cpw), 0);
+                if constexpr (mask_bits) {
+#pragma unroll
+                    for (int y = 0; y < 2; ++y) {
+                        mw[2 * n + y] = __builtin_amdgcn_raw_buffer_load_b32(rmb, bvo[y][0], (unsigned)(c * mbw) * 4u, 0);
+                        if constexpr (!even_w)
+                            mw2[2 * n + y] = __builtin_amdgcn_raw_buffer_load_b32(rmb, bvo[y][1], (unsigned)(c * mbw) * 4u, 0);
+                    }
+                }
 #pragma unroll
                 for (int y = 0; y < 2; ++y) {
                     if (mask_blob && !(STX_H2_SKIP & 16)) mk[2 * n + y] = ld2(rmask, lr, y, so, even_c);
@@ -662,6 +688,12 @@
                             const unsigned nib = mkb[n] >> (2 * y);
                             v[y].x = (nib & 1u) ? v[y].x : 0.f;
                             v[y].y = (nib & 2u) ? v[y].y : 0.f;
+                        } else if constexpr (mask_bits) {
+                            const unsigned w0 = mw[2 * n + y] >> bsh[y][0];
+                            unsigned w1 = w0 >> 1;
+                            if constexpr (!even_w) w1 = mw2[2 * n + y] >> bsh[y][1];
+                            v[y].x = (w0 & 1u) ? v[y].x : 0.f;
+                            v[y].y = (w1 & 1u) ? v[y].y : 0.f;
                         } else if (mask_blob && !(STX_H2_SKIP & 16)) {
                             v[y].x = mk[2 * n + y].x > 0.f ? v[y].x : 0.f;
                             v[y].y = mk[2 * n + y].y > 0.f ? v[y].y : 0.f;
@@ -779,6 +811,9 @@
     STX_H2_VAR(kH2Style | kH2MaskBlob, 1 + STX_POOL_MAX)
     STX_H2_VAR(kH2Style | kH2MaskNibbles, 1 + STX_POOL_AVE)
     STX_H2_VAR(kH2Style | kH2MaskBlob, 1 + STX_POOL_AVE)
+    STX_H2_VAR(kH2Style | kH2MaskBits, 0)
+    STX_H2_VAR(kH2Style | kH2MaskBits, 1 + STX_POOL_MAX)
+    STX_H2_VAR(kH2Style | kH2MaskBits, 1 + STX_POOL_AVE)
 #undef STX_H2_VAR
     set_error("h2_launch_variant: no specialised body %d for a pooled input of kind %d", var, pin);
     return STX_ERR_UNSUPPORTED;
@@ -975,6 +1010,7 @@
 template __global__ void conv_h2_kernel<3, 2, 1, 0, kH2Content | kH2MaskNibbles>(WinoArgs);
 template __global__ void conv_h2_kernel<3, 1, 2, 1, kH2Style | kH2MaskBlob>(WinoArgs);
 template __global__ void conv_h2_kernel<3, 2, 1, 1, kH2Style | kH2MaskNibbles>(WinoArgs);
+template __global__ void conv_h2_kernel<3, 1, 2, 1, kH2Style | kH2MaskBits>(WinoArgs);
 #else
 int h2_variant(const ConvProblem &p, int pin, bool split) {
     if (split || p.epilogue != kEpiDgrad) return 0;
@@ -984,6 +1020,7 @@
     if (content && pin) return 0;
     const char *env = sw_env("STX_H2_INJECT_GENERIC");
     if (env && atoi(env) != 0) return 0;
+    if (!p.mask_codes && p.mask_bits && style) return kH2Style | kH2MaskBits;
     return (style ? kH2Style : kH2Content) | (p.mask_codes ? kH2MaskNibbles : kH2MaskBlob);
 }
 
@@ -1051,6 +1088,7 @@
     const int pin_kind = pin ? 1 + p.pin_mode : 0;
     const int var = h2_variant(p, pin_kind, split);
     if (p.variant_out) *p.variant_out = var;
+    if ((var >> 2) == (kH2MaskBits >> 2)) a.mask_bits = p.mask_bits;
     if (var) return h2_launch_variant(s, a, n_wg, cfg.id, pin_kind, var);
 #define STX_H2_CASE(E)                                                                   \
     case E:                                                                              \
diff --git a/style_transfer_amd/csrc/engine.cpp b/style_transfer_amd/csrc/engine.cpp
--- a/style_transfer_amd/csrc/engine.cpp
+++ b/style_transfer_amd/csrc/engine.cpp
@@ -370,6 +370,7 @@
         b.diff.release();
         b.codes.release();
         b.relu_codes.release();
+        b.sign_bits.release();
     }
     for (hipEvent_t ev : e->fence_events) (void)hipEventDestroy(ev);
     bool last;
diff --git a/style_transfer_amd/csrc/engine.h b/style_transfer_amd/csrc/engine.h
--- a/style_transfer_amd/csrc/engine.h
+++ b/style_transfer_amd/csrc/engine.h
@@ -56,6 +56,8 @@
     DevBuf relu_codes;
     bool relu_codes_valid = false;
     bool relu_codes_wanted = false;
+    DevBuf sign_bits;
+    bool sign_bits_valid = false, sign_bits_wanted = false;
     int amax_data = -1, amax_diff = -1;
     size_t count() const { return (size_t)channels * h * w; }
 };
@@ -419,7 +421,7 @@
 int launch_style_terms(stx_engine *e, hipStream_t stream, const float *feat, int C, int h, int w,
                        const float *target, float *sgrad, float *sc, const std::string &name,
                        const unsigned *f_amax = nullptr, float *term_scratch = nullptr,
-                       std::vector<SumJob> *defer = nullptr);
+                       std::vector<SumJob> *defer = nullptr, Blob *own = nullptr);
 constexpr size_t kMaskScratchFloats = kMaskParts + kMaskSgradParts;
 int launch_masked_style_terms(stx_engine *e, hipStream_t stream, const float *feat, int C, int h, int w,
                               const float *mask_map, const ContentWindow &win, const float *target,
diff --git a/style_transfer_amd/csrc/op_hooks.cpp b/style_transfer_amd/csrc/op_hooks.cpp
--- a/style_transfer_amd/csrc/op_hooks.cpp
+++ b/style_transfer_amd/csrc/op_hooks.cpp
@@ -416,4 +416,25 @@
     return STX_OK;
 }
 
-}
+int stx_op_blob_sign_bits(stx_engine *e, const char *layer, unsigned *words_out, size_t n_words, int *valid) {
+    if (!e || !layer || !valid) return STX_ERR_ARG;
+    const int blob = e->find_blob(layer);
+    if (blob < 0) {
+        set_error("stx_op_blob_sign_bits: unknown layer '%s'", layer);
+        return STX_ERR_ARG;
+    }
+    STX_TRY(e->set_device());
+    const Blob &b = e->blobs[blob];
+    *valid = b.sign_bits_valid ? 1 : 0;
+    if (!b.sign_bits_valid) return STX_OK;
+    if (!words_out || n_words != symm_sign_bits_words(b.channels, b.h * b.w)) {
+        set_error("stx_op_blob_sign_bits: the plane of %s has %zu words, the caller gave %zu", layer,
+                  symm_sign_bits_words(b.channels, b.h * b.w), n_words);
+        return STX_ERR_ARG;
+    }
+    STX_HIP(hipMemcpyAsync(words_out, b.sign_bits.ptr, n_words * sizeof(unsigned), hipMemcpyDeviceToHost, e->stream));
+    STX_HIP(hipStreamSynchronize(e->stream));
+    return STX_OK;
+}
+
+}
diff --git a/style_transfer_amd/csrc/symm.hip b/style_transfer_amd/csrc/symm.hip
--- a/style_transfer_amd/csrc/symm.hip
+++ b/style_transfer_amd/csrc/symm.hip
@@ -2,6 +2,7 @@
 #include <algorithm>
 #include <cstdlib>
 #include <cstring>
+#include <type_traits>
 
 #include "bf16x3.h"
 #include "common.h"
@@ -33,6 +34,30 @@
 constexpr int kChunkBytes = 3 * kPieceBytes;
 
 typedef unsigned u32x4y __attribute__((ext_vector_type(4)));
+
+template <int I = 0, typename F>
+__device__ __forceinline__ void static_for4(F &&f) {
+    if constexpr (I < 4) {
+        f(std::integral_constant<int, I>{});
+        static_for4<I + 1>(f);
+    }
+}
+
+template <int LANE>
+__device__ __forceinline__ unsigned put_ballots4(unsigned word, unsigned long long b0, unsigned long long b1,
+                                                 unsigned long long b2, unsigned long long b3) {
+    asm("s_nop 3\n\t"
+        "v_writelane_b32 %0, %1, %9\n\tv_writelane_b32 %0, %2, %10\n\t"
+        "v_writelane_b32 %0, %3, %11\n\tv_writelane_b32 %0, %4, %12\n\t"
+        "v_writelane_b32 %0, %5, %13\n\tv_writelane_b32 %0, %6, %14\n\t"
+        "v_writelane_b32 %0, %7, %15\n\tv_writelane_b32 %0, %8, %16"
+        : "+v"(word)
+        : "s"((unsigned)b0), "s"((unsigned)(b0 >> 32)), "s"((unsigned)b1), "s"((unsigned)(b1 >> 32)),
+          "s"((unsigned)b2), "s"((unsigned)(b2 >> 32)), "s"((unsigned)b3), "s"((unsigned)(b3 >> 32)),
+          "n"(LANE), "n"(32 + LANE), "n"(LANE + 1), "n"(33 + LANE), "n"(LANE + 2), "n"(34 + LANE), "n"(LANE + 3),
+          "n"(35 + LANE));
+    return word;
+}
 
 }
 
@@ -211,14 +236,16 @@
 constexpr int kHChunkBytes = 2 * kPieceBytes;
 constexpr int kHDLoads = kSM * kSK / 4 / 256;
 
-template <bool BIG>
+template <bool BIG, bool BITS = false>
 __global__ __launch_bounds__(256, 2) void symm_h2_kernel(const float *__restrict__ F,
                                                          const float *__restrict__ D,
                                                          const unsigned *__restrict__ d_amax, int n_damax,
                                                          const unsigned *__restrict__ f_amax,
                                                          float *__restrict__ S,
                                                          float *__restrict__ partials, int C, int Cp,
-                                                         int HW, unsigned f_bytes, int m_tiles) {
+                                                         int HW, unsigned f_bytes, int m_tiles,
+                                                         unsigned *__restrict__ bits) {
+    static_assert(!(BIG && BITS), "the sign-bit plane goes with the 32-bit addressing");
     __shared__ __attribute__((aligned(16))) unsigned char lds[2 * kHChunkBytes];
     __shared__ float wave_sum[4];
     __shared__ unsigned wave_max[4];
@@ -323,6 +350,31 @@
     if (n_chunks > 1) d_load(1);
     __syncthreads();
 
+    const int nw = (HW + 31) >> 5;
+    [[maybe_unused]] const __amdgpu_buffer_rsrc_t rb =
+        __builtin_amdgcn_make_buffer_rsrc(BITS ? bits : nullptr, 0, BITS ? C * nw * 4 : 0, 0x00020000);
+    [[maybe_unused]] unsigned bvoff = kOob;
+    [[maybe_unused]] int bch = 0;
+    const int wi0 = px0 >> 5;
+    if constexpr (BITS) {
+        const int bj = (l31 >> 3) & 1;
+        bch = g * 8 + (l31 & 7);
+        bvoff = l31 < 16 && wi0 + bj < nw ? (unsigned)(bch * nw + bj) * 4u : kOob;
+    }
+    [[maybe_unused]] auto sign_words = [&](int step_, int slot_) {
+        const int k0 = __builtin_amdgcn_readfirstlane(step_ * 16);
+        if (mt != 0 || k0 >= C || wi0 >= nw) return;
+        unsigned word = 0;
+        static_for4([&](auto q_c) __attribute__((always_inline)) {
+            constexpr int i = 4 * decltype(q_c)::value;
+            const float *x = &raw[slot_][i >> 3][i & 7];
+            word = put_ballots4<i>(word, __builtin_amdgcn_ballot_w64(x[0] > 0.f), __builtin_amdgcn_ballot_w64(x[1] > 0.f),
+                                   __builtin_amdgcn_ballot_w64(x[2] > 0.f), __builtin_amdgcn_ballot_w64(x[3] > 0.f));
+        });
+        const unsigned vo = k0 + bch < C ? bvoff : kOob;
+        __builtin_amdgcn_raw_buffer_store_b32(word, rb, vo, (unsigned)(k0 * nw + wi0) * 4u, 0);
+    };
+
     const unsigned a_off = (unsigned)(l31 * kRowBytes + g * 16);
     auto do_step = [&](int slot_, int buf, int s_in_chunk) {
         f16x8h bh[2], bl[2], ah[2], al[2];
@@ -345,6 +397,7 @@
         const int chunk = step / kSPC, s_in = step % kSPC, buf = chunk & 1;
         if (step + kRing - 1 < n_steps) f_load(step + kRing - 1, (slot_ + kRing - 1) % kRing);
         do_step(slot_, buf, s_in);
+        if constexpr (BITS) sign_words(step, slot_);
         if (s_in == kSPC - 1) {
             if (chunk + 1 < n_chunks) d_store(buf ^ 1);
             if (chunk + 2 < n_chunks) d_load(chunk + 2);
@@ -436,18 +489,34 @@
     return C % 4 == 0 && symm_bf3_usable(feat, out, C, HW);
 }
 
+static bool symm_h2_big(int C, int HW) {
+    const char *force_big = sw_env("STX_WINO_BIG");
+    return 4.0 * C * (double)HW >= 2147483648.0 || (force_big && atoi(force_big) == 1);
+}
+
+bool symm_h2_writes_sign_bits(int C, int HW) { return !symm_h2_big(C, HW); }
+
+size_t symm_sign_bits_words(int C, int HW) { return (size_t)C * ceil_div(HW, 32); }
+
 int symm_h2_launch(hipStream_t s, const float *feat, const float *dsym, const unsigned *d_amax, int n_damax,
-                   const unsigned *f_amax, float *out, float *partials, int C, int HW) {
+                   const unsigned *f_amax, float *out, float *partials, int C, int HW, unsigned *sign_bits) {
     const int Cp = ceil_div(C, kSM) * kSM;
     const int m_tiles = Cp / kSM;
     const double bytes = 4.0 * C * (double)HW;
-    const char *force_big = sw_env("STX_WINO_BIG");
-    if (bytes >= 2147483648.0 || (force_big && atoi(force_big) == 1))
+    const bool big = symm_h2_big(C, HW);
+    if (sign_bits && big) {
+        set_error("symm_h2_launch: no sign-bit plane from the launch of a blob of 2 GiB and more");
+        return STX_ERR_UNSUPPORTED;
+    }
+    if (big)
         symm_h2_kernel<true><<<symm_num_workgroups(C, HW), 256, 0, s>>>(feat, dsym, d_amax, n_damax, f_amax, out,
-                                                                      partials, C, Cp, HW, 0u, m_tiles);
+                                                                      partials, C, Cp, HW, 0u, m_tiles, nullptr);
+    else if (sign_bits)
+        symm_h2_kernel<false, true><<<symm_num_workgroups(C, HW), 256, 0, s>>>(
+            feat, dsym, d_amax, n_damax, f_amax, out, partials, C, Cp, HW, (unsigned)bytes, m_tiles, sign_bits);
     else
-        symm_h2_kernel<false><<<symm_num_workgroups(C, HW), 256, 0, s>>>(feat, dsym, d_amax, n_damax, f_amax, out,
-                                                                       partials, C, Cp, HW, (unsigned)bytes, m_tiles);
+        symm_h2_kernel<false><<<symm_num_workgroups(C, HW), 256, 0, s>>>(
+            feat, dsym, d_amax, n_damax, f_amax, out, partials, C, Cp, HW, (unsigned)bytes, m_tiles, nullptr);
     STX_CHECK_LAUNCH();
     return STX_OK;
 }
diff --git a/style_transfer_amd/csrc/tile_path.cpp b/style_transfer_amd/csrc/tile_path.cpp
--- a/style_transfer_amd/csrc/tile_path.cpp
+++ b/style_transfer_amd/csrc/tile_path.cpp
@@ -201,6 +201,12 @@
     return plan;
 }
 
+static bool wants_sign_bits(const Blob &t, const FwdConvPlan &plan) {
+    const char *codes = sw_env("STX_RELU_CODES"), *bits = sw_env("STX_SIGN_BITS");
+    if ((codes && atoi(codes) == 0) || (bits && atoi(bits) == 0)) return false;
+    return plan.relu_codes && t.relu && plan.conv_reader && conv_h2_enabled() && !t.relu_codes_valid;
+}
+
 static int run_conv_forward(stx_engine *e, int li, const FwdConvPlan &plan, bool *pooled) {
     const Layer &L = e->layers[li];
     const Layer *const pool = plan.pool;
@@ -215,6 +221,8 @@
         b.relu_codes_valid = false;
         b.relu_codes_wanted = false;
         t.relu_codes_valid = false;
+        t.sign_bits_valid = false;
+        t.sign_bits_wanted = wants_sign_bits(t, plan);
         unsigned *y_amax = nullptr;
         t.amax_data = -1;
         if (conv_h2_enabled()) {
@@ -280,6 +288,8 @@
         t.relu_codes_valid = conv_writes_out_codes(cfg, p, conv_splitk_factor(cfg, p));
         if (!t.relu_codes_valid) p.out_codes = nullptr;
     }
+    t.sign_bits_valid = false;
+    t.sign_bits_wanted = wants_sign_bits(t, plan);
     ProfScope scope(e, "fwd " + L.name, direct);
     return launch_conv(e, cfg, p);
 }
@@ -317,6 +327,7 @@
     p.mask = b.relu ? b.data.f() : nullptr;
     p.mask_codes = b.relu && b.relu_codes_valid ? static_cast<const unsigned char *>(b.relu_codes.ptr) : nullptr;
     p.wants_codes = b.relu && b.relu_codes_wanted;
+    p.mask_bits = b.relu && b.sign_bits_valid ? static_cast<const unsigned *>(b.sign_bits.ptr) : nullptr;
     if (cp.ks == 3 && cp.cin <= 4) {
         if (fused) *fused = false;
         const float *packed = nullptr;
@@ -483,6 +494,8 @@
     for (Blob &b : e->blobs) {
         b.amax_data = -1;
         b.relu_codes_valid = false;
+        b.sign_bits_valid = false;
+        b.sign_bits_wanted = false;
     }
     for (size_t li = 1; li < e->layers.size(); ++li) {
         const Layer &L = e->layers[li];
diff --git a/style_transfer_amd/csrc/tile_terms.cpp b/style_transfer_amd/csrc/tile_terms.cpp
--- a/style_transfer_amd/csrc/tile_terms.cpp
+++ b/style_transfer_amd/csrc/tile_terms.cpp
@@ -13,7 +13,7 @@
 
 int launch_style_terms(stx_engine *e, hipStream_t stream, const float *feat, int C, int h, int w,
                        const float *target, float *sgrad, float *sc, const std::string &name,
-                       const unsigned *f_amax, float *term_scratch, std::vector<SumJob> *defer) {
+                       const unsigned *f_amax, float *term_scratch, std::vector<SumJob> *defer, Blob *own) {
     const int HW = h * w;
     const bool fused = e->first_gram_valid && e->first_gram_blob >= 0 &&
                        feat == e->blobs[e->first_gram_blob].data.f() && C == 64;
@@ -65,10 +65,17 @@
             STX_TRY(e->symm_partials.ensure((size_t)n_wg * sizeof(float)));
             symm_partials = e->symm_partials.f();
         }
-        if (symm_h2)
+        if (symm_h2) {
+            unsigned *sign_bits = nullptr;
+            if (own && feat == own->data.f() && own->relu && own->sign_bits_wanted && !own->relu_codes_valid &&
+                symm_h2_writes_sign_bits(C, HW)) {
+                STX_TRY(own->sign_bits.ensure(symm_sign_bits_words(C, HW) * sizeof(unsigned)));
+                sign_bits = static_cast<unsigned *>(own->sign_bits.ptr);
+            }
             STX_TRY(symm_h2_launch(stream, feat, e->dsym.f(), reinterpret_cast<const unsigned *>(block_sumsq + fin_blocks),
-                                   fin_blocks, f_amax, sgrad, symm_partials, C, HW));
-        else
+                                   fin_blocks, f_amax, sgrad, symm_partials, C, HW, sign_bits));
+            if (sign_bits) own->sign_bits_valid = true;
+        } else
             STX_TRY(symm_bf3_launch(stream, feat, e->dsym.f(), static_cast<unsigned short *>(e->dsym_pieces.ptr),
                                     pieces != nullptr, sgrad, symm_partials, C, HW));
         return finish(symm_partials, n_wg);
@@ -514,7 +521,7 @@
 int queue_tap_terms(TileRun &run, size_t k) {
     stx_engine *e = run.e;
     const TilePlan &plan = run.plan;
-    const Blob &b = e->blobs[plan.order[k].blob];
+    Blob &b = e->blobs[plan.order[k].blob];
     for (size_t i = plan.first_term[k]; i < plan.terms.size() && plan.terms[i].tap == (int)k; ++i) {
         const PlannedTerm &t = plan.terms[i];
         size_t si;
@@ -538,7 +545,7 @@
             break;
         case TermKind::Style:
             STX_TRY(launch_style_terms(e, e->stream, b.data.f(), b.channels, b.h, b.w, t.target, sgrad, sc, b.name,
-                                       f_amax, late, run.defer()));
+                                       f_amax, late, run.defer(), &b));
             break;
         case TermKind::MaskedStyle:
             STX_TRY(launch_masked_style_terms(e, e->stream, b.data.f(), b.channels, b.h, b.w, t.mask, t.win, t.target,
diff --git a/style_transfer_amd/lib.py b/style_transfer_amd/lib.py
--- a/style_transfer_amd/lib.py
+++ b/style_transfer_amd/lib.py
@@ -188,6 +188,7 @@
     'stx_op_pool_forward': [_vp, _vp, _i, _i, _i, _i, _vp],
     'stx_op_pool_backward': [_vp, _vp, _vp, _i, _i, _i, _i, _vp, _vp],
     'stx_op_style_terms': [_vp, _vp, _i, _i, _i, _vp, _vp, _vp, c_double_p, c_double_p],
+    'stx_op_blob_sign_bits': [_vp, ctypes.c_char_p, _vp, _sz, c_int_p],
     'stx_op_masked_style_terms': [_vp, _vp, _i, _i, _i, _vp, _i, _i, _i, _i, c_int_p, _vp, _vp, c_double_p],
     'stx_op_masked_content_terms': [_vp, _vp, _i, _i, _i, _vp, _i, _i, _vp, _i, _i, c_int_p, _vp, c_double_p],
     'stx_op_stat_terms': [_vp, _vp, _i, _i, _i, _vp, _vp, _vp, c_double_p],
```

New measurement: 283.4, median of 2. About the same (-0.0%).
